# g1mv/density

Hardware: NVIDIA H100
Metric: chameleon_encode_input_GBps (higher is better)
Workload: dtype u32

## Files before the change

### density_b200/csrc/api.cu

```cuda
#include "../../include/density_b200.h"
#include "common.cuh"
#include "encode_internal.cuh"

#include <dlfcn.h>

#include <atomic>
#include <condition_variable>
#include <cstdio>
#include <cstring>
#include <deque>
#include <mutex>
#include <string>
#include <thread>
#include <vector>

namespace dns {

static thread_local std::string g_last_error;
static std::atomic<uint64_t> g_launches{0};

static void set_error(const char* what, cudaError_t e) {
    char buf[512];
    snprintf(buf, sizeof buf, "%s: %s (%s)", what, cudaGetErrorString(e), cudaGetErrorName(e));
    g_last_error = buf;
}
static void set_error(const char* what) { g_last_error = what; }

struct DevBuf {
    uint8_t* p = nullptr; size_t bytes = 0;
    cudaError_t ensure(size_t need, cudaStream_t stream = nullptr) {
        if (need <= bytes) return cudaSuccess;
        if (p) { cudaFree(p); p = nullptr; bytes = 0; }
        size_t want = need + need / 8 + 4096;
        cudaError_t e = cudaMalloc(&p, want);
        if (e != cudaSuccess) { cudaGetLastError(); e = cudaMalloc(&p, need); want = need; }
        if (e == cudaSuccess) { bytes = want; e = cudaMemsetAsync(p, 0, want, stream); }
        return e;
    }
    void release() { if (p) cudaFree(p); p = nullptr; bytes = 0; }
};

class CopyPool {
public:
    static CopyPool& get() { static CopyPool p; return p; }
    void copy(void* dst, const void* src, size_t n) {
        const size_t nparts = (n >= (8u << 20) && !th_.empty()) ? th_.size() : 1;
        if (nparts == 1) { memcpy(dst, src, n); return; }
        Job job; job.left = (int)nparts;
        const size_t per = ((n + nparts - 1) / nparts + 4095) & ~(size_t)4095;
        {
            std::lock_guard<std::mutex> lk(m_);
            for (size_t k = 0; k < nparts; ++k) {
                const size_t off = k * per;
                const size_t len = off >= n ? 0 : (n - off < per ? n - off : per);
                q_.push_back(Task{static_cast<uint8_t*>(dst) + off, static_cast<const uint8_t*>(src) + off, len, &job});
            }
        }
        cv_.notify_all();
        std::unique_lock<std::mutex> lk(m_);
        done_.wait(lk, [&] { return job.left == 0; });
    }
private:
    struct Job { int left; };
    struct Task { uint8_t* d; const uint8_t* s; size_t n; Job* job; };
    CopyPool() {
        unsigned hw = std::thread::hardware_concurrency();
        unsigned nt = hw >= 128 ? 32 : (hw >= 32 ? 16 : (hw >= 8 ? hw / 2 : 0));
        for (unsigned i = 0; i < nt; ++i) th_.emplace_back([this] { run(); });
    }
    ~CopyPool() {
        { std::lock_guard<std::mutex> lk(m_); stop_ = true; }
        cv_.notify_all();
        for (auto& t : th_) t.join();
    }
    void run() {
        for (;;) {
            Task t;
            {
                std::unique_lock<std::mutex> lk(m_);
                cv_.wait(lk, [&] { return stop_ || !q_.empty(); });
                if (stop_ && q_.empty()) return;
                t = q_.front(); q_.pop_front();
            }
            if (t.n) memcpy(t.d, t.s, t.n);
            {
                std::lock_guard<std::mutex> lk(m_);
                if (--t.job->left == 0) done_.notify_all();
            }
        }
    }
    std::vector<std::thread> th_;
    std::mutex m_;
    std::condition_variable cv_, done_;
    std::deque<Task> q_;
    bool stop_ = false;
};

constexpr size_t PIN_SLOT = 64u << 20;
struct PinRing {
    uint8_t* slot[2] = {nullptr, nullptr};
    cudaEvent_t ev[2] = {nullptr, nullptr};
    bool used[2] = {false, false};
    unsigned next = 0;
    cudaError_t ensure() {
        for (int k = 0; k < 2; ++k) {
            if (!slot[k]) { cudaError_t e = cudaHostAlloc(reinterpret_cast<void**>(&slot[k]), PIN_SLOT, cudaHostAllocDefault); if (e != cudaSuccess) return e; }
            if (!ev[k]) { cudaError_t e = cudaEventCreateWithFlags(&ev[k], cudaEventDisableTiming); if (e != cudaSuccess) return e; }
        }
        return cudaSuccess;
    }
    void release() {
        for (int k = 0; k < 2; ++k) { if (slot[k]) cudaFreeHost(slot[k]); if (ev[k]) cudaEventDestroy(ev[k]); slot[k] = nullptr; ev[k] = nullptr; used[k] = false; }
    }
};

static bool is_pageable_host(const void* p) {
    cudaPointerAttributes a;
    cudaError_t e = cudaPointerGetAttributes(&a, p);
    if (e != cudaSuccess) { cudaGetLastError(); return true; }
    return a.type == cudaMemoryTypeUnregistered;
}
static cudaError_t h2d_any(PinRing& ring, uint8_t* dst_dev, const uint8_t* src, size_t n, cudaStream_t s, bool pageable) {
    if (!pageable) return cudaMemcpyAsync(dst_dev, src, n, cudaMemcpyHostToDevice, s);
    cudaError_t e = ring.ensure();
    for (size_t off = 0; off < n && e == cudaSuccess; off += PIN_SLOT) {
        const size_t len = n - off < PIN_SLOT ? n - off : PIN_SLOT;
        const unsigned k = ring.next++ & 1u;
        if (ring.used[k]) e = cudaEventSynchronize(ring.ev[k]);
        if (e != cudaSuccess) break;
        CopyPool::get().copy(ring.slot[k], src + off, len);
        e = cudaMemcpyAsync(dst_dev + off, ring.slot[k], len, cudaMemcpyHostToDevice, s);
        if (e == cudaSuccess) e = cudaEventRecord(ring.ev[k], s);
        ring.used[k] = true;
    }
    return e;
}
static cudaError_t d2h_any(PinRing& ring, uint8_t* dst, const uint8_t* src_dev, size_t n, cudaStream_t s, bool pageable) {
    if (!pageable) return cudaMemcpyAsync(dst, src_dev, n, cudaMemcpyDeviceToHost, s);
    cudaError_t e = ring.ensure();
    size_t pend_off = 0, pend_len = 0; unsigned pend_k = 0; bool pending = false;
    for (size_t off = 0; off < n && e == cudaSuccess; off += PIN_SLOT) {
        const size_t len = n - off < PIN_SLOT ? n - off : PIN_SLOT;
        const unsigned k = ring.next++ & 1u;
        if (ring.used[k] && !(pending && pend_k == k)) e = cudaEventSynchronize(ring.ev[k]);
        if (e != cudaSuccess) break;
        e = cudaMemcpyAsync(ring.slot[k], src_dev + off, len, cudaMemcpyDeviceToHost, s);
        if (e == cudaSuccess) e = cudaEventRecord(ring.ev[k], s);
        ring.used[k] = true;
        if (pending && e == cudaSuccess) {
            e = cudaEventSynchronize(ring.ev[pend_k]);
            if (e == cudaSuccess) CopyPool::get().copy(dst + pend_off, ring.slot[pend_k], pend_len);
        }
        pend_off = off; pend_len = len; pend_k = k; pending = true;
    }
    if (pending && e == cudaSuccess) {
        e = cudaEventSynchronize(ring.ev[pend_k]);
        if (e == cudaSuccess) CopyPool::get().copy(dst + pend_off, ring.slot[pend_k], pend_len);
    }
    return e;
}

struct DeviceCtx {
    int dev = -1;
    int num_sms = 0;
    bool ready = false;
    cudaStream_t stream = nullptr;
    cudaStream_t h2d_stream = nullptr, d2h_stream = nullptr;
    DevBuf ws, stage_in, stage_out, pipe_tables, dec_tables;
    DevBuf chee_tables[2][3];
    uint32_t chee_epoch = 0;
    uint64_t* h_sizes = nullptr;
    cudaEvent_t ev_h2d[2] = {nullptr, nullptr};
    PinRing ring_in, ring_out;
    uint64_t* d_size = nullptr;
    uint64_t* h_size = nullptr;
    ChamLayout layout{};
    int last_was_chameleon_fastpath_capable = 0;
    bool profile = false;
    static constexpr int PROF_RING = 64;
    cudaEvent_t ev[PROF_RING][4] = {};
    uint64_t prof_count = 0;
    const void* last_cl_status = nullptr;
    cudaEvent_t ws_free = nullptr;
    bool ws_free_recorded = false;
    std::mutex mu;
};

constexpr int MAX_DEVICES = 64;
static DeviceCtx g_ctx[MAX_DEVICES];
static std::mutex g_ctx_mu;

static DeviceCtx* current_ctx() {
    int dev = -1;
    cudaError_t e = cudaGetDevice(&dev);
    if (e != cudaSuccess) { set_error("cudaGetDevice", e); return nullptr; }
    if (dev < 0 || dev >= MAX_DEVICES) { set_error("device index out of range"); return nullptr; }
    DeviceCtx* c = &g_ctx[dev];
    std::lock_guard<std::mutex> lk(g_ctx_mu);
    if (!c->ready) {
        cudaDeviceProp prop;
        e = cudaGetDeviceProperties(&prop, dev);
        if (e != cudaSuccess) { set_error("cudaGetDeviceProperties", e); return nullptr; }
        if (prop.major != 9 || prop.minor != 0) { set_error("density_b200 is built for sm_90a and requires a compute capability 9.0 device (H100)"); return nullptr; }
        c->dev = dev;
        c->num_sms = prop.multiProcessorCount;
        e = cudaStreamCreateWithFlags(&c->stream, cudaStreamNonBlocking);
        if (e == cudaSuccess) e = cudaStreamCreateWithFlags(&c->h2d_stream, cudaStreamNonBlocking);
        if (e == cudaSuccess) e = cudaStreamCreateWithFlags(&c->d2h_stream, cudaStreamNonBlocking);
        if (e != cudaSuccess) { set_error("cudaStreamCreate", e); return nullptr; }
        e = cudaMalloc(&c->d_size, 64);
        if (e != cudaSuccess) { set_error("cudaMalloc", e); return nullptr; }
        e = cudaMallocHost(&c->h_size, 64);
        if (e == cudaSuccess) e = cudaMallocHost(&c->h_sizes, sizeof(uint64_t) * 4096);
        if (e != cudaSuccess) { set_error("cudaMallocHost", e); return nullptr; }
        e = cudaEventCreateWithFlags(&c->ws_free, cudaEventDisableTiming);
        if (e != cudaSuccess) { set_error("cudaEventCreate", e); return nullptr; }
        c->ready = true;
    }
    return c;
}

static size_t safe_size(int alg, size_t size) {
    const size_t B = alg_block_bytes(alg), S = alg_sig_bytes(alg);
    return size + (size / B) * S + ((size % B) ? S : 0);
}

static bool is_device_pointer(const void* p) {
    cudaPointerAttributes a;
    cudaError_t e = cudaPointerGetAttributes(&a, p);
    if (e != cudaSuccess) { cudaGetLastError(); return false; }
    return a.type == cudaMemoryTypeDevice || a.type == cudaMemoryTypeManaged;
}

static bool ws_acquire(DeviceCtx* c, cudaStream_t stream) {
    if (!c->ws_free_recorded) return true;
    cudaError_t e = cudaStreamWaitEvent(stream, c->ws_free, 0);
    if (e != cudaSuccess) { set_error("cudaStreamWaitEvent", e); return false; }
    return true;
}
static void ws_release(DeviceCtx* c, cudaStream_t stream) {
    if (cudaEventRecord(c->ws_free, stream) == cudaSuccess) c->ws_free_recorded = true;
}

static int encode_device_locked_impl(DeviceCtx* c, int alg, const uint8_t* d_in, size_t n, uint8_t* d_out, size_t cap,
                                     uint64_t* d_out_size, cudaStream_t stream, int path);
static int encode_device_locked(DeviceCtx* c, int alg, const uint8_t* d_in, size_t n, uint8_t* d_out, size_t cap,
                                uint64_t* d_out_size, cudaStream_t stream, int path) {
    if (!ws_acquire(c, stream)) return DENSITY_B200_ECUDA;
    const int rc = encode_device_locked_impl(c, alg, d_in, n, d_out, cap, d_out_size, stream, path);
    ws_release(c, stream);
    return rc;
}
static int encode_device_locked_impl(DeviceCtx* c, int alg, const uint8_t* d_in, size_t n, uint8_t* d_out, size_t cap,
                                     uint64_t* d_out_size, cudaStream_t stream, int path) {
    uint64_t launches = 0;
    cudaError_t e;
    const bool aligned = !(reinterpret_cast<uintptr_t>(d_in) & 3) && !(reinterpret_cast<uintptr_t>(d_out) & 1);
    if (alg == ALG_CHAMELEON && path != 3 && aligned) {
        ChamLayout L;
        size_t need = cham_workspace_bytes(n, c->num_sms, &L);
        e = c->ws.ensure(need, stream);
        if (e != cudaSuccess) { set_error("workspace cudaMalloc", e); return DENSITY_B200_ECUDA; }
        c->layout = L;
        if (path == 2) {
            e = cham_encode_protected_only(d_in, n, c->ws.p, L, d_out, cap, d_out_size, stream, &launches);
        } else {
            const uint32_t nruns = cham_pick_runs(n, c->num_sms);
            cudaEvent_t* ev = nullptr;
            if (c->profile) {
                ev = c->ev[c->prof_count % DeviceCtx::PROF_RING];
                for (int i = 0; i < 4; ++i) if (!ev[i]) cudaEventCreate(&ev[i]);
            }
            e = cham_encode_phase1(d_in, n, c->ws.p, L, nruns, nullptr, stream, &launches, ev);
            if (e == cudaSuccess && path == 4)
                e = cham_encode_phase2_blocking(d_in, n, c->ws.p, L, nruns, d_out, cap, d_out_size, 12, stream, &launches);
            else if (e == cudaSuccess)
                e = cham_encode_phase2(d_in, n, c->ws.p, L, nruns, nullptr, d_out, cap, d_out_size, path == 0, false, stream, &launches, ev);
            if (ev != nullptr && e == cudaSuccess) c->prof_count++;
        }
        c->last_was_chameleon_fastpath_capable = (path != 2);
    } else if ((alg == ALG_CHEETAH || alg == ALG_LION) && path != 3 && !(reinterpret_cast<uintptr_t>(d_in) & 3) && !(reinterpret_cast<uintptr_t>(d_out) & 1)) {
        const size_t pw = (chee_workspace_bytes(n, c->num_sms) + 255) & ~(size_t)255;
        e = c->ws.ensure(pw + 256 + scalar_workspace_bytes(alg), stream);
        if (e != cudaSuccess) { set_error("workspace cudaMalloc", e); return DENSITY_B200_ECUDA; }
        DevBuf* tb = c->chee_tables[alg == ALG_LION];
        for (int rg = 0; rg < 3 && e == cudaSuccess; ++rg) e = tb[rg].ensure(chee_tables_bytes(alg, rg, n, c->num_sms) + 256, stream);
        if (e != cudaSuccess) { set_error("workspace cudaMalloc", e); return DENSITY_B200_ECUDA; }
        if (c->chee_epoch > 0x0FFFFF00u) {
            for (int a2 = 0; a2 < 2; ++a2) for (int rg = 0; rg < 3; ++rg)
                if (c->chee_tables[a2][rg].p) { e = cudaMemsetAsync(c->chee_tables[a2][rg].p, 0, c->chee_tables[a2][rg].bytes, stream); if (e != cudaSuccess) break; }
            if (e != cudaSuccess) { set_error("cudaMemsetAsync", e); return DENSITY_B200_ECUDA; }
            c->chee_epoch = 0;
        }
        uint32_t* d_conv = reinterpret_cast<uint32_t*>(c->ws.p + pw);
        uint8_t* const tabs[3] = {tb[0].p, tb[1].p, tb[2].p};
        for (int attempt = 0; attempt <= (path == 4 ? 12 : 0); ++attempt) {
            if (attempt > 0) {
                uint32_t conv = 0;
                e = cudaMemcpyAsync(&conv, d_conv, sizeof conv, cudaMemcpyDeviceToHost, stream);
                if (e == cudaSuccess) e = cudaStreamSynchronize(stream);
                if (e != cudaSuccess || conv) break;
            }
            const uint32_t epoch_base = c->chee_epoch + 1;
            c->chee_epoch += 32;
            e = chee_encode_parallel(alg, d_in, n, d_out, cap, c->ws.p, tabs, epoch_base, c->num_sms, d_out_size, d_conv, attempt > 0, stream, &launches);
            if (e != cudaSuccess) break;
        }
        if (e == cudaSuccess && path != 1)
            e = scalar_encode(alg, d_in, n, d_out, cap, c->ws.p + pw + 256, d_out_size, stream, &launches, d_conv);
        c->last_was_chameleon_fastpath_capable = 0;
    } else {
        if (reinterpret_cast<uintptr_t>(d_out) & 1) { set_error("encode_device: d_out must be 2-byte aligned"); return DENSITY_B200_EARG; }
        e = c->ws.ensure(scalar_workspace_bytes(alg), stream);
        if (e != cudaSuccess) { set_error("workspace cudaMalloc", e); return DENSITY_B200_ECUDA; }
        e = scalar_encode(alg, d_in, n, d_out, cap, c->ws.p, d_out_size, stream, &launches);
        c->last_was_chameleon_fastpath_capable = 0;
    }
    g_launches += launches;
    if (e != cudaSuccess) { set_error("encode launch", e); return DENSITY_B200_ECUDA; }
    return DENSITY_B200_OK;
}

static int decode_device_locked_impl(DeviceCtx* c, int alg, const uint8_t* d_in, size_t n, uint8_t* d_out, size_t cap,
                                     uint64_t* d_out_size, cudaStream_t stream, int path);
static int decode_device_locked(DeviceCtx* c, int alg, const uint8_t* d_in, size_t n, uint8_t* d_out, size_t cap,
                                uint64_t* d_out_size, cudaStream_t stream, int path = 0) {
    if (!ws_acquire(c, stream)) return DENSITY_B200_ECUDA;
    const int rc = decode_device_locked_impl(c, alg, d_in, n, d_out, cap, d_out_size, stream, path);
    ws_release(c, stream);
    return rc;
}
static int decode_device_locked_impl(DeviceCtx* c, int alg, const uint8_t* d_in, size_t n, uint8_t* d_out, size_t cap,
                                     uint64_t* d_out_size, cudaStream_t stream, int path) {
    uint64_t launches = 0;
    cudaError_t e;
    const bool parallel_ok = alg == ALG_CHAMELEON && path != 3 && !(reinterpret_cast<uintptr_t>(d_in) & 1) && !(reinterpret_cast<uintptr_t>(d_out) & 3);
    if (parallel_ok) {
        const size_t pw = (cham_decode_workspace_bytes(n, cap, c->num_sms) + 255) & ~(size_t)255;
        e = c->ws.ensure(pw + 256 + scalar_workspace_bytes(alg), stream);
        if (e != cudaSuccess) { set_error("workspace cudaMalloc", e); return DENSITY_B200_ECUDA; }
        uint32_t* d_nonquiet = reinterpret_cast<uint32_t*>(c->ws.p + pw);
        e = cham_decode_parallel(d_in, n, d_out, cap, c->ws.p, c->num_sms, d_out_size, d_nonquiet, stream, &launches);
        if (e == cudaSuccess && path != 1)
            e = scalar_decode(alg, d_in, n, d_out, cap, c->ws.p + pw + 256, d_out_size, stream, &launches, d_nonquiet);
        g_launches += launches;
        if (e != cudaSuccess) { set_error("decode launch", e); return DENSITY_B200_ECUDA; }
        return DENSITY_B200_OK;
    }
    if (alg == ALG_CHEETAH && path != 3 && !(reinterpret_cast<uintptr_t>(d_in) & 1) && !(reinterpret_cast<uintptr_t>(d_out) & 3)) {
        const size_t pw = (chee_decode_workspace_bytes(n, cap, c->num_sms) + 255) & ~(size_t)255;
        e = c->ws.ensure(pw + 256 + 2 * ((scalar_workspace_bytes(alg) + 255) & ~(size_t)255), stream);
        if (e == cudaSuccess) e = c->dec_tables.ensure(chee_decode_tables_bytes(n, c->num_sms) + 256, stream);
        if (e != cudaSuccess) { set_error("workspace cudaMalloc", e); return DENSITY_B200_ECUDA; }
        uint32_t* d_fallback = reinterpret_cast<uint32_t*>(c->ws.p + pw);
        uint8_t* tail_ws = c->ws.p + pw + 256;
        uint8_t* scalar_ws = tail_ws + ((scalar_workspace_bytes(alg) + 255) & ~(size_t)255);
        e = cudaMemsetAsync(tail_ws, 0, 256, stream);
        if (e == cudaSuccess) e = chee_decode_parallel(d_in, n, d_out, cap, c->ws.p, c->dec_tables.p, tail_ws, c->num_sms, d_out_size, d_fallback, stream, &launches);
        if (e == cudaSuccess) {
            const void* cl_st = nullptr;
            const void* b_st = chee_decode_status_ptr(c->ws.p, n, cap, c->num_sms, &cl_st);
            c->last_cl_status = cl_st;
            e = scalar_decode_tail(alg, d_in, n, d_out, cap, tail_ws, b_st, cl_st, d_out_size, stream, &launches, d_fallback);
        }
        if (e == cudaSuccess && path != 1)
            e = scalar_decode(alg, d_in, n, d_out, cap, scalar_ws, d_out_size, stream, &launches, d_fallback);
        g_launches += launches;
        if (e != cudaSuccess) { set_error("decode launch", e); return DENSITY_B200_ECUDA; }
        return DENSITY_B200_OK;
    }
    e = c->ws.ensure(scalar_workspace_bytes(alg), stream);
    if (e != cudaSuccess) { set_error("workspace cudaMalloc", e); return DENSITY_B200_ECUDA; }
    e = scalar_decode(alg, d_in, n, d_out, cap, c->ws.p, d_out_size, stream, &launches);
    g_launches += launches;
    if (e != cudaSuccess) { set_error("decode launch", e); return DENSITY_B200_ECUDA; }
    return DENSITY_B200_OK;
}

constexpr size_t PIPE_CHUNK = 64u << 20;
constexpr size_t PIPE_MIN_BYTES = 96u << 20;

static size_t chameleon_encode_host_pipelined(DeviceCtx* c, const uint8_t* in, size_t n, uint8_t* out, size_t out_cap) {
    const size_t nchunks = (n + PIPE_CHUNK - 1) / PIPE_CHUNK;
    if (nchunks > 4096) return (size_t)-1;
    cudaError_t e = c->stage_in.ensure(n + 16);
    if (e == cudaSuccess) e = c->stage_out.ensure(safe_size(ALG_CHAMELEON, n) + 16);
    if (e == cudaSuccess) e = c->pipe_tables.ensure(2 * 65536 * sizeof(uint32_t) + (nchunks + 1) * sizeof(uint64_t) + 256);
    ChamLayout L;
    if (e == cudaSuccess) e = c->ws.ensure(cham_workspace_bytes(PIPE_CHUNK, c->num_sms, &L));
    if (e != cudaSuccess) { set_error("pipeline cudaMalloc", e); return 0; }
    c->layout = L;
    uint32_t* d_acc = reinterpret_cast<uint32_t*>(c->pipe_tables.p);
    uint32_t* d_tab = d_acc + 65536;
    uint64_t* d_sizes = reinterpret_cast<uint64_t*>(c->pipe_tables.p + 2 * 65536 * sizeof(uint32_t));
    uint32_t* d_flag = reinterpret_cast<uint32_t*>(d_sizes + nchunks);
    for (int k = 0; k < 2; ++k) if (!c->ev_h2d[k]) cudaEventCreateWithFlags(&c->ev_h2d[k], cudaEventDisableTiming);
    uint64_t launches = 0;
    const bool pg_in = is_pageable_host(in), pg_out = is_pageable_host(out);
    std::vector<cudaEvent_t> evs(nchunks, nullptr);
    bool ok = true;
    auto stage_chunk = [&](size_t i) {
        const size_t off = i * PIPE_CHUNK, len = (n - off < PIPE_CHUNK) ? (n - off) : PIPE_CHUNK;
        ok = h2d_any(c->ring_in, c->stage_in.p + off, in + off, len, c->h2d_stream, pg_in) == cudaSuccess;
        if (ok) ok = cudaEventCreateWithFlags(&evs[i], cudaEventDisableTiming) == cudaSuccess;
        if (ok) ok = cudaEventRecord(evs[i], c->h2d_stream) == cudaSuccess;
    };
    size_t staged = 0;
    for (; staged < (pg_in ? (size_t)1 : nchunks) && ok; ++staged) stage_chunk(staged);
    size_t out_off = 0;
    bool nonquiet = false;
    e = cudaMemsetAsync(d_flag, 0, sizeof(uint32_t), c->stream);
    if (ok && e == cudaSuccess) e = cham_table_init(d_acc, c->stream, &launches);
    for (size_t i = 0; i < nchunks && ok && e == cudaSuccess; ++i) {
        const size_t off = i * PIPE_CHUNK, len = (n - off < PIPE_CHUNK) ? (n - off) : PIPE_CHUNK;
        const uint32_t nruns = cham_pick_runs(len, c->num_sms);
        e = cudaStreamWaitEvent(c->stream, evs[i], 0);
        if (e == cudaSuccess) e = cham_encode_phase1(c->stage_in.p + off, len, c->ws.p, L, nruns, d_tab, c->stream, &launches);
        if (e == cudaSuccess) e = cham_encode_phase2(c->stage_in.p + off, len, c->ws.p, L, nruns, i ? d_acc : nullptr, c->stage_out.p + out_off,
                                                     c->stage_out.bytes - out_off, d_sizes + i, false, i != 0, c->stream, &launches);
        if (e == cudaSuccess) e = cham_status_accumulate(c->ws.p, L, d_flag, c->stream, &launches);
        if (e == cudaSuccess) e = cham_table_fold(d_acc, d_tab, c->stream, &launches);
        if (e == cudaSuccess) e = cudaMemcpyAsync(c->h_sizes + i, d_sizes + i, sizeof(uint64_t), cudaMemcpyDeviceToHost, c->stream);
        if (e == cudaSuccess) e = cudaMemcpyAsync(c->h_size, d_flag, sizeof(uint32_t), cudaMemcpyDeviceToHost, c->stream);
        if (e == cudaSuccess && pg_in && staged < nchunks) { stage_chunk(staged); ++staged; }
        if (e == cudaSuccess) e = cudaStreamSynchronize(c->stream);
        if (e != cudaSuccess) break;
        if (*reinterpret_cast<uint32_t*>(c->h_size) != 0) { nonquiet = true; break; }
        const uint64_t sz = c->h_sizes[i];
        if (sz == 0) { ok = false; set_error("pipelined encode: device reported an error"); break; }
        if (out_off + sz > out_cap) { ok = false; set_error("output buffer too small"); break; }
        e = d2h_any(c->ring_out, out + out_off, c->stage_out.p + out_off, sz, c->d2h_stream, pg_out);
        out_off += sz;
    }
    g_launches += launches;
    if (nonquiet) for (; staged < nchunks && ok; ++staged) stage_chunk(staged);
    cudaError_t e2 = cudaStreamSynchronize(c->h2d_stream);
    cudaError_t e3 = cudaStreamSynchronize(c->d2h_stream);
    for (auto ev : evs) if (ev) cudaEventDestroy(ev);
    if (e != cudaSuccess || e2 != cudaSuccess || e3 != cudaSuccess) { set_error("pipelined encode", e != cudaSuccess ? e : (e2 != cudaSuccess ? e2 : e3)); return 0; }
    if (!ok) return 0;
    if (nonquiet) return (size_t)-1;
    c->last_was_chameleon_fastpath_capable = 2;
    return out_off;
}

static size_t run_sync(bool encode, int alg, const uint8_t* in, size_t n, uint8_t* out, size_t out_cap) {
    g_last_error.clear();
    if ((!in && n) || (!out && out_cap)) { set_error("null pointer"); return 0; }
    if (n == 0) return 0;
    DeviceCtx* c = current_ctx();
    if (!c) return 0;
    std::lock_guard<std::mutex> lk(c->mu);
    const bool in_dev = is_device_pointer(in), out_dev = is_device_pointer(out);
    cudaError_t e;
    if (in_dev || out_dev) {
        e = cudaDeviceSynchronize();
        if (e != cudaSuccess) { set_error("cudaDeviceSynchronize", e); return 0; }
    }
    const uint8_t* d_in = in;
    uint8_t* d_out = out;
    size_t d_cap = out_cap;
    bool input_staged = false;
    if (encode && alg == ALG_CHAMELEON && !in_dev && !out_dev && n >= PIPE_MIN_BYTES) {
        const size_t r = chameleon_encode_host_pipelined(c, in, n, out, out_cap);
        if (r != (size_t)-1) return r;
        input_staged = true;
        d_in = c->stage_in.p;
    }
    if (!in_dev && !input_staged) {
        e = c->stage_in.ensure(n + 16);
        if (e != cudaSuccess) { set_error("staging cudaMalloc", e); return 0; }
        e = h2d_any(c->ring_in, c->stage_in.p, in, n, c->stream, is_pageable_host(in));
        if (e != cudaSuccess) { set_error("H2D copy", e); return 0; }
        d_in = c->stage_in.p;
    }
    if (!out_dev) {
        d_cap = encode ? safe_size(alg, n) : out_cap;
        e = c->stage_out.ensure(d_cap + 16);
        if (e != cudaSuccess) { set_error("staging cudaMalloc", e); return 0; }
        d_out = c->stage_out.p;
    }
    int rc = encode ? encode_device_locked(c, alg, d_in, n, d_out, d_cap, c->d_size, c->stream, 4)
                    : decode_device_locked(c, alg, d_in, n, d_out, d_cap, c->d_size, c->stream);
    if (rc != DENSITY_B200_OK) { cudaStreamSynchronize(c->stream); return 0; }
    e = cudaMemcpyAsync(c->h_size, c->d_size, sizeof(uint64_t), cudaMemcpyDeviceToHost, c->stream);
    if (e == cudaSuccess) e = cudaStreamSynchronize(c->stream);
    if (e != cudaSuccess) { set_error("stream sync", e); return 0; }
    const uint64_t produced = *c->h_size;
    if (produced == 0) { set_error(encode ? "encode failed on device (output capacity?)" : "decode failed on device (malformed stream or output capacity)"); return 0; }
    if (produced > out_cap) { set_error("output buffer too small"); return 0; }
    if (!out_dev) {
        e = d2h_any(c->ring_out, out, d_out, produced, c->stream, is_pageable_host(out));
        if (e == cudaSuccess) e = cudaStreamSynchronize(c->stream);
        if (e != cudaSuccess) { set_error("D2H copy", e); return 0; }
    }
    return (size_t)produced;
}

}

using namespace dns;

extern "C" {

int density_b200_decode_status(uint64_t* out10) {
    DeviceCtx* c = current_ctx();
    if (!c || !c->ws.p) return DENSITY_B200_EARG;
    std::lock_guard<std::mutex> lk(c->mu);
    unsigned char raw[64] = {0};
    if (cudaDeviceSynchronize() != cudaSuccess || cudaMemcpy(raw, c->ws.p, sizeof(raw), cudaMemcpyDeviceToHost) != cudaSuccess) return DENSITY_B200_ECUDA;
    const unsigned long long* q = reinterpret_cast<const unsigned long long*>(raw);
    const unsigned int* w = reinterpret_cast<const unsigned int*>(raw + 24);
    out10[0] = q[0]; out10[1] = q[1]; out10[2] = q[2];
    for (int k = 0; k < 7; ++k) out10[3 + k] = w[k];
    return DENSITY_B200_OK;
}

size_t chameleon_encode(const uint8_t* i, size_t n, uint8_t* o, size_t c) { return run_sync(true, ALG_CHAMELEON, i, n, o, c); }
size_t chameleon_decode(const uint8_t* i, size_t n, uint8_t* o, size_t c) { return run_sync(false, ALG_CHAMELEON, i, n, o, c); }
size_t chameleon_safe_encode_buffer_size(size_t s) { return safe_size(ALG_CHAMELEON, s); }
size_t cheetah_encode(const uint8_t* i, size_t n, uint8_t* o, size_t c) { return run_sync(true, ALG_CHEETAH, i, n, o, c); }
size_t cheetah_decode(const uint8_t* i, size_t n, uint8_t* o, size_t c) { return run_sync(false, ALG_CHEETAH, i, n, o, c); }
size_t cheetah_safe_encode_buffer_size(size_t s) { return safe_size(ALG_CHEETAH, s); }
size_t lion_encode(const uint8_t* i, size_t n, uint8_t* o, size_t c) { return run_sync(true, ALG_LION, i, n, o, c); }
size_t lion_decode(const uint8_t* i, size_t n, uint8_t* o, size_t c) { return run_sync(false, ALG_LION, i, n, o, c); }
size_t lion_safe_encode_buffer_size(size_t s) { return safe_size(ALG_LION, s); }

static int device_entry(bool encode, int alg, const uint8_t* d_in, size_t n, uint8_t* d_out, size_t cap, uint64_t* d_out_size,
                        void* stream, int path) {
    g_last_error.clear();
    if (alg < 0 || alg > 2) { set_error("bad algorithm id"); return DENSITY_B200_EARG; }
    if (!d_out_size || (!d_in && n) || (!d_out && cap)) { set_error("null pointer"); return DENSITY_B200_EARG; }
    DeviceCtx* c = current_ctx();
    if (!c) return DENSITY_B200_ECUDA;
    std::lock_guard<std::mutex> lk(c->mu);
    cudaStream_t s = reinterpret_cast<cudaStream_t>(stream);
    if (n == 0) {
        cudaError_t e = cudaMemsetAsync(d_out_size, 0, sizeof(uint64_t), s);
        if (e != cudaSuccess) { set_error("memset", e); return DENSITY_B200_ECUDA; }
        return DENSITY_B200_OK;
    }
    return encode ? encode_device_locked(c, alg, d_in, n, d_out, cap, d_out_size, s, path)
                  : decode_device_locked(c, alg, d_in, n, d_out, cap, d_out_size, s, path);
}

int density_b200_encode_device(int alg, const uint8_t* d_in, size_t n, uint8_t* d_out, size_t cap, uint64_t* d_out_size, void* stream) {
    return device_entry(true, alg, d_in, n, d_out, cap, d_out_size, stream, 0);
}
int density_b200_decode_device(int alg, const uint8_t* d_in, size_t n, uint8_t* d_out, size_t cap, uint64_t* d_out_size, void* stream) {
    return device_entry(false, alg, d_in, n, d_out, cap, d_out_size, stream, 0);
}
int density_b200_encode_device_path(int alg, const uint8_t* d_in, size_t n, uint8_t* d_out, size_t cap, uint64_t* d_out_size,
                                    void* stream, int path) {
    if (path < 0 || path > 4) { set_error("bad path"); return DENSITY_B200_EARG; }
    return device_entry(true, alg, d_in, n, d_out, cap, d_out_size, stream, path);
}
int density_b200_decode_device_path(int alg, const uint8_t* d_in, size_t n, uint8_t* d_out, size_t cap, uint64_t* d_out_size,
                                    void* stream, int path) {
    if (path != 0 && path != 1 && path != 3) { set_error("bad path"); return DENSITY_B200_EARG; }
    return device_entry(false, alg, d_in, n, d_out, cap, d_out_size, stream, path);
}

struct density_b200_shard {
    DevBuf ws;
    ChamLayout L{};
    const uint8_t* d_in = nullptr;
    size_t n = 0;
    uint32_t nruns = 0;
    int is_last = 1;
    int num_sms = 0;
    bool phase1_done = false;
};

density_b200_shard* density_b200_shard_create(void) {
    g_last_error.clear();
    DeviceCtx* c = current_ctx();
    if (!c) return nullptr;
    density_b200_shard* s = new density_b200_shard();
    s->num_sms = c->num_sms;
    return s;
}
void density_b200_shard_destroy(density_b200_shard* s) {
    if (!s) return;
    s->ws.release();
    delete s;
}
int density_b200_shard_phase1(density_b200_shard* s, const uint8_t* d_in, size_t n, int is_last_shard, uint32_t* d_table_out, void* stream) {
    g_last_error.clear();
    if (!s || (!d_in && n) || !d_table_out) { set_error("null pointer"); return DENSITY_B200_EARG; }
    if (!is_last_shard && (n % 256)) { set_error("non-final shards must be a multiple of 256 bytes"); return DENSITY_B200_EARG; }
    if (reinterpret_cast<uintptr_t>(d_in) & 3) { set_error("d_in must be 4-byte aligned"); return DENSITY_B200_EARG; }
    size_t need = cham_workspace_bytes(n, s->num_sms, &s->L);
    cudaError_t e = s->ws.ensure(need);
    if (e != cudaSuccess) { set_error("workspace cudaMalloc", e); return DENSITY_B200_ECUDA; }
    s->d_in = d_in; s->n = n; s->is_last = is_last_shard; s->nruns = cham_pick_runs(n, s->num_sms);
    uint64_t launches = 0;
    cudaStream_t st = reinterpret_cast<cudaStream_t>(stream);
    if (n == 0) {
        e = cudaMemsetAsync(d_table_out, 0, 65536 * sizeof(uint32_t), st);
    } else {
        e = cham_encode_phase1(d_in, n, s->ws.p, s->L, s->nruns, d_table_out, st, &launches);
    }
    g_launches += launches;
    if (e != cudaSuccess) { set_error("shard phase1", e); return DENSITY_B200_ECUDA; }
    s->phase1_done = true;
    return DENSITY_B200_OK;
}
int density_b200_shard_phase2(density_b200_shard* s, const uint32_t* d_carry_in, uint8_t* d_out, size_t cap, uint64_t* d_out_size,
                              uint32_t* d_flags, void* stream) {
    g_last_error.clear();
    if (!s || !s->phase1_done || !d_out_size) { set_error("shard_phase2: phase1 not done / null pointer"); return DENSITY_B200_EARG; }
    if (reinterpret_cast<uintptr_t>(d_out) & 1) { set_error("d_out must be 2-byte aligned"); return DENSITY_B200_EARG; }
    uint64_t launches = 0;
    cudaStream_t st = reinterpret_cast<cudaStream_t>(stream);
    cudaError_t e = cham_encode_phase2(s->d_in, s->n, s->ws.p, s->L, s->nruns, d_carry_in, d_out, cap, d_out_size, false,
                                       d_carry_in != nullptr, st, &launches, nullptr);
    if (e == cudaSuccess && d_flags) {
        if (s->n) e = cudaMemcpyAsync(d_flags, s->ws.p + s->L.status + offsetof(Status, nonquiet), sizeof(uint32_t), cudaMemcpyDeviceToDevice, st);
        else e = cudaMemsetAsync(d_flags, 0, sizeof(uint32_t), st);
    }
    g_launches += launches;
    if (e != cudaSuccess) { set_error("shard phase2", e); return DENSITY_B200_ECUDA; }
    return DENSITY_B200_OK;
}

struct density_b200_decode_shard {
    DevBuf ws;
    const uint8_t* d_in = nullptr;
    size_t n = 0, cap = 0;
    int is_last = 1;
    int num_sms = 0;
    bool phase1_done = false;
};

density_b200_decode_shard* density_b200_decode_shard_create(void) {
    g_last_error.clear();
    DeviceCtx* c = current_ctx();
    if (!c) return nullptr;
    density_b200_decode_shard* s = new density_b200_decode_shard();
    s->num_sms = c->num_sms;
    return s;
}
void density_b200_decode_shard_destroy(density_b200_decode_shard* s) {
    if (!s) return;
    s->ws.release();
    delete s;
}
int density_b200_decode_shard_phase1(density_b200_decode_shard* s, const uint8_t* d_in, size_t n, size_t cap, int is_last_shard,
                                     uint32_t* d_table_out, void* stream) {
    g_last_error.clear();
    if (!s || (!d_in && n) || !d_table_out) { set_error("null pointer"); return DENSITY_B200_EARG; }
    if (reinterpret_cast<uintptr_t>(d_in) & 1) { set_error("d_in must be 2-byte aligned"); return DENSITY_B200_EARG; }
    cudaStream_t st = reinterpret_cast<cudaStream_t>(stream);
    s->phase1_done = false;
    cudaError_t e = s->ws.ensure(cham_decode_workspace_bytes(n, cap, s->num_sms), st);
    if (e != cudaSuccess) { set_error("workspace cudaMalloc", e); return DENSITY_B200_ECUDA; }
    s->d_in = d_in; s->n = n; s->cap = cap; s->is_last = is_last_shard;
    uint64_t launches = 0;
    if (n == 0) e = cudaMemsetAsync(d_table_out, 0, 65536 * sizeof(uint32_t), st);
    else e = cham_decode_phase1(d_in, n, cap, s->ws.p, s->num_sms, d_table_out, st, &launches);
    g_launches += launches;
    if (e != cudaSuccess) { set_error("decode shard phase1", e); return DENSITY_B200_ECUDA; }
    s->phase1_done = true;
    return DENSITY_B200_OK;
}
int density_b200_decode_shard_phase2(density_b200_decode_shard* s, const uint32_t* d_carry_in, uint8_t* d_out, uint64_t* d_out_size,
                                     uint32_t* d_seam8, void* stream) {
    g_last_error.clear();
    if (!s || !s->phase1_done) { set_error("decode_shard_phase2: phase1 not done"); return DENSITY_B200_EARG; }
    if ((!d_out && s->cap) || !d_out_size || !d_seam8) { set_error("null pointer"); return DENSITY_B200_EARG; }
    if (reinterpret_cast<uintptr_t>(d_out) & 3) { set_error("d_out must be 4-byte aligned"); return DENSITY_B200_EARG; }
    cudaStream_t st = reinterpret_cast<cudaStream_t>(stream);
    uint64_t launches = 0;
    cudaError_t e;
    if (s->n == 0) {
        e = cudaMemsetAsync(d_out_size, 0, sizeof(uint64_t), st);
        if (e == cudaSuccess) e = cudaMemsetAsync(d_seam8, 0, 8 * sizeof(uint32_t), st);
    } else {
        e = cham_decode_phase2(s->d_in, s->n, d_out, s->cap, s->ws.p, s->num_sms, d_carry_in, d_out_size, st, &launches);
        if (e == cudaSuccess) e = cham_decode_seam_words(s->d_in, s->n, s->cap, s->ws.p, s->num_sms, s->is_last, d_out_size, d_seam8, st, &launches);
    }
    g_launches += launches;
    s->phase1_done = false;
    if (e != cudaSuccess) { set_error("decode shard phase2", e); return DENSITY_B200_ECUDA; }
    return DENSITY_B200_OK;
}

namespace {
typedef struct ncclComm* nccl_comm_t;
struct nccl_unique_id { char internal[128]; };
enum { NCCL_UINT8 = 1, NCCL_UINT32 = 3 };
struct NcclApi {
    int (*GetUniqueId)(nccl_unique_id*) = nullptr;
    int (*CommInitRank)(nccl_comm_t*, int, nccl_unique_id, int) = nullptr;
    int (*CommDestroy)(nccl_comm_t) = nullptr;
    int (*AllGather)(const void*, void*, size_t, int, nccl_comm_t, cudaStream_t) = nullptr;
    int (*Send)(const void*, size_t, int, int, nccl_comm_t, cudaStream_t) = nullptr;
    int (*Recv)(void*, size_t, int, int, nccl_comm_t, cudaStream_t) = nullptr;
    int (*GroupStart)() = nullptr;
    int (*GroupEnd)() = nullptr;
    const char* (*GetErrorString)(int) = nullptr;
    bool ok = false;
};
NcclApi* nccl_api() {
    static NcclApi api;
    static std::once_flag once;
    std::call_once(once, [] {
        void* h = dlopen("libnccl.so.2", RTLD_NOW | RTLD_NOLOAD);
        if (!h) h = dlopen("libnccl.so.2", RTLD_NOW | RTLD_GLOBAL);
        if (!h) return;
        auto sym = [&](const char* n) { return dlsym(h, n); };
        api.GetUniqueId = reinterpret_cast<decltype(api.GetUniqueId)>(sym("ncclGetUniqueId"));
        api.CommInitRank = reinterpret_cast<decltype(api.CommInitRank)>(sym("ncclCommInitRank"));
        api.CommDestroy = reinterpret_cast<decltype(api.CommDestroy)>(sym("ncclCommDestroy"));
        api.AllGather = reinterpret_cast<decltype(api.AllGather)>(sym("ncclAllGather"));
        api.Send = reinterpret_cast<decltype(api.Send)>(sym("ncclSend"));
        api.Recv = reinterpret_cast<decltype(api.Recv)>(sym("ncclRecv"));
        api.GroupStart = reinterpret_cast<decltype(api.GroupStart)>(sym("ncclGroupStart"));
        api.GroupEnd = reinterpret_cast<decltype(api.GroupEnd)>(sym("ncclGroupEnd"));
        api.GetErrorString = reinterpret_cast<decltype(api.GetErrorString)>(sym("ncclGetErrorString"));
        api.ok = api.GetUniqueId && api.CommInitRank && api.CommDestroy && api.AllGather && api.Send && api.Recv && api.GroupStart && api.GroupEnd;
    });
    return api.ok ? &api : nullptr;
}
bool nccl_check(int rc, const char* what) {
    if (rc == 0) return true;
    NcclApi* a = nccl_api();
    std::string m = std::string(what) + ": " + ((a && a->GetErrorString) ? a->GetErrorString(rc) : "NCCL error");
    dns::set_error(m.c_str());
    return false;
}
}

struct density_b200_sharded {
    int rank = 0, world = 1, num_sms = 0;
    nccl_comm_t comm = nullptr;
    DevBuf ws, aux;
    DevBuf dws;
    ChamLayout L{};
    uint64_t* h_offsets = nullptr;
    uint64_t* h_maps = nullptr;
    cudaEvent_t ev[6] = {};
    bool timed = false;
};

int density_b200_sharded_unique_id(uint8_t* out128) {
    g_last_error.clear();
    NcclApi* a = nccl_api();
    if (!a || !out128) { set_error("NCCL is not available in this process"); return DENSITY_B200_ECUDA; }
    nccl_unique_id id;
    if (!nccl_check(a->GetUniqueId(&id), "ncclGetUniqueId")) return DENSITY_B200_ECUDA;
    memcpy(out128, id.internal, 128);
    return DENSITY_B200_OK;
}

density_b200_sharded* density_b200_sharded_create(const uint8_t* nccl_unique_id_128, int rank, int world) {
    g_last_error.clear();
    if (world < 1 || rank < 0 || rank >= world) { set_error("bad rank / world"); return nullptr; }
    DeviceCtx* c = current_ctx();
    if (!c) return nullptr;
    density_b200_sharded* h = new density_b200_sharded();
    h->rank = rank; h->world = world; h->num_sms = c->num_sms;
    if (world > 1) {
        NcclApi* a = nccl_api();
        if (!a || !nccl_unique_id_128) { set_error("NCCL is not available / no unique id"); delete h; return nullptr; }
        nccl_unique_id id; memcpy(id.internal, nccl_unique_id_128, 128);
        if (!nccl_check(a->CommInitRank(&h->comm, world, id, rank), "ncclCommInitRank")) { delete h; return nullptr; }
    }
    if (cudaMallocHost(&h->h_offsets, sizeof(uint64_t) * (world + 2)) != cudaSuccess ||
        cudaMallocHost(&h->h_maps, sizeof(uint64_t) * DENSITY_B200_LOCATE_MAP_WORDS * world) != cudaSuccess) {
        set_error("cudaMallocHost");
        if (h->h_offsets) cudaFreeHost(h->h_offsets);
        if (h->comm) { NcclApi* a = nccl_api(); if (a) a->CommDestroy(h->comm); }
        delete h;
        return nullptr;
    }
    for (auto& e : h->ev) cudaEventCreate(&e);
    return h;
}

void density_b200_sharded_destroy(density_b200_sharded* h) {
    if (!h) return;
    if (h->comm) { NcclApi* a = nccl_api(); if (a) a->CommDestroy(h->comm); }
    h->ws.release(); h->aux.release(); h->dws.release();
    if (h->h_offsets) cudaFreeHost(h->h_offsets);
    if (h->h_maps) cudaFreeHost(h->h_maps);
    for (auto& e : h->ev) if (e) cudaEventDestroy(e);
    delete h;
}

struct ShardedAux { uint32_t *tables, *carry, *words; uint64_t *offsets, *maps; };
static cudaError_t sharded_aux(density_b200_sharded* h, cudaStream_t st, ShardedAux* x) {
    const size_t W = (size_t)h->world;
    const size_t aux_tables = W * 65536 * sizeof(uint32_t), aux_carry = 65536 * sizeof(uint32_t), aux_words = W * 8 * sizeof(uint32_t);
    const size_t aux_offsets = (W + 2) * sizeof(uint64_t), aux_maps = W * DENSITY_B200_LOCATE_MAP_WORDS * sizeof(uint64_t);
    const cudaError_t e = h->aux.ensure(aux_tables + aux_carry + aux_words + aux_offsets + aux_maps + 256, st);
    x->tables = reinterpret_cast<uint32_t*>(h->aux.p);
    x->carry = reinterpret_cast<uint32_t*>(h->aux.p + aux_tables);
    x->words = reinterpret_cast<uint32_t*>(h->aux.p + aux_tables + aux_carry);
    x->offsets = reinterpret_cast<uint64_t*>(h->aux.p + aux_tables + aux_carry + aux_words);
    x->maps = reinterpret_cast<uint64_t*>(h->aux.p + aux_tables + aux_carry + aux_words + aux_offsets);
    return e;
}

int density_b200_encode_sharded(density_b200_sharded* h, const uint8_t* d_in, size_t n, uint8_t* d_out, size_t cap, uint64_t* d_out_size,
                                uint32_t* d_flags, uint64_t* d_total_size, int gather_root, uint8_t* d_gather, size_t gather_cap, void* stream_v) {
    g_last_error.clear();
    if (!h || (!d_in && n) || !d_out || !d_out_size) { set_error("null pointer"); return DENSITY_B200_EARG; }
    const bool last = h->rank == h->world - 1;
    if (!last && (n % 256)) { set_error("non-final shards must be a multiple of 256 bytes"); return DENSITY_B200_EARG; }
    if ((reinterpret_cast<uintptr_t>(d_in) & 3) || (reinterpret_cast<uintptr_t>(d_out) & 1)) { set_error("d_in must be 4-byte, d_out 2-byte aligned"); return DENSITY_B200_EARG; }
    if (gather_root >= h->world) { set_error("bad gather root"); return DENSITY_B200_EARG; }
    cudaStream_t st = reinterpret_cast<cudaStream_t>(stream_v);
    NcclApi* a = h->world > 1 ? nccl_api() : nullptr;
    const size_t W = (size_t)h->world;
    cudaError_t e = h->ws.ensure(cham_workspace_bytes(n, h->num_sms, &h->L), st);
    ShardedAux x;
    if (e == cudaSuccess) e = sharded_aux(h, st, &x);
    if (e != cudaSuccess) { set_error("workspace cudaMalloc", e); return DENSITY_B200_ECUDA; }
    uint32_t* d_tables = x.tables;
    uint32_t* d_carry = x.carry;
    uint32_t* d_words = x.words;
    uint64_t* d_offsets = x.offsets;
    const uint32_t nruns = cham_pick_runs(n, h->num_sms);
    uint64_t launches = 0;
    cudaEventRecord(h->ev[0], st);
    cudaEvent_t pev[4] = {nullptr, nullptr, nullptr, nullptr};
    if (n) e = cham_encode_phase1(d_in, n, h->ws.p, h->L, nruns, d_tables + (size_t)h->rank * 65536, st, &launches);
    else e = cudaMemsetAsync(d_tables + (size_t)h->rank * 65536, 0, 65536 * sizeof(uint32_t), st);
    if (e != cudaSuccess) { set_error("sharded phase 1", e); return DENSITY_B200_ECUDA; }
    cudaEventRecord(h->ev[1], st);
    if (h->world > 1) {
        if (!a) { set_error("NCCL is not available"); return DENSITY_B200_ECUDA; }
        if (!nccl_check(a->AllGather(d_tables + (size_t)h->rank * 65536, d_tables, 65536, NCCL_UINT32, h->comm, st), "ncclAllGather(tables)")) return DENSITY_B200_ECUDA;
    }
    e = cham_rank_fold(d_tables, (uint32_t)h->rank, d_carry, st, &launches);
    cudaEventRecord(h->ev[2], st);
    pev[2] = h->ev[3]; pev[3] = h->ev[4];
    if (e == cudaSuccess) e = cham_encode_phase2(d_in, n, h->ws.p, h->L, nruns, d_carry, d_out, cap, d_out_size, false, false, st, &launches, n ? pev : nullptr);
    if (!n) { cudaEventRecord(h->ev[3], st); cudaEventRecord(h->ev[4], st); }
    if (e == cudaSuccess && n) e = cham_seam_words(h->ws.p, h->L, n, d_out_size, d_words + 8 * h->rank, st, &launches);
    else if (e == cudaSuccess) e = cudaMemsetAsync(d_words + 8 * h->rank, 0, 8 * sizeof(uint32_t), st);
    if (e != cudaSuccess) { set_error("sharded phase 2", e); return DENSITY_B200_ECUDA; }
    if (h->world > 1 && !nccl_check(a->AllGather(d_words + 8 * h->rank, d_words, 8, NCCL_UINT32, h->comm, st), "ncclAllGather(seams)")) return DENSITY_B200_ECUDA;
    e = cham_seam_verdict(d_words, (uint32_t)h->world, (uint32_t)h->rank, d_flags, d_total_size, d_offsets, st, &launches);
    if (e != cudaSuccess) { set_error("seam verdict", e); return DENSITY_B200_ECUDA; }
    if (gather_root >= 0) {
        e = cudaMemcpyAsync(h->h_offsets, d_offsets, (W + 1) * sizeof(uint64_t), cudaMemcpyDeviceToHost, st);
        if (e == cudaSuccess) e = cudaStreamSynchronize(st);
        if (e != cudaSuccess) { set_error("gather: sizes to host", e); return DENSITY_B200_ECUDA; }
        const uint64_t total = h->h_offsets[W];
        const uint64_t my_off = h->h_offsets[h->rank], my_size = h->h_offsets[h->rank + 1] - my_off;
        if (h->rank == gather_root) {
            if (!d_gather || gather_cap < total) { set_error("gather buffer too small"); return DENSITY_B200_ECAPACITY; }
            if (my_size) e = cudaMemcpyAsync(d_gather + my_off, d_out, my_size, cudaMemcpyDeviceToDevice, st);
            if (e != cudaSuccess) { set_error("gather: local piece", e); return DENSITY_B200_ECUDA; }
        }
        if (h->world > 1) {
            if (!nccl_check(a->GroupStart(), "ncclGroupStart")) return DENSITY_B200_ECUDA;
            bool ok = true;
            if (h->rank == gather_root) {
                for (int r = 0; r < h->world && ok; ++r) {
                    const uint64_t sz = h->h_offsets[r + 1] - h->h_offsets[r];
                    if (r != h->rank && sz) ok = nccl_check(a->Recv(d_gather + h->h_offsets[r], sz, NCCL_UINT8, r, h->comm, st), "ncclRecv");
                }
            } else if (my_size) ok = nccl_check(a->Send(d_out, my_size, NCCL_UINT8, gather_root, h->comm, st), "ncclSend");
            if (!nccl_check(a->GroupEnd(), "ncclGroupEnd") || !ok) return DENSITY_B200_ECUDA;
        }
    }
    cudaEventRecord(h->ev[5], st);
    h->timed = true;
    g_launches += launches;
    return DENSITY_B200_OK;
}

static int decode_sharded_piece(density_b200_sharded* h, const uint8_t* d_in, size_t n, int is_last, uint8_t* d_out, size_t cap,
                                uint64_t* d_out_size, uint32_t* d_flags, uint64_t* d_total_size, uint64_t* d_out_offset, cudaStream_t st) {
    NcclApi* a = h->world > 1 ? nccl_api() : nullptr;
    if (h->world > 1 && !a) { set_error("NCCL is not available"); return DENSITY_B200_ECUDA; }
    ShardedAux x;
    cudaError_t e = h->dws.ensure(cham_decode_workspace_bytes(n, cap, h->num_sms), st);
    if (e == cudaSuccess) e = sharded_aux(h, st, &x);
    if (e != cudaSuccess) { set_error("workspace cudaMalloc", e); return DENSITY_B200_ECUDA; }
    uint32_t* my_table = x.tables + (size_t)h->rank * 65536;
    uint32_t* my_words = x.words + 8 * h->rank;
    uint64_t launches = 0;
    if (n) e = cham_decode_phase1(d_in, n, cap, h->dws.p, h->num_sms, my_table, st, &launches);
    else e = cudaMemsetAsync(my_table, 0, 65536 * sizeof(uint32_t), st);
    if (e != cudaSuccess) { set_error("sharded decode phase 1", e); return DENSITY_B200_ECUDA; }
    if (h->world > 1 && !nccl_check(a->AllGather(my_table, x.tables, 65536, NCCL_UINT32, h->comm, st), "ncclAllGather(tables)")) return DENSITY_B200_ECUDA;
    e = cham_rank_fold(x.tables, (uint32_t)h->rank, x.carry, st, &launches);
    if (e == cudaSuccess && n) e = cham_decode_phase2(d_in, n, d_out, cap, h->dws.p, h->num_sms, x.carry, d_out_size, st, &launches);
    if (e == cudaSuccess && n) e = cham_decode_seam_words(d_in, n, cap, h->dws.p, h->num_sms, is_last, d_out_size, my_words, st, &launches);
    if (e == cudaSuccess && !n) e = cudaMemsetAsync(d_out_size, 0, sizeof(uint64_t), st);
    if (e == cudaSuccess && !n) e = cudaMemsetAsync(my_words, 0, 8 * sizeof(uint32_t), st);
    if (e != cudaSuccess) { set_error("sharded decode phase 2", e); return DENSITY_B200_ECUDA; }
    if (h->world > 1 && !nccl_check(a->AllGather(my_words, x.words, 8, NCCL_UINT32, h->comm, st), "ncclAllGather(seams)")) return DENSITY_B200_ECUDA;
    e = cham_seam_verdict(x.words, (uint32_t)h->world, (uint32_t)h->rank, d_flags, d_total_size, x.offsets, st, &launches);
    g_launches += launches;
    if (e == cudaSuccess && d_out_offset) e = cudaMemcpyAsync(d_out_offset, x.offsets + h->rank, sizeof(uint64_t), cudaMemcpyDeviceToDevice, st);
    if (e != cudaSuccess) { set_error("seam verdict", e); return DENSITY_B200_ECUDA; }
    return DENSITY_B200_OK;
}

int density_b200_decode_sharded(density_b200_sharded* h, const uint8_t* d_in, size_t n, uint8_t* d_out, size_t cap, uint64_t* d_out_size,
                                uint32_t* d_flags, uint64_t* d_total_size, void* stream_v) {
    g_last_error.clear();
    if (!h || (!d_in && n) || (!d_out && cap) || !d_out_size || !d_flags) { set_error("null pointer"); return DENSITY_B200_EARG; }
    if ((reinterpret_cast<uintptr_t>(d_in) & 1) || (reinterpret_cast<uintptr_t>(d_out) & 3)) { set_error("d_in must be 2-byte, d_out 4-byte aligned"); return DENSITY_B200_EARG; }
    return decode_sharded_piece(h, d_in, n, h->rank == h->world - 1, d_out, cap, d_out_size, d_flags, d_total_size, nullptr,
                                reinterpret_cast<cudaStream_t>(stream_v));
}

int density_b200_decode_locate(density_b200_decode_shard* s, const uint8_t* d_in, size_t n_range, size_t n_halo, uint64_t* d_map, void* stream) {
    g_last_error.clear();
    if (!s || (!d_in && n_range + n_halo) || !d_map) { set_error("null pointer"); return DENSITY_B200_EARG; }
    if ((reinterpret_cast<uintptr_t>(d_in) & 1) || (reinterpret_cast<uintptr_t>(d_map) & 7)) { set_error("d_in must be 2-byte, d_map 8-byte aligned"); return DENSITY_B200_EARG; }
    cudaStream_t st = reinterpret_cast<cudaStream_t>(stream);
    s->phase1_done = false;
    cudaError_t e = s->ws.ensure(cham_locate_workspace_bytes(n_range + n_halo), st);
    if (e != cudaSuccess) { set_error("workspace cudaMalloc", e); return DENSITY_B200_ECUDA; }
    uint64_t launches = 0;
    e = cham_decode_locate(d_in, n_range, n_halo, s->ws.p, d_map, st, &launches);
    g_launches += launches;
    if (e != cudaSuccess) { set_error("decode locate", e); return DENSITY_B200_ECUDA; }
    return DENSITY_B200_OK;
}

int density_b200_locate_piece(const uint64_t* h_maps, int world, int rank, uint64_t out4[4]) {
    g_last_error.clear();
    constexpr uint64_t W = DENSITY_B200_LOCATE_MAP_WORDS, TERM = ~0ull, CH = 16384, HALO = 264, NCAND = 132;
    if (!h_maps || !out4 || world < 1 || rank < 0 || rank >= world) { set_error("locate_piece: null pointer / bad rank or world"); return DENSITY_B200_EARG; }
    uint64_t later = 0;
    for (int r = world - 1; r >= 0; --r) {
        const uint64_t* m = h_maps + (size_t)r * W;
        if (r < world - 1 && m[0] % CH) { set_error("locate_piece: a non-last range is not a multiple of 16384 bytes"); return DENSITY_B200_EARG; }
        if (m[1] != (later < HALO ? later : HALO)) { set_error("locate_piece: a halo is not min(264, the bytes of the later ranges)"); return DENSITY_B200_EARG; }
        for (uint64_t c = 0; c < NCAND; ++c)
            if (m[2 + 2 * c] != TERM && m[2 + 2 * c] >= NCAND) { set_error("locate_piece: bad exit index in a range map"); return DENSITY_B200_EARG; }
        if (m[0] > ~later) { set_error("locate_piece: ranges overflow"); return DENSITY_B200_EARG; }
        later += m[0];
    }
    uint64_t idx = 0, blocks = 0;
    for (int r = 0; r < rank; ++r) {
        const uint64_t* m = h_maps + (size_t)r * W;
        if (m[0] == 0) continue;
        blocks += m[3 + 2 * idx];
        idx = m[2 + 2 * idx];
        if (idx == TERM) { out4[0] = 0; out4[1] = 0; out4[2] = blocks; out4[3] = 1; return DENSITY_B200_OK; }
    }
    const uint64_t* m = h_maps + (size_t)rank * W;
    const uint64_t n_range = m[0], n_halo = m[1];
    if (n_range == 0) { out4[0] = 0; out4[1] = 0; out4[2] = blocks; out4[3] = n_halo == 0; return DENSITY_B200_OK; }
    const uint64_t ex = m[2 + 2 * idx];
    const uint64_t start = 2 * idx, end = ex == TERM ? n_range + n_halo : n_range + 2 * ex;
    if (start > end || end > n_range + n_halo) { set_error("locate_piece: inconsistent range maps"); return DENSITY_B200_EARG; }
    out4[0] = start; out4[1] = end; out4[2] = blocks; out4[3] = end == n_range + n_halo;
    return DENSITY_B200_OK;
}

int density_b200_decode_sharded_stream(density_b200_sharded* h, const uint8_t* d_in, size_t n_range, size_t n_halo, uint8_t* d_out, size_t cap,
                                       uint64_t* d_out_size, uint64_t* d_out_offset, uint32_t* d_flags, uint64_t* d_total_size, void* stream_v) {
    g_last_error.clear();
    if (!h || (!d_in && n_range + n_halo) || (!d_out && cap) || !d_out_size || !d_flags) { set_error("null pointer"); return DENSITY_B200_EARG; }
    if ((reinterpret_cast<uintptr_t>(d_in) & 1) || (reinterpret_cast<uintptr_t>(d_out) & 3)) { set_error("d_in must be 2-byte, d_out 4-byte aligned"); return DENSITY_B200_EARG; }
    cudaStream_t st = reinterpret_cast<cudaStream_t>(stream_v);
    NcclApi* a = h->world > 1 ? nccl_api() : nullptr;
    if (h->world > 1 && !a) { set_error("NCCL is not available"); return DENSITY_B200_ECUDA; }
    const size_t W = (size_t)h->world;
    ShardedAux x;
    cudaError_t e = h->dws.ensure(cham_decode_workspace_bytes(n_range + n_halo, cap, h->num_sms), st);
    if (e == cudaSuccess) e = sharded_aux(h, st, &x);
    if (e != cudaSuccess) { set_error("workspace cudaMalloc", e); return DENSITY_B200_ECUDA; }
    uint64_t* my_map = x.maps + (size_t)h->rank * DENSITY_B200_LOCATE_MAP_WORDS;
    uint64_t launches = 0;
    e = cham_decode_locate(d_in, n_range, n_halo, h->dws.p, my_map, st, &launches);
    g_launches += launches;
    if (e != cudaSuccess) { set_error("decode locate", e); return DENSITY_B200_ECUDA; }
    if (h->world > 1 && !nccl_check(a->AllGather(my_map, x.maps, DENSITY_B200_LOCATE_MAP_WORDS * 8, NCCL_UINT8, h->comm, st), "ncclAllGather(maps)"))
        return DENSITY_B200_ECUDA;
    e = cudaMemcpyAsync(h->h_maps, x.maps, W * DENSITY_B200_LOCATE_MAP_WORDS * sizeof(uint64_t), cudaMemcpyDeviceToHost, st);
    if (e == cudaSuccess) e = cudaStreamSynchronize(st);
    if (e != cudaSuccess) { set_error("range maps to host", e); return DENSITY_B200_ECUDA; }
    uint64_t piece[4];
    const int rc = density_b200_locate_piece(h->h_maps, h->world, h->rank, piece);
    if (rc != DENSITY_B200_OK) return rc;
    return decode_sharded_piece(h, d_in + piece[0], (size_t)(piece[1] - piece[0]), (int)piece[3], d_out, cap, d_out_size, d_flags,
                                d_total_size, d_out_offset, st);
}

int density_b200_sharded_profile(density_b200_sharded* h, float* out_ms) {
    if (!h || !out_ms || !h->timed) return DENSITY_B200_EARG;
    cudaError_t e = cudaEventSynchronize(h->ev[5]);
    for (int k = 0; k < 5 && e == cudaSuccess; ++k) e = cudaEventElapsedTime(&out_ms[k], h->ev[k], h->ev[k + 1]);
    if (e != cudaSuccess) { set_error("sharded_profile", e); return DENSITY_B200_ECUDA; }
    return DENSITY_B200_OK;
}


struct density_b200_codec {
    int alg = 0;
    DevBuf state;
    DevBuf tables;
};

density_b200_codec* density_b200_codec_create(int alg) {
    g_last_error.clear();
    if (alg < 0 || alg > 2) { set_error("bad algorithm id"); return nullptr; }
    DeviceCtx* c = current_ctx();
    if (!c) return nullptr;
    density_b200_codec* h = new density_b200_codec();
    h->alg = alg;
    cudaError_t e = h->state.ensure(scalar_workspace_bytes(alg) + 256, c->stream);
    if (e == cudaSuccess && alg == ALG_CHAMELEON) e = h->tables.ensure(2 * 65536 * sizeof(uint32_t), c->stream);
    if (e == cudaSuccess) e = cudaStreamSynchronize(c->stream);
    if (e != cudaSuccess) { set_error("codec_create", e); h->state.release(); h->tables.release(); delete h; return nullptr; }
    return h;
}
void density_b200_codec_destroy(density_b200_codec* h) {
    if (!h) return;
    h->state.release(); h->tables.release();
    delete h;
}
int density_b200_codec_clear_state(density_b200_codec* h) {
    g_last_error.clear();
    DeviceCtx* c = current_ctx();
    if (!h || !c) return DENSITY_B200_EARG;
    std::lock_guard<std::mutex> lk(c->mu);
    cudaError_t e = cudaMemsetAsync(h->state.p, 0, scalar_workspace_bytes(h->alg) + 256, c->stream);
    if (e == cudaSuccess) e = cudaStreamSynchronize(c->stream);
    if (e != cudaSuccess) { set_error("clear_state", e); return DENSITY_B200_ECUDA; }
    return DENSITY_B200_OK;
}

static size_t codec_run(density_b200_codec* h, bool encode, const uint8_t* in, size_t n, uint8_t* out, size_t out_cap) {
    g_last_error.clear();
    if (!h || (!in && n) || (!out && out_cap)) { set_error("null pointer"); return 0; }
    if (n == 0) return 0;
    DeviceCtx* c = current_ctx();
    if (!c) return 0;
    std::lock_guard<std::mutex> lk(c->mu);
    const int alg = h->alg;
    const bool in_dev = is_device_pointer(in), out_dev = is_device_pointer(out);
    cudaError_t e = cudaSuccess;
    if (in_dev || out_dev) { e = cudaDeviceSynchronize(); if (e != cudaSuccess) { set_error("cudaDeviceSynchronize", e); return 0; } }
    cudaStream_t st = c->stream;
    if (!ws_acquire(c, st)) return 0;
    const uint8_t* d_in = in; uint8_t* d_out = out; size_t d_cap = out_cap;
    if (!in_dev) {
        e = c->stage_in.ensure(n + 16, st);
        if (e == cudaSuccess) e = cudaMemcpyAsync(c->stage_in.p, in, n, cudaMemcpyHostToDevice, st);
        if (e != cudaSuccess) { set_error("H2D copy", e); return 0; }
        d_in = c->stage_in.p;
    }
    if (!out_dev) {
        d_cap = encode ? safe_size(alg, n) : out_cap;
        e = c->stage_out.ensure(d_cap + 16, st);
        if (e != cudaSuccess) { set_error("staging cudaMalloc", e); return 0; }
        d_out = c->stage_out.p;
    }
    uint64_t launches = 0;
    uint32_t* quads = reinterpret_cast<uint32_t*>(h->state.p + 256);
    bool done = false;
    if (encode && alg == ALG_CHAMELEON && !(reinterpret_cast<uintptr_t>(d_in) & 3) && !(reinterpret_cast<uintptr_t>(d_out) & 1)) {
        uint32_t* d_carry = reinterpret_cast<uint32_t*>(h->tables.p);
        uint32_t* d_tab = d_carry + 65536;
        ChamLayout L;
        e = c->ws.ensure(cham_workspace_bytes(n, c->num_sms, &L), st);
        c->layout = L;
        const uint32_t nruns = cham_pick_runs(n, c->num_sms);
        bool ok = false;
        if (e == cudaSuccess) e = cham_quads_to_table(quads, d_carry, st, &launches);
        if (e == cudaSuccess) e = cham_encode_phase1(d_in, n, c->ws.p, L, nruns, nullptr, st, &launches);
        if (e == cudaSuccess) e = cham_encode_phase2_stream(d_in, n, c->ws.p, L, nruns, d_carry, d_out, d_cap, c->d_size, d_tab, 12, st, &launches, &ok);
        if (e == cudaSuccess && ok) { e = cham_table_into_quads(d_tab, quads, st, &launches); done = true; }
        c->last_was_chameleon_fastpath_capable = 0;
    }
    if (e == cudaSuccess && !done) {
        e = encode ? scalar_encode(alg, d_in, n, d_out, d_cap, h->state.p, c->d_size, st, &launches, nullptr, true)
                   : scalar_decode(alg, d_in, n, d_out, d_cap, h->state.p, c->d_size, st, &launches, nullptr, true);
    }
    g_launches += launches;
    if (e == cudaSuccess) e = cudaMemcpyAsync(c->h_size, c->d_size, sizeof(uint64_t), cudaMemcpyDeviceToHost, st);
    if (e == cudaSuccess) e = cudaStreamSynchronize(st);
    ws_release(c, st);
    if (e != cudaSuccess) { set_error("codec call", e); return 0; }
    const uint64_t produced = *c->h_size;
    if (produced == 0) { set_error(encode ? "encode failed on device (output capacity?)" : "decode failed on device (malformed stream or output capacity)"); return 0; }
    if (produced > out_cap) { set_error("output buffer too small"); return 0; }
    if (!out_dev) {
        e = cudaMemcpyAsync(out, d_out, produced, cudaMemcpyDeviceToHost, st);
        if (e == cudaSuccess) e = cudaStreamSynchronize(st);
        if (e != cudaSuccess) { set_error("D2H copy", e); return 0; }
    }
    return (size_t)produced;
}
size_t density_b200_codec_encode(density_b200_codec* h, const uint8_t* in, size_t n, uint8_t* out, size_t cap) { return codec_run(h, true, in, n, out, cap); }
size_t density_b200_codec_decode(density_b200_codec* h, const uint8_t* in, size_t n, uint8_t* out, size_t cap) { return codec_run(h, false, in, n, out, cap); }

int density_b200_table_init(uint32_t* d_table, void* stream) {
    uint64_t l = 0;
    cudaError_t e = cham_table_init(d_table, reinterpret_cast<cudaStream_t>(stream), &l);
    g_launches += l;
    if (e != cudaSuccess) { set_error("table_init", e); return DENSITY_B200_ECUDA; }
    return DENSITY_B200_OK;
}
int density_b200_table_fold(uint32_t* d_acc, const uint32_t* d_next, void* stream) {
    uint64_t l = 0;
    cudaError_t e = cham_table_fold(d_acc, d_next, reinterpret_cast<cudaStream_t>(stream), &l);
    g_launches += l;
    if (e != cudaSuccess) { set_error("table_fold", e); return DENSITY_B200_ECUDA; }
    return DENSITY_B200_OK;
}

void density_b200_profile_enable(int enable) {
    DeviceCtx* c = current_ctx();
    if (!c) return;
    std::lock_guard<std::mutex> lk(c->mu);
    c->profile = enable != 0;
    c->prof_count = 0;
}
int density_b200_profile_get(float* out_ms) {
    DeviceCtx* c = current_ctx();
    if (!c || !out_ms) return DENSITY_B200_EARG;
    std::lock_guard<std::mutex> lk(c->mu);
    if (c->prof_count == 0) return DENSITY_B200_EARG;
    const int nset = (int)(c->prof_count < (uint64_t)DeviceCtx::PROF_RING ? c->prof_count : DeviceCtx::PROF_RING);
    double acc[3] = {0, 0, 0};
    cudaError_t e = cudaSuccess;
    for (int s = 0; s < nset && e == cudaSuccess; ++s) {
        cudaEvent_t* ev = c->ev[s];
        float ms[3];
        e = cudaEventSynchronize(ev[3]);
        if (e == cudaSuccess) e = cudaEventElapsedTime(&ms[0], ev[0], ev[1]);
        if (e == cudaSuccess) e = cudaEventElapsedTime(&ms[1], ev[1], ev[2]);
        if (e == cudaSuccess) e = cudaEventElapsedTime(&ms[2], ev[2], ev[3]);
        for (int k = 0; k < 3; ++k) acc[k] += ms[k];
    }
    if (e != cudaSuccess) { set_error("profile_get", e); return DENSITY_B200_ECUDA; }
    for (int k = 0; k < 3; ++k) out_ms[k] = (float)(acc[k] / nset);
    return DENSITY_B200_OK;
}

const char* density_b200_last_error(void) { return g_last_error.c_str(); }
uint64_t density_b200_kernel_launches(void) { return g_launches.load(); }

int density_b200_last_encode_was_fast(void) {
    DeviceCtx* c = current_ctx();
    if (!c) return 0;
    std::lock_guard<std::mutex> lk(c->mu);
    if (c->last_was_chameleon_fastpath_capable == 2) return 1;
    if (!c->last_was_chameleon_fastpath_capable || !c->ws.p) return 0;
    Status st;
    if (cudaDeviceSynchronize() != cudaSuccess) return 0;
    if (cudaMemcpy(&st, c->ws.p + c->layout.status, sizeof st, cudaMemcpyDeviceToHost) != cudaSuccess) return 0;
    return st.nonquiet ? 0 : 1;
}

int density_b200_encode_status(uint64_t* out6) {
    DeviceCtx* c = current_ctx();
    if (!c || !c->ws.p) return DENSITY_B200_EARG;
    std::lock_guard<std::mutex> lk(c->mu);
    Status st;
    if (cudaDeviceSynchronize() != cudaSuccess || cudaMemcpy(&st, c->ws.p + c->layout.status, sizeof st, cudaMemcpyDeviceToHost) != cudaSuccess) return DENSITY_B200_ECUDA;
    out6[0] = st.out_bytes; out6[1] = st.nonquiet; out6[2] = st.error; out6[3] = st.first_nonquiet_block; out6[4] = st.converged; out6[5] = st.iter_changed;
    return DENSITY_B200_OK;
}

void density_b200_shutdown(void) {
    std::lock_guard<std::mutex> lk(g_ctx_mu);
    int cur = -1;
    cudaGetDevice(&cur);
    for (int d = 0; d < MAX_DEVICES; ++d) {
        DeviceCtx& c = g_ctx[d];
        if (!c.ready) continue;
        cudaSetDevice(d);
        c.ws.release(); c.stage_in.release(); c.stage_out.release(); c.dec_tables.release(); for (int a2 = 0; a2 < 2; ++a2) for (int rg = 0; rg < 3; ++rg) c.chee_tables[a2][rg].release();
        c.chee_epoch = 0;
        if (c.d_size) cudaFree(c.d_size);
        if (c.h_size) cudaFreeHost(c.h_size);
        if (c.stream) cudaStreamDestroy(c.stream);
        if (c.ws_free) { cudaEventDestroy(c.ws_free); c.ws_free = nullptr; c.ws_free_recorded = false; }
        if (c.h2d_stream) cudaStreamDestroy(c.h2d_stream);
        if (c.d2h_stream) cudaStreamDestroy(c.d2h_stream);
        if (c.h_sizes) cudaFreeHost(c.h_sizes);
        c.h2d_stream = c.d2h_stream = nullptr; c.h_sizes = nullptr; c.pipe_tables.release();
        c.ring_in.release(); c.ring_out.release();
        for (auto& set : c.ev) for (auto& e : set) if (e) { cudaEventDestroy(e); e = nullptr; }
        c.d_size = nullptr; c.h_size = nullptr; c.stream = nullptr; c.ready = false;
    }
    if (cur >= 0) cudaSetDevice(cur);
}

int density_b200_cheetah_decode_rounds(uint32_t* out4) {
    DeviceCtx* c = current_ctx();
    if (!c || !c->last_cl_status || !out4) return DENSITY_B200_EARG;
    std::lock_guard<std::mutex> lk(c->mu);
    unsigned int raw[8] = {0};
    if (cudaDeviceSynchronize() != cudaSuccess || cudaMemcpy(raw, c->last_cl_status, sizeof raw, cudaMemcpyDeviceToHost) != cudaSuccess) return DENSITY_B200_ECUDA;
    out4[0] = raw[3]; out4[1] = raw[2] && !raw[5]; out4[2] = raw[6]; out4[3] = 40;
    return DENSITY_B200_OK;
}

void density_b200_test_set_stage_rounds(int k) { g_chee_stage_rounds = (k >= 1 && k <= 7) ? k : 7; }

void density_b200_test_set_flag_impl(int k) { g_cham_flag_impl = (k == 1) ? 1 : 6; }
void density_b200_test_set_decode_impl(int k) { g_cham_decode_impl = (k == 1) ? 1 : 7; }

int density_b200_prot_debug(uint64_t* out32) {
    if (!out32) return DENSITY_B200_EARG;
    if (cudaDeviceSynchronize() != cudaSuccess) return DENSITY_B200_ECUDA;
    return prot_debug_read(reinterpret_cast<unsigned long long*>(out32)) == cudaSuccess ? DENSITY_B200_OK : DENSITY_B200_ECUDA;
}

const char* density_b200_version(void) { return "density_b200 0.1.0 (sm_90a)"; }

}
```

### density_b200/csrc/chameleon_encode.cu

```cuda
#include <cstdio>
#include "common.cuh"
#include "encode_internal.cuh"

namespace dns {
namespace cham {

constexpr int FP_THREADS = 1024;
constexpr int FP_QPT = 4;
constexpr int TILE_Q = FP_THREADS * FP_QPT;
constexpr int SIDE_N = 8192;
constexpr uint32_t SIDE_EMPTY = 0xFFFFFFFFu;

constexpr int CLS_N = 32;
constexpr int CLS_CAP = 128;

constexpr uint32_t R_TOUCHED = 1u << 12, R_SLOW = 1u << 13, R_FIRST = 1u << 14;

struct FlagSmem {
    uint16_t tab[65536];
    uint32_t vbit[2048];
    uint32_t conf[2048];
    uint32_t side[SIDE_N];
    uint2 rec[TILE_Q];
    uint16_t cls_list[CLS_N][CLS_CAP];
    uint32_t cls_count[CLS_N];
    uint32_t sigw[TILE_Q / 32];
    uint32_t nrec;
    uint32_t unres_count;
    uint32_t cls_overflow;
};
static_assert(sizeof(FlagSmem) <= 227 * 1024, "flag pass shared memory");

__device__ __forceinline__ bool bit_test(const uint32_t* bm, uint32_t i) { return (bm[i >> 5] >> (i & 31)) & 1u; }

__device__ __forceinline__ void append_unres(bool pred, uint32_t qidx_in_run, uint32_t h, uint32_t f,
                                             uint32_t* s_count, uint2* __restrict__ unres_run) {
    uint32_t m = __ballot_sync(0xFFFFFFFFu, pred);
    if (m == 0) return;
    uint32_t base = 0;
    const uint32_t lane = threadIdx.x & 31;
    if (lane == 0) base = atomicAdd(s_count, (uint32_t)__popc(m));
    base = __shfl_sync(0xFFFFFFFFu, base, 0);
    if (pred) {
        uint32_t idx = base + __popc(m & lanemask_lt());
        if (idx < 65536u) unres_run[idx] = make_uint2(qidx_in_run, h | (f << 16));
    }
}

__device__ __noinline__ void tile_in_order(FlagSmem& S, const uint32_t* qs, uint32_t rem, uint32_t run_q0,
                                           uint2* __restrict__ unres_run, const uint8_t* __restrict__ cm_tile) {
    const uint32_t lane = threadIdx.x & 31;
    for (uint32_t c = 0; c < TILE_Q / 32; ++c) {
        const uint32_t pos = c * 32 + lane;
        const bool valid = pos < rem && !(cm_tile && cm_tile[pos >> 6]);
        const uint32_t q = qs[pos];
        const uint32_t p = hash_prod(q);
        const uint32_t hh = valid ? prod_hash(p) : 0x10000u + lane;
        const uint32_t ff = prod_fp(p, q);
        uint32_t cur = 0; bool touched = false;
        if (valid) { cur = S.tab[hh]; touched = cur != 0 || bit_test(S.vbit, hh); }
        const uint32_t grp = __match_any_sync(0xFFFFFFFFu, hh);
        const uint32_t lower = grp & lanemask_lt();
        const int pl = lower ? 31 - __clz(lower) : 0;
        const uint32_t fprev = __shfl_sync(0xFFFFFFFFu, ff, pl);
        const bool hit = valid && (lower ? (fprev == ff) : (touched && cur == ff));
        const bool is_last = (grp & lanemask_gt()) == 0;
        if (valid && is_last && (lower || !hit)) {
            S.tab[hh] = (uint16_t)ff;
            if (ff == 0) atomicOr(&S.vbit[hh >> 5], 1u << (hh & 31));
        }
        const uint32_t fb = __ballot_sync(0xFFFFFFFFu, hit);
        if (lane == 0) S.sigw[c] = fb;
        append_unres(valid && !lower && !touched, run_q0 + pos, hh, ff, &S.unres_count, unres_run);
        __syncwarp();
    }
}

__global__ void __launch_bounds__(FP_THREADS, 1)
cham_flag_pass(const uint32_t* __restrict__ in, uint64_t nquads, uint32_t tiles_total, uint32_t nruns,
               uint32_t* __restrict__ sigw_g,
               uint2* __restrict__ unres,
               uint32_t* __restrict__ unres_count,
               uint32_t* __restrict__ final_tab,
               const uint8_t* __restrict__ copymap,
               const Status* __restrict__ gate)
{
    if (gate && !(gate->nonquiet && !gate->converged)) return;
    extern __shared__ __align__(16) unsigned char smem_raw[];
    FlagSmem& S = *reinterpret_cast<FlagSmem*>(smem_raw);
    const uint32_t tid = threadIdx.x, lane = tid & 31, warp = tid >> 5;
    const uint32_t run = blockIdx.x;
    const uint64_t t_begin = (uint64_t)run * tiles_total / nruns;
    const uint64_t t_end = (uint64_t)(run + 1) * tiles_total / nruns;
    uint2* __restrict__ unres_run = unres + (size_t)run * 65536;
    const uint32_t pos0 = warp * 128 + lane;
    const uint32_t ntile_run = (uint32_t)(t_end - t_begin);
    const uint64_t q_begin = t_begin * TILE_Q;
    const uint64_t q_end64 = (t_end * TILE_Q < nquads) ? t_end * TILE_Q : nquads;
    const uint32_t run_quads = q_begin < q_end64 ? (uint32_t)(q_end64 - q_begin) : 0u;
    const uint32_t* __restrict__ rin = in + q_begin;
    uint32_t* __restrict__ rsig = sigw_g + t_begin * (TILE_Q / 32);
    const uint8_t* __restrict__ rcm = copymap ? copymap + t_begin * 64 : nullptr;

    {
        uint4 z = make_uint4(0, 0, 0, 0);
        uint4* t4 = reinterpret_cast<uint4*>(S.tab);
        #pragma unroll 1
        for (uint32_t i = tid; i < 65536 * 2 / 16; i += FP_THREADS) t4[i] = z;
        #pragma unroll 1
        for (uint32_t i = tid; i < 2048; i += FP_THREADS) { S.vbit[i] = 0; S.conf[i] = 0; }
        #pragma unroll 1
        for (uint32_t i = tid; i < SIDE_N; i += FP_THREADS) S.side[i] = SIDE_EMPTY;
        if (tid < CLS_N) S.cls_count[tid] = 0;
        if (tid == 0) { S.unres_count = 0; S.cls_overflow = 0; S.nrec = 0; }
    }
    __syncthreads();

    uint32_t nxt[FP_QPT];
#pragma unroll
    for (int j = 0; j < FP_QPT; ++j) nxt[j] = (pos0 + 32 * j < run_quads) ? ld_stream_u32(rin + pos0 + 32 * j) : 0u;

#ifdef DNS_PHASE_TIMING
    long long ph[8] = {0, 0, 0, 0, 0, 0, 0, 0}, tprev = clock64();
#define DNS_PH(k) { long long tn = clock64(); ph[k] += tn - tprev; tprev = tn; }
#else
#define DNS_PH(k)
#endif
    #pragma unroll 1
    for (uint32_t lt = 0; lt < ntile_run; ++lt) {
        uint32_t q[FP_QPT], h[FP_QPT], f[FP_QPT];
        const uint32_t run_q0 = lt * TILE_Q;
        const uint32_t left = run_q0 < run_quads ? run_quads - run_q0 : 0u;
        const uint32_t rem = left < (uint32_t)TILE_Q ? left : (uint32_t)TILE_Q;
#pragma unroll
        for (int j = 0; j < FP_QPT; ++j) q[j] = nxt[j];
        {
            const uint32_t nleft = left > (uint32_t)TILE_Q ? left - TILE_Q : 0u;
            const uint32_t* __restrict__ np = rin + run_q0 + TILE_Q + pos0;
#pragma unroll
            for (int j = 0; j < FP_QPT; ++j) nxt[j] = (pos0 + 32 * j < nleft) ? ld_stream_u32(np + 32 * j) : 0u;
        }

        uint32_t actmask = 0;
        {
            uint32_t cp = 0;
            if (rcm) cp = (rcm[lt * 64 + warp * 2] ? 1u : 0u) | (rcm[lt * 64 + warp * 2 + 1] ? 2u : 0u);
#pragma unroll
            for (int j = 0; j < FP_QPT; ++j)
                if (pos0 + 32 * j < rem && !((cp >> (j >> 1)) & 1u)) actmask |= 1u << j;
        }
        uint32_t missmask = 0;
        {
            uint32_t old[FP_QPT], tch = 0;
#pragma unroll
            for (int j = 0; j < FP_QPT; ++j) {
                const uint32_t p = hash_prod(q[j]);
                h[j] = prod_hash(p);
                f[j] = prod_fp(p, q[j]);
                old[j] = S.tab[h[j]];
            }
            uint32_t mb[FP_QPT], tot = 0;
#pragma unroll
            for (int j = 0; j < FP_QPT; ++j) {
                bool touched = old[j] != 0;
                if (!touched) touched = bit_test(S.vbit, h[j]);
                if (touched) tch |= 1u << j;
                const bool miss = ((actmask >> j) & 1u) && !(touched && old[j] == f[j]);
                if (miss) missmask |= 1u << j;
                mb[j] = __ballot_sync(0xFFFFFFFFu, miss);
                tot += __popc(mb[j]);
            }
            if (tot) {
                uint32_t base = 0;
                if (lane == 0) base = atomicAdd(&S.nrec, tot);
                base = __shfl_sync(0xFFFFFFFFu, base, 0);
#pragma unroll
                for (int j = 0; j < FP_QPT; ++j) {
                    if (missmask & (1u << j))
                        S.rec[base + __popc(mb[j] & lanemask_lt())] =
                            make_uint2(h[j] | (f[j] << 16), (pos0 + 32 * j) | ((tch >> j) & 1u ? R_TOUCHED : 0u) | (old[j] << 16));
                    base += __popc(mb[j]);
                }
            }
        }
        __syncthreads();
        DNS_PH(0)
        const uint32_t nmiss = S.nrec;

        #pragma unroll 1
        for (uint32_t i = tid; i < nmiss; i += FP_THREADS) {
            const uint2 r = S.rec[i];
            const uint32_t hh = r.x & 0xFFFFu;
            S.tab[hh] = (uint16_t)(r.x >> 16);
            atomicMin(&S.side[hh & (SIDE_N - 1)], ((r.y & 0xFFFu) << 16) | hh);
        }
        __syncthreads();
        DNS_PH(1)

#pragma unroll
        for (int j = 0; j < FP_QPT; ++j) {
            const uint32_t pos = pos0 + 32 * j;
            bool ok = false;
            if (((actmask >> j) & 1u) && !(missmask & (1u << j))) {
                ok = S.tab[h[j]] == f[j];
                if (!ok) {
                    const uint32_t slot = S.side[h[j] & (SIDE_N - 1)];
                    if ((slot & 0xFFFFu) == h[j] && pos < (slot >> 16)) {
                        ok = true;
                    } else {
                        const uint32_t idx = atomicAdd(&S.nrec, 1u);
                        S.rec[idx] = make_uint2(h[j] | (f[j] << 16), pos | R_TOUCHED | (f[j] << 16));
                        const uint32_t c = h[j] >> 11;
                        const uint32_t k = atomicAdd(&S.cls_count[c], 1u);
                        if (k < CLS_CAP) S.cls_list[c][k] = (uint16_t)idx; else S.cls_overflow = 1;
                        atomicOr(&S.conf[h[j] >> 5], 1u << (h[j] & 31));
                    }
                }
            }
            const uint32_t fb = __ballot_sync(0xFFFFFFFFu, ok);
            if (lane == 0) S.sigw[warp * 4 + j] = fb;
        }
        #pragma unroll 1
        for (uint32_t i = tid; i < nmiss; i += FP_THREADS) {
            const uint2 r = S.rec[i];
            const uint32_t hh = r.x & 0xFFFFu;
            const uint32_t slot = S.side[hh & (SIDE_N - 1)];
            const uint32_t w = S.tab[hh];
            uint32_t y = r.y;
            if ((slot & 0xFFFFu) != hh || w != (r.x >> 16)) {
                y |= R_SLOW;
                atomicOr(&S.conf[hh >> 5], 1u << (hh & 31));
            } else if (slot == (((r.y & 0xFFFu) << 16) | hh)) {
                y |= R_FIRST;
            }
            if (y != r.y) S.rec[i].y = y;
        }
        __syncthreads();
        DNS_PH(2)

        #pragma unroll 1
        for (uint32_t i = tid; i < nmiss; i += FP_THREADS) {
            const uint2 r = S.rec[i];
            const uint32_t hh = r.x & 0xFFFFu;
            uint32_t y = r.y;
            if (!(y & R_SLOW) && bit_test(S.conf, hh)) { y |= R_SLOW; S.rec[i].y = y; }
            if (y & R_SLOW) {
                const uint32_t c = hh >> 11;
                const uint32_t k = atomicAdd(&S.cls_count[c], 1u);
                if (k < CLS_CAP) S.cls_list[c][k] = (uint16_t)i; else S.cls_overflow = 1;
            } else if (!(y & R_FIRST)) {
                const uint32_t pos = y & 0xFFFu;
                atomicOr(&S.sigw[pos >> 5], 1u << (pos & 31));
            }
            S.side[hh & (SIDE_N - 1)] = SIDE_EMPTY;
        }
        __syncthreads();
        DNS_PH(3)

        S.conf[tid] = 0; S.conf[tid + FP_THREADS] = 0;
        if (S.cls_overflow) {
            #pragma unroll 1
            for (uint32_t i = tid; i < nmiss; i += FP_THREADS) {
                const uint2 r = S.rec[i];
                S.tab[r.x & 0xFFFFu] = (uint16_t)(r.y >> 16);
            }
            if (tid < CLS_N) S.cls_count[tid] = 0;
            __syncthreads();
            uint32_t* qs = reinterpret_cast<uint32_t*>(S.rec);
#pragma unroll
            for (int j = 0; j < FP_QPT; ++j) qs[pos0 + 32 * j] = q[j];
            if (tid == 0) { S.nrec = 0; S.cls_overflow = 0; }
            __syncthreads();
            if (warp == 0) tile_in_order(S, qs, rem, run_q0, unres_run, rcm ? rcm + lt * 64 : nullptr);
        } else {
            #pragma unroll 1
            for (uint32_t base = warp * 32; base < nmiss; base += FP_THREADS) {
                const uint32_t i = base + lane;
                uint2 r = make_uint2(0, 0);
                if (i < nmiss) r = S.rec[i];
                const uint32_t hh = r.x & 0xFFFFu;
                const bool first = (i < nmiss) && (r.y & (R_FIRST | R_SLOW)) == R_FIRST;
                if (first && (r.x >> 16) == 0) atomicOr(&S.vbit[hh >> 5], 1u << (hh & 31));
                append_unres(first && !(r.y & R_TOUCHED), run_q0 + (r.y & 0xFFFu), hh, r.x >> 16, &S.unres_count, unres_run);
            }
            const uint32_t n = S.cls_count[warp];
            const uint16_t* __restrict__ lst = S.cls_list[warp];
            #pragma unroll 1
            for (uint32_t base = 0; base < n; base += 32) {
                const uint32_t i = base + lane;
                const bool valid = i < n;
                uint32_t pos = 0, hh = 0xFFFFFFFFu, ff = 0, oldv = 0; bool touched = false;
                if (valid) {
                    const uint2 d = S.rec[lst[i]];
                    hh = d.x & 0xFFFFu; ff = d.x >> 16; pos = d.y & 0xFFFu; touched = (d.y & R_TOUCHED) != 0; oldv = d.y >> 16;
                }
                int best = -1; uint32_t bestf = 0; bool later = false;
                #pragma unroll 1
                for (uint32_t k = 0; k < n; ++k) {
                    const uint2 dk = S.rec[lst[k]];
                    const uint32_t pk = dk.y & 0xFFFu;
                    if ((dk.x & 0xFFFFu) == hh) {
                        if (pk < pos && (int)pk > best) { best = (int)pk; bestf = dk.x >> 16; }
                        later |= pk > pos;
                    }
                }
                const bool hit = valid && (best >= 0 ? (bestf == ff) : (touched && oldv == ff));
                if (hit) atomicOr(&S.sigw[pos >> 5], 1u << (pos & 31));
                if (valid && !later) {
                    S.tab[hh] = (uint16_t)ff;
                    if (ff == 0) atomicOr(&S.vbit[hh >> 5], 1u << (hh & 31));
                }
                append_unres(valid && best < 0 && !touched, run_q0 + pos, hh, ff, &S.unres_count, unres_run);
            }
            __syncwarp();
            if (lane == 0) S.cls_count[warp] = 0;
            if (tid == 0) S.nrec = 0;
        }
        __syncthreads();
        DNS_PH(4)

        if (tid < TILE_Q / 32) rsig[lt * (TILE_Q / 32) + tid] = S.sigw[tid];
    }

#ifdef DNS_PHASE_TIMING
    if (tid == 0 && run == 77) { const long long nt = (long long)ntile_run;
        printf("run %u tiles %lld cycles/tile: A %lld B %lld C %lld D %lld F %lld  total %lld\n", run, nt,
               ph[0] / nt, ph[1] / nt, ph[2] / nt, ph[3] / nt, ph[4] / nt, (ph[0] + ph[1] + ph[2] + ph[3] + ph[4]) / nt); }
#endif
    #pragma unroll 1
    for (uint32_t i = tid; i < 65536; i += FP_THREADS) {
        uint32_t v = S.tab[i];
        uint32_t tch = (v != 0 || bit_test(S.vbit, i)) ? 0x10000u : 0u;
        final_tab[(size_t)run * 65536 + i] = v | tch;
    }
    if (tid == 0) unres_count[run] = S.unres_count < 65536u ? S.unres_count : 65536u;
}

constexpr int F6_THREADS = 512, F6_QPT = 8;
constexpr int F6_NW = F6_THREADS / 32, F6_WQ = 32 * F6_QPT;
static_assert(F6_THREADS * F6_QPT == TILE_Q, "tile geometry");
constexpr int F6_MB_SLOTS = 4096, F6_MB_CAP = 4;
constexpr int F6_SEC_SLOTS = 64, F6_SEC_CAP = 16;
#ifdef DNS_PHASE_TIMING
__device__ long long g_f6_ph[8];
#define F6_PH(k) { if (threadIdx.x == 0 && blockIdx.x == 77) { long long tn = clock64(); g_f6_ph[k] += tn - f6_tprev; f6_tprev = tn; } }
#define F6_PH_DECL long long f6_tprev = clock64();
#else
#define F6_PH(k)
#define F6_PH_DECL
#endif
constexpr uint32_t F6_TOUCHED = 1u << 12, F6_DROPPED = 1u << 13;
struct Flag6Smem {
    uint16_t tab[65536];
    uint32_t vbit[2048];
    uint2 rec[TILE_Q];
    union {
        uint16_t mb[F6_MB_SLOTS][F6_MB_CAP];
        uint2 stage[F6_NW][64];
    };
    uint32_t mbcnt[2][F6_MB_SLOTS / 4];
    __align__(16) uint32_t sec[F6_SEC_SLOTS][F6_SEC_CAP];
    uint32_t seccnt[2][F6_SEC_SLOTS];
    uint32_t sigw[2][TILE_Q / 32];
    uint32_t cnt[32];
    uint32_t unres_count;
    uint32_t overflow;
};
static_assert(sizeof(Flag6Smem) <= 227 * 1024, "flag pass shared memory");

__device__ __forceinline__ void f6_append_unres(bool pred, uint32_t qidx_in_run, uint32_t hf, uint32_t* s_count, uint2* __restrict__ unres_run) {
    const uint32_t m = __ballot_sync(0xFFFFFFFFu, pred);
    if (m == 0) return;
    uint32_t base = 0;
    if ((threadIdx.x & 31) == 0) base = atomicAdd(s_count, (uint32_t)__popc(m));
    base = __shfl_sync(0xFFFFFFFFu, base, 0);
    if (pred) {
        const uint32_t idx = base + __popc(m & lanemask_lt());
        if (idx < 65536u) unres_run[idx] = make_uint2(qidx_in_run, hf);
    }
}

static_assert(F6_NW == 16, "one warp per bucket class hash >> 12");
__device__ __forceinline__ void f6_replay_step(Flag6Smem& S, const uint2* stage, uint32_t n, uint32_t buf, uint32_t run_q0,
                                               uint2* __restrict__ unres_run) {
    const uint32_t lane = threadIdx.x & 31;
    const bool valid = lane < n;
    uint2 r = make_uint2(0, 0);
    if (valid) r = stage[lane];
    const uint32_t hh = r.x & 0xFFFFu, ff = r.x >> 16, pos = r.y & 0xFFFu;
    uint32_t cur = 0;
    if (valid) cur = S.tab[hh];
    const uint32_t grp = __match_any_sync(0xFFFFFFFFu, valid ? hh : 0x10000u + lane);
    const uint32_t lower = grp & lanemask_lt();
    const uint32_t fprev = __shfl_sync(0xFFFFFFFFu, ff, lower ? 31 - __clz(lower) : 0);
    bool touched = true, hit;
    if (lower) hit = fprev == ff;
    else {
        if (cur == 0) touched = bit_test(S.vbit, hh);
        hit = touched && cur == ff;
    }
    if (valid && (grp & lanemask_gt()) == 0) {
        S.tab[hh] = (uint16_t)ff;
        if (ff == 0) atomicOr(&S.vbit[hh >> 5], 1u << (hh & 31));
    }
    if (valid && hit) atomicOr(&S.sigw[buf][pos >> 5], 1u << (pos & 31));
    f6_append_unres(valid && !touched, run_q0 + pos, r.x, &S.unres_count, unres_run);
    __syncwarp();
}

__device__ __noinline__ void f6_replay(Flag6Smem& S, uint32_t buf, uint32_t run_q0, uint2* __restrict__ unres_run) {
    const uint32_t lane = threadIdx.x & 31, warp = threadIdx.x >> 5;
    {
        const uint32_t n = S.cnt[warp];
        const uint2* __restrict__ myrec = S.rec + warp * F6_WQ;
        #pragma unroll 1
        for (uint32_t i = lane; i < n; i += 32) {
            const uint2 r = myrec[i];
            S.tab[r.x & 0xFFFFu] = (uint16_t)(r.y >> 16);
        }
    }
    __syncthreads();
    uint2* __restrict__ stage = S.stage[warp];
    uint32_t ns = 0;
    #pragma unroll 1
    for (uint32_t w = 0; w < (uint32_t)F6_NW; ++w) {
        const uint32_t n = S.cnt[w];
        const uint2* __restrict__ rg = S.rec + w * F6_WQ;
        #pragma unroll 1
        for (uint32_t i0 = 0; i0 < n; i0 += 32) {
            const uint32_t i = i0 + lane;
            uint2 r = make_uint2(0, 0);
            if (i < n) r = rg[i];
            const bool mine = i < n && ((r.x & 0xFFFFu) >> 12) == warp;
            const uint32_t m = __ballot_sync(0xFFFFFFFFu, mine);
            if (mine) stage[ns + __popc(m & lanemask_lt())] = r;
            ns += __popc(m);
            if (ns >= 32) {
                __syncwarp();
                f6_replay_step(S, stage, 32, buf, run_q0, unres_run);
                const uint2 rest = stage[32 + lane];
                __syncwarp();
                if (lane < ns - 32) stage[lane] = rest;
                ns -= 32;
                __syncwarp();
            }
        }
    }
    __syncwarp();
    if (ns) f6_replay_step(S, stage, ns, buf, run_q0, unres_run);
}

template <bool GENERIC>
__device__ __forceinline__ void f6_tile(Flag6Smem& S, const uint32_t (&q)[F6_QPT], uint32_t validmask, uint32_t buf, uint32_t run_q0,
                                        uint2* __restrict__ unres_run) {
    const uint32_t tid = threadIdx.x, lane = tid & 31, warp = tid >> 5;
    const uint32_t pos0 = warp * F6_WQ + lane;
    uint32_t h[F6_QPT], f[F6_QPT], old[F6_QPT];
    uint32_t missmask = 0;
    F6_PH_DECL
#pragma unroll
    for (int k = 0; k < F6_MB_SLOTS / 4 / F6_THREADS; ++k) S.mbcnt[buf ^ 1u][tid + k * F6_THREADS] = 0;
    if (tid < F6_SEC_SLOTS) S.seccnt[buf ^ 1u][tid] = 0;
#pragma unroll
    for (int j = 0; j < F6_QPT; ++j) {
        const uint32_t p = hash_prod(q[j]);
        h[j] = prod_hash(p);
        f[j] = prod_fp(p, q[j]);
        old[j] = S.tab[h[j]];
    }
    uint32_t fmin = f[0];
#pragma unroll
    for (int j = 0; j < F6_QPT; ++j) {
        bool miss = old[j] != f[j];
        if (GENERIC) miss = miss && ((validmask >> j) & 1u);
        if (miss) missmask |= 1u << j;
        fmin = min(fmin, f[j]);
    }
    if (fmin == 0) {
#pragma unroll
        for (int j = 0; j < F6_QPT; ++j)
            if (f[j] == 0 && old[j] == 0 && (!GENERIC || ((validmask >> j) & 1u)) && !bit_test(S.vbit, h[j])) missmask |= 1u << j;
    }
    __syncthreads();
    F6_PH(0)
#pragma unroll
    for (int j = 0; j < F6_QPT; ++j)
        if (missmask & (1u << j)) S.tab[h[j]] = (uint16_t)f[j];
    __syncthreads();
    F6_PH(1)
    uint32_t clean[F6_QPT], base = 0;
    uint2* __restrict__ myrec = S.rec + warp * F6_WQ;
#pragma unroll
    for (int j = 0; j < F6_QPT; ++j) {
        bool dirty = (missmask >> j) & 1u;
        if (!dirty) dirty = S.tab[h[j]] != f[j];
        if (GENERIC) dirty = dirty && ((validmask >> j) & 1u);
        const uint32_t db = __ballot_sync(0xFFFFFFFFu, dirty);
        clean[j] = GENERIC ? __ballot_sync(0xFFFFFFFFu, !dirty && ((validmask >> j) & 1u)) : ~db;
        if (dirty) myrec[base + __popc(db & lanemask_lt())] = make_uint2(h[j] | (f[j] << 16), (pos0 + 32 * j) | (old[j] << 16));
        base += __popc(db);
    }
    if (lane == 0) {
#pragma unroll
        for (int j = 0; j < F6_QPT; j += 4)
            *reinterpret_cast<uint4*>(&S.sigw[buf][warp * F6_QPT + j]) = make_uint4(clean[j], clean[j + 1], clean[j + 2], clean[j + 3]);
        S.cnt[warp] = base;
    }
    __syncwarp();
    uint2 r0 = make_uint2(0, 0);
    bool drop0 = false;
    {
        uint32_t carry_x = 0, carry_pos = 0;
        #pragma unroll 1
        for (uint32_t i0 = 0; i0 < base; i0 += 32) {
            const uint32_t i = i0 + lane;
            const bool valid = i < base;
            uint2 r = make_uint2(0xFFFFFFFFu, 0);
            if (valid) {
                r = myrec[i];
                if ((r.y >> 16) != 0 || bit_test(S.vbit, r.x & 0xFFFFu)) r.y |= F6_TOUCHED;
            }
            uint32_t px = __shfl_up_sync(0xFFFFFFFFu, r.x, 1), ppos = __shfl_up_sync(0xFFFFFFFFu, r.y & 0xFFFu, 1);
            if (lane == 0) { px = carry_x; ppos = carry_pos; }
            const bool drop = valid && i != 0 && px == r.x && ppos + 1 == (r.y & 0xFFFu);
            carry_x = __shfl_sync(0xFFFFFFFFu, r.x, 31); carry_pos = __shfl_sync(0xFFFFFFFFu, r.y & 0xFFFu, 31);
            if (i0 == 0) { r0 = r; drop0 = drop; }
            if (drop) {
                const uint32_t pos = r.y & 0xFFFu;
                atomicOr(&S.sigw[buf][pos >> 5], 1u << (pos & 31));
                if (i0) myrec[i].y = r.y | F6_DROPPED;
            } else if (valid) {
                if (i0 && (r.y & F6_TOUCHED)) myrec[i].y = r.y;
                const uint32_t hh = r.x & 0xFFFFu, slot = hh & (F6_MB_SLOTS - 1), sh = (slot & 3u) * 8u;
                const uint32_t k = (atomicAdd(&S.mbcnt[buf][slot >> 2], 1u << sh) >> sh) & 0xFFu;
                if (k < (uint32_t)F6_MB_CAP) S.mb[slot][k] = (uint16_t)(((hh >> 12) << 12) | (warp * F6_WQ + i));
                else {
                    const uint32_t s2 = slot & (F6_SEC_SLOTS - 1);
                    const uint32_t k2 = atomicAdd(&S.seccnt[buf][s2], 1u);
                    if (k2 < (uint32_t)F6_SEC_CAP) S.sec[s2][k2] = (hh << 12) | (warp * F6_WQ + i);
                    else S.overflow = 1;
                }
            }
        }
    }
    __syncthreads();
    F6_PH(2)
#ifdef DNS_PHASE_TIMING
    if (threadIdx.x == 0 && blockIdx.x == 77) { g_f6_ph[6] += S.overflow; uint32_t tot = 0; for (int w = 0; w < F6_NW; ++w) tot += S.cnt[w]; g_f6_ph[7] += tot; }
#endif
    if (S.overflow) {
        f6_replay(S, buf, run_q0, unres_run);
    } else {
        #pragma unroll 1
        for (uint32_t i0 = 0; i0 < base; i0 += 32) {
            const uint32_t i = i0 + lane;
            bool valid = i < base;
            uint2 r = r0;
            if (i0) r = valid ? myrec[i] : make_uint2(0, 0);
            if (i0 ? (r.y & F6_DROPPED) != 0 : drop0) valid = false;
            const uint32_t hh = r.x & 0xFFFFu, ff = r.x >> 16, pos = r.y & 0xFFFu, slot = hh & (F6_MB_SLOTS - 1);
            const uint32_t myidx = warp * F6_WQ + i;
            bool later = false, hit = false, unres = false;
            if (valid) {
                const uint32_t n = (S.mbcnt[buf][slot >> 2] >> ((slot & 3u) * 8u)) & 0xFFu;
                const uint2 e2 = *reinterpret_cast<const uint2*>(&S.mb[slot][0]);
                const uint32_t me = ((hh >> 12) << 12) | myidx;
                int best = -1;
#pragma unroll
                for (int t = 0; t < F6_MB_CAP; ++t) {
                    const uint32_t e = ((t & 2) ? e2.y : e2.x) >> ((t & 1) * 16) & 0xFFFFu;
                    if ((uint32_t)t < n && ((e ^ me) >> 12) == 0) {
                        if (e < me) best = max(best, (int)(e & 0xFFFu));
                        later |= e > me;
                    }
                }
                if (n > (uint32_t)F6_MB_CAP) {
                    const uint32_t s2 = slot & (F6_SEC_SLOTS - 1);
                    const uint32_t n2 = S.seccnt[buf][s2];
                    const uint32_t mine = (hh << 12) | myidx;
                    #pragma unroll 1
                    for (uint32_t t4 = 0; t4 < n2; t4 += 4) {
                        const uint4 e4 = *reinterpret_cast<const uint4*>(&S.sec[s2][t4]);
                        const uint32_t ev[4] = {e4.x, e4.y, e4.z, e4.w};
#pragma unroll
                        for (int t = 0; t < 4; ++t) {
                            const uint32_t e = ev[t];
                            if (t4 + t < n2 && ((e ^ mine) & 0xFFFFF000u) == 0) {
                                if (e < mine) best = max(best, (int)(e & 0xFFFu));
                                later |= e > mine;
                            }
                        }
                    }
                }
                if (best >= 0) hit = (S.rec[best].x >> 16) == ff;
                else if (r.y & F6_TOUCHED) hit = (r.y >> 16) == ff;
                else unres = true;
                if (!later) {
                    S.tab[hh] = (uint16_t)ff;
                    if (ff == 0) atomicOr(&S.vbit[hh >> 5], 1u << (hh & 31));
                }
                if (hit) atomicOr(&S.sigw[buf][pos >> 5], 1u << (pos & 31));
            }
            f6_append_unres(unres, run_q0 + pos, r.x, &S.unres_count, unres_run);
        }
    }
    __syncthreads();
    F6_PH(3)
}

__global__ void __launch_bounds__(F6_THREADS, 1)
cham_flag_pass6(const uint32_t* __restrict__ in, uint64_t nquads, uint32_t tiles_total, uint32_t nruns,
                uint32_t* __restrict__ sigw_g, uint2* __restrict__ unres, uint32_t* __restrict__ unres_count,
                uint32_t* __restrict__ final_tab, const uint8_t* __restrict__ copymap, const Status* __restrict__ gate)
{
    if (gate && !(gate->nonquiet && !gate->converged)) return;
    extern __shared__ __align__(16) unsigned char smem_raw[];
    Flag6Smem& S = *reinterpret_cast<Flag6Smem*>(smem_raw);
    const uint32_t tid = threadIdx.x, lane = tid & 31, warp = tid >> 5;
    const uint32_t run = blockIdx.x;
    const uint64_t t_begin = (uint64_t)run * tiles_total / nruns;
    const uint64_t t_end = (uint64_t)(run + 1) * tiles_total / nruns;
    uint2* __restrict__ unres_run = unres + (size_t)run * 65536;
    const uint32_t pos0 = warp * F6_WQ + lane;
    const uint32_t ntile_run = (uint32_t)(t_end - t_begin);
    const uint64_t q_begin = t_begin * TILE_Q;
    const uint64_t q_end64 = (t_end * TILE_Q < nquads) ? t_end * TILE_Q : nquads;
    const uint32_t run_quads = q_begin < q_end64 ? (uint32_t)(q_end64 - q_begin) : 0u;
    const uint32_t* __restrict__ rin = in + q_begin;
    uint32_t* __restrict__ rsig = sigw_g + t_begin * (TILE_Q / 32);
    const uint8_t* __restrict__ rcm = copymap ? copymap + t_begin * 64 : nullptr;
    {
        const uint4 z = make_uint4(0, 0, 0, 0);
        uint4* t4 = reinterpret_cast<uint4*>(S.tab);
        #pragma unroll 1
        for (uint32_t i = tid; i < 65536 * 2 / 16; i += F6_THREADS) t4[i] = z;
        #pragma unroll 1
        for (uint32_t i = tid; i < 2048; i += F6_THREADS) S.vbit[i] = 0;
        #pragma unroll 1
        for (uint32_t i = tid; i < F6_MB_SLOTS / 4; i += F6_THREADS) { S.mbcnt[0][i] = 0; S.mbcnt[1][i] = 0; }
        if (tid < F6_SEC_SLOTS) { S.seccnt[0][tid] = 0; S.seccnt[1][tid] = 0; }
        if (tid == 0) { S.unres_count = 0; S.overflow = 0; }
    }
    __syncthreads();
    uint32_t nxt[F6_QPT], nxt2[F6_QPT];
#pragma unroll
    for (int j = 0; j < F6_QPT; ++j) {
        nxt[j] = (pos0 + 32 * j < run_quads) ? ld_stream_u32(rin + pos0 + 32 * j) : 0u;
        nxt2[j] = (TILE_Q + pos0 + 32 * j < run_quads) ? ld_stream_u32(rin + TILE_Q + pos0 + 32 * j) : 0u;
    }
    #pragma unroll 1
    for (uint32_t lt = 0; lt < ntile_run; ++lt) {
        uint32_t q[F6_QPT];
        const uint32_t run_q0 = lt * TILE_Q;
        const uint32_t left = run_q0 < run_quads ? run_quads - run_q0 : 0u;
        const uint32_t buf = lt & 1u;
#pragma unroll
        for (int j = 0; j < F6_QPT; ++j) { q[j] = nxt[j]; nxt[j] = nxt2[j]; }
        {
            const uint32_t nleft = left > 2u * TILE_Q ? left - 2u * TILE_Q : 0u;
            const uint32_t* __restrict__ np = rin + run_q0 + 2 * TILE_Q + pos0;
            if (nleft >= (uint32_t)TILE_Q) {
#pragma unroll
                for (int j = 0; j < F6_QPT; ++j) nxt2[j] = ld_stream_u32(np + 32 * j);
            } else {
#pragma unroll
                for (int j = 0; j < F6_QPT; ++j) nxt2[j] = (pos0 + 32 * j < nleft) ? ld_stream_u32(np + 32 * j) : 0u;
            }
        }
        if (left >= (uint32_t)TILE_Q && !rcm) {
            f6_tile<false>(S, q, (1u << F6_QPT) - 1u, buf, run_q0, unres_run);
        } else {
            uint32_t validmask = 0, cp = 0;
            if (rcm) {
#pragma unroll
                for (int b = 0; b < F6_WQ / 64; ++b) cp |= (rcm[lt * 64 + warp * (F6_WQ / 64) + b] ? 1u : 0u) << b;
            }
#pragma unroll
            for (int j = 0; j < F6_QPT; ++j)
                if (pos0 + 32 * j < left && !((cp >> (j >> 1)) & 1u)) validmask |= 1u << j;
            f6_tile<true>(S, q, validmask, buf, run_q0, unres_run);
        }
        if (tid < TILE_Q / 32) rsig[lt * (TILE_Q / 32) + tid] = S.sigw[buf][tid];
        if (tid == 0) S.overflow = 0;
    }
    #pragma unroll 1
    for (uint32_t i = tid; i < 65536; i += F6_THREADS) {
        const uint32_t v = S.tab[i];
        const uint32_t tch = (v != 0 || bit_test(S.vbit, i)) ? 0x10000u : 0u;
        final_tab[(size_t)run * 65536 + i] = v | tch;
    }
    if (tid == 0) unres_count[run] = S.unres_count < 65536u ? S.unres_count : 65536u;
#ifdef DNS_PHASE_TIMING
    if (tid == 0 && run == 77 && ntile_run) { const long long nt = ntile_run;
        printf("f6 run %u tiles %lld cycles/tile: A %lld B %lld C+deposit %lld D+S4 %lld  overflow tiles %lld dirty/tile %lld\n", run, nt, g_f6_ph[0] / nt, g_f6_ph[1] / nt,
               g_f6_ph[2] / nt, g_f6_ph[3] / nt, g_f6_ph[6], g_f6_ph[7] / nt);
        for (int k = 0; k < 8; ++k) g_f6_ph[k] = 0; }
#endif
}

__device__ __forceinline__ bool gate_open(const Status* g) { return !g || (g->nonquiet && !g->converged); }

__global__ void cham_carry_scan(const uint32_t* __restrict__ final_tab, const uint32_t* __restrict__ init, int init_untouched,
                                uint32_t nruns, uint32_t* __restrict__ carry, uint32_t* __restrict__ table_out,
                                const Status* __restrict__ gate = nullptr) {
    if (!gate_open(gate)) return;
    uint32_t hb = blockIdx.x * blockDim.x + threadIdx.x;
    if (hb >= 65536) return;
    uint32_t c = init ? init[hb] : ((hb == 0 && !init_untouched) ? 0x10000u : 0u);
    for (uint32_t r = 0; r < nruns; ++r) {
        if (carry) carry[(size_t)r * 65536 + hb] = c;
        uint32_t v = final_tab[(size_t)r * 65536 + hb];
        if (v & 0x10000u) c = v;
    }
    if (table_out) table_out[hb] = c;
}

__global__ void cham_resolve(const uint2* __restrict__ unres, const uint32_t* __restrict__ unres_count,
                             const uint32_t* __restrict__ carry, uint32_t tiles_total, uint32_t nruns,
                             uint32_t* __restrict__ sigw_g, const Status* __restrict__ gate = nullptr) {
    if (!gate_open(gate)) return;
    const uint32_t run = blockIdx.y;
    const uint32_t n = unres_count[run];
    const uint64_t run_q0 = ((uint64_t)run * tiles_total / nruns) * TILE_Q;
    for (uint32_t i = blockIdx.x * blockDim.x + threadIdx.x; i < n; i += gridDim.x * blockDim.x) {
        uint2 e = unres[(size_t)run * 65536 + i];
        uint32_t c = carry[(size_t)run * 65536 + (e.y & 0xFFFFu)];
        if ((c & 0x10000u) && (c & 0xFFFFu) == (e.y >> 16)) {
            uint64_t gq = run_q0 + e.x;
            atomicOr(&sigw_g[gq >> 5], 1u << (gq & 31));
        }
    }
}

struct ProtSmem {
    uint16_t tab[65536];
    uint32_t vbit[2048];
};

__global__ void __launch_bounds__(1024, 1)
cham_protected_pass(const uint32_t* __restrict__ in, uint64_t nbytes, const Status* __restrict__ status, int only_if_nonquiet,
                    uint32_t* __restrict__ sigw_g, uint8_t* __restrict__ copymap) {
    if (only_if_nonquiet && !(status->nonquiet && !status->converged)) return;
    extern __shared__ __align__(16) unsigned char smem_raw[];
    ProtSmem& S = *reinterpret_cast<ProtSmem*>(smem_raw);
    const uint32_t tid = threadIdx.x, lane = tid & 31;
    {
        uint4 z = make_uint4(0, 0, 0, 0);
        uint4* t4 = reinterpret_cast<uint4*>(S.tab);
        for (uint32_t i = tid; i < 65536 * 2 / 16; i += blockDim.x) t4[i] = z;
        for (uint32_t i = tid; i < 2048; i += blockDim.x) S.vbit[i] = (i == 0) ? 1u : 0u;
    }
    __syncthreads();
    if (tid >= 32) return;

    const uint64_t nquads = nbytes / 4;
    const uint64_t nblocks = (nbytes + 255) / 256;
    Protection ps; ps.init();
    uint32_t n0 = 0, n1 = 0;
    if (nblocks) {
        if (lane < nquads) n0 = in[lane];
        if (32 + lane < nquads) n1 = in[32 + lane];
    }
    for (uint64_t b = 0; b < nblocks; ++b) {
        const uint32_t q0 = n0, q1 = n1;
        {
            uint64_t g = (b + 1) * 64 + lane;
            n0 = (b + 1 < nblocks && g < nquads) ? in[g] : 0u;
            n1 = (b + 1 < nblocks && g + 32 < nquads) ? in[g + 32] : 0u;
        }
        const uint64_t bq0 = b * 64;
        const uint32_t nq = (uint32_t)((nquads - bq0 < 64) ? (nquads - bq0) : 64);
        if (ps.revert_to_copy()) {
            if (lane == 0) { copymap[b] = 1; sigw_g[2 * b] = 0; sigw_g[2 * b + 1] = 0; }
            ps.decay();
            continue;
        }
        uint32_t sig[2];
#pragma unroll
        for (int half = 0; half < 2; ++half) {
            const uint32_t q = half ? q1 : q0;
            const bool valid = half * 32 + lane < nq;
            const uint32_t p = hash_prod(q);
            uint32_t hh = valid ? prod_hash(p) : 0x10000u + lane;
            const uint32_t ff = prod_fp(p, q);
            uint32_t cur = 0; bool touched = false;
            if (valid) { cur = S.tab[hh]; touched = cur != 0 || bit_test(S.vbit, hh); }
            const uint32_t grp = __match_any_sync(0xFFFFFFFFu, hh);
            const uint32_t lower = grp & lanemask_lt();
            const int pl = lower ? 31 - __clz(lower) : 0;
            const uint32_t fprev = __shfl_sync(0xFFFFFFFFu, ff, pl);
            const bool hit = valid && (lower ? (fprev == ff) : (touched && cur == ff));
            const bool is_last = (grp & lanemask_gt()) == 0;
            if (valid && is_last && (lower || !hit)) {
                S.tab[hh] = (uint16_t)ff;
                if (ff == 0) atomicOr(&S.vbit[hh >> 5], 1u << (hh & 31));
            }
            sig[half] = __ballot_sync(0xFFFFFFFFu, hit);
            __syncwarp();
        }
        if (lane == 0) { copymap[b] = 0; sigw_g[2 * b] = sig[0]; sigw_g[2 * b + 1] = sig[1]; }
        const uint32_t hits = __popc(sig[0]) + __popc(sig[1]);
        const uint32_t tailb = (b == nblocks - 1) ? (uint32_t)(nbytes & 3) : 0u;
        const uint32_t out_sz = 8 + 4 * nq - 2 * hits + tailb;
        ps.update(out_sz >= 256);
    }
}

constexpr int PSEG = 256;

__device__ __forceinline__ uint32_t prot_pack(const Protection& ps) { return ps.copy_penalty | (ps.copy_penalty_start << 8) | (ps.previous_incompressible << 16); }
__device__ __forceinline__ void prot_walk(Protection& ps, const uint8_t* __restrict__ inc, uint64_t b0, uint64_t b1, uint8_t* __restrict__ cm) {
    for (uint64_t b = b0; b < b1; ++b) {
        if (ps.revert_to_copy()) { cm[b] = 1; ps.decay(); }
        else { cm[b] = 0; ps.update(__ldcg(&inc[b]) != 0); }
    }
}
constexpr int PROT_ROUNDS = 48, PROT_FAST_ROUNDS = 4;
constexpr int PI_THREADS = 1024;

constexpr uint32_t PC_NS = 10, PC_NP = 10, PC_NC = 2 * PC_NS * PC_NP, PC_ESC = 0xFFFFu, PC_GROUP = 128;
__host__ __device__ __forceinline__ size_t prot_table_elems(uint64_t nseg) {
    const uint64_t ngrp = (nseg + PC_GROUP - 1) / PC_GROUP;
    return (size_t)(2 * (ngrp + 2) + nseg * PC_NC + ngrp * PC_NC + 64);
}
__device__ __forceinline__ void pc_decode(uint32_t c, Protection& ps) {
    ps.copy_penalty = c % PC_NP; ps.copy_penalty_start = (c / PC_NP) % PC_NS + 1u; ps.previous_incompressible = c / (PC_NP * PC_NS);
}
__device__ __forceinline__ uint32_t pc_encode(const Protection& ps) {
    if (ps.copy_penalty >= PC_NP || ps.copy_penalty_start < 1u || ps.copy_penalty_start > PC_NS) return PC_ESC;
    return (ps.previous_incompressible * PC_NS + (ps.copy_penalty_start - 1u)) * PC_NP + ps.copy_penalty;
}

__device__ __forceinline__ void grid_barrier(unsigned int* counter, unsigned int nctas, unsigned int& epoch) {
    __syncthreads();
    if (threadIdx.x == 0) {
        __threadfence();
        atomicAdd(counter, 1u);
        const unsigned int target = (epoch + 1) * nctas;
        while (atomicAdd(counter, 0u) < target) { __nanosleep(64); }
        __threadfence();
    }
    ++epoch;
    __syncthreads();
}

__device__ unsigned long long g_prot_dbg[16][2];

__global__ void __launch_bounds__(PI_THREADS)
prot_iterate(const uint32_t* __restrict__ sigw_g, uint64_t nbytes, uint64_t nblocks, uint32_t nseg, Status* __restrict__ st, int it,
             uint8_t* __restrict__ inc, uint8_t* __restrict__ cm_old, uint8_t* __restrict__ cm_new,
             uint32_t* __restrict__ in_state, uint32_t* __restrict__ out_state, uint16_t* __restrict__ ptab) {
    if (!gate_open(st)) return;
    __shared__ uint32_t s_state[1024], s_in[1024];
    __shared__ uint8_t s_inc[PSEG], s_cm[PSEG];
    __shared__ uint32_t s_cur, s_redo;
    const uint32_t tid = threadIdx.x;
    const uint64_t gtid = (uint64_t)blockIdx.x * PI_THREADS + tid, gsz = (uint64_t)gridDim.x * PI_THREADS;
    unsigned int epoch = 0;
    unsigned int* bar = &st->barrier[it & 7];

    if (sigw_g)
        for (uint64_t b = gtid; b < nblocks; b += gsz)
            if (!(it && cm_old[b])) inc[b] = (nbytes - b * 256 >= 256) && (__popc(sigw_g[2 * b]) + __popc(sigw_g[2 * b + 1]) <= 4);
    if (gtid == 0) { st->relax_changed[0] = 0; st->relax_changed[1] = 0; st->iter_changed = 0; st->pad2[0] = 0; }
    if (gtid < 16 && it == 0) { g_prot_dbg[gtid][0] = ~0ull; g_prot_dbg[gtid][1] = 0; }
    grid_barrier(bar, gridDim.x, epoch);

    bool settled = false;
    int round = 0;
    for (int phase = 0; phase < 2 && !settled; ++phase) {
    const int limit = (phase == 0 && ptab) ? PROT_FAST_ROUNDS : PROT_ROUNDS;
    for (; round < limit; ++round) {
        for (uint64_t s = gtid; s < nseg; s += gsz) {
            const uint32_t new_in = (s && round) ? __ldcg(&out_state[s - 1]) : (1u << 8);
            if (round > 0 && new_in == in_state[s]) continue;
            Protection ps;
            ps.copy_penalty = new_in & 0xFFu; ps.copy_penalty_start = (new_in >> 8) & 0xFFu; ps.previous_incompressible = (new_in >> 16) & 1u;
            ps.counter = s * PSEG;
            const uint64_t b1 = ((s + 1) * PSEG < nblocks) ? (s + 1) * PSEG : nblocks;
            prot_walk(ps, inc, s * PSEG, b1, cm_new);
            in_state[s] = new_in;
            out_state[s] = prot_pack(ps);
            if (round > 0) st->relax_changed[round & 1] = 1;
            else if (prot_pack(ps) != (1u << 8)) atomicAdd(&st->pad2[0], 1u);
        }
        grid_barrier(bar, gridDim.x, epoch);
        if (round == 0 && phase == 0 && ptab) {
            const unsigned int bad = *((volatile unsigned int*)&st->pad2[0]);
            if (bad == 0) { settled = true; break; }
            if (bad > 8u) { round = 1; break; }
        }
        if (round > 0) {
            const bool changed = *((volatile unsigned int*)&st->relax_changed[round & 1]) != 0;
            if (!changed) { settled = true; break; }
        }
        if (gtid == 0) st->relax_changed[(round + 1) & 1] = 0;
        grid_barrier(bar, gridDim.x, epoch);
    }
    if (phase == 0 && !settled && ptab) {
        const uint32_t ngrp = (nseg + PC_GROUP - 1) / PC_GROUP;
        uint32_t* gin = reinterpret_cast<uint32_t*>(ptab);
        uint16_t* T = ptab + 2 * (ngrp + 2);
        uint16_t* GT = T + (size_t)nseg * PC_NC;
        for (uint64_t idx = gtid; idx < (uint64_t)nseg * PC_NC; idx += gsz) {
            const uint64_t s = idx / PC_NC;
            Protection ps; pc_decode((uint32_t)(idx % PC_NC), ps);
            ps.counter = s * PSEG;
            const uint64_t b1 = ((s + 1) * PSEG < nblocks) ? (s + 1) * PSEG : nblocks;
            uint64_t b = s * PSEG;
            for (; b + 16 <= b1; b += 16) {
                const uint4 v = __ldcg(reinterpret_cast<const uint4*>(inc + b));
                const uint32_t w[4] = {v.x, v.y, v.z, v.w};
#pragma unroll
                for (int k = 0; k < 16; ++k) {
                    if (ps.revert_to_copy()) ps.decay();
                    else ps.update(((w[k >> 2] >> ((k & 3) * 8)) & 0xFFu) != 0);
                }
            }
            for (; b < b1; ++b) {
                if (ps.revert_to_copy()) ps.decay();
                else ps.update(__ldcg(&inc[b]) != 0);
            }
            T[idx] = (uint16_t)pc_encode(ps);
        }
        grid_barrier(bar, gridDim.x, epoch);
        for (uint64_t idx = gtid; idx < (uint64_t)ngrp * PC_NC; idx += gsz) {
            const uint32_t g = (uint32_t)(idx / PC_NC);
            uint32_t x = (uint32_t)(idx % PC_NC);
            const uint32_t s1 = ((g + 1) * PC_GROUP < nseg) ? (g + 1) * PC_GROUP : nseg;
            for (uint32_t s = g * PC_GROUP; s < s1 && x != PC_ESC; ++s) x = __ldcg(&T[(size_t)s * PC_NC + x]);
            GT[idx] = (uint16_t)x;
        }
        grid_barrier(bar, gridDim.x, epoch);
        if (gtid == 0) {
            uint32_t x = 0;
            for (uint32_t g = 0; g < ngrp; ++g) { gin[g] = x; if (x != PC_ESC) x = __ldcg(&GT[(size_t)g * PC_NC + x]); }
            gin[ngrp] = x;
        }
        grid_barrier(bar, gridDim.x, epoch);
        if (__ldcg(&gin[ngrp]) != PC_ESC) {
            for (uint64_t g = gtid; g < ngrp; g += gsz) {
                uint32_t x = __ldcg(&gin[g]);
                const uint32_t s1 = ((g + 1) * PC_GROUP < nseg) ? (uint32_t)((g + 1) * PC_GROUP) : nseg;
                for (uint32_t s = (uint32_t)g * PC_GROUP; s < s1; ++s) { in_state[s] = x; x = __ldcg(&T[(size_t)s * PC_NC + x]); }
            }
            grid_barrier(bar, gridDim.x, epoch);
            for (uint64_t s = gtid; s < nseg; s += gsz) {
                Protection ps; pc_decode(__ldcg(&in_state[s]), ps);
                ps.counter = s * PSEG;
                const uint64_t b1 = ((s + 1) * PSEG < nblocks) ? (s + 1) * PSEG : nblocks;
                prot_walk(ps, inc, s * PSEG, b1, cm_new);
            }
            grid_barrier(bar, gridDim.x, epoch);
            settled = true;
        }
    }

    }

    if (!settled) {
        if (blockIdx.x == 0) {
            if (tid == 0) s_cur = 1u << 8;
            for (uint32_t s0 = 0; s0 < nseg; s0 += 1024) {
                __syncthreads();
                for (uint32_t i = tid; i < 1024 && s0 + i < nseg; i += PI_THREADS) { s_state[i] = __ldcg(&out_state[s0 + i]); s_in[i] = __ldcg(&in_state[s0 + i]); }
                __syncthreads();
                const uint32_t cnt = (nseg - s0 < 1024u) ? (nseg - s0) : 1024u;
                uint32_t i = 0;
                while (i < cnt) {
                    if (tid == 0) {
                        uint32_t cur = s_cur;
                        while (i < cnt && cur == s_in[i]) { cur = s_state[i]; ++i; }
                        s_cur = cur;
                        s_redo = (i < cnt) ? i : 0xFFFFFFFFu;
                    }
                    __syncthreads();
                    const uint32_t r = s_redo;
                    if (r == 0xFFFFFFFFu) break;
                    const uint64_t b0 = (uint64_t)(s0 + r) * PSEG;
                    const uint32_t nb = (uint32_t)((nblocks - b0 < (uint64_t)PSEG) ? (nblocks - b0) : PSEG);
                    if (tid < nb) s_inc[tid] = __ldcg(&inc[b0 + tid]);
                    __syncthreads();
                    if (tid == 0) {
                        Protection ps; const uint32_t c = s_cur;
                        ps.copy_penalty = c & 0xFFu; ps.copy_penalty_start = (c >> 8) & 0xFFu; ps.previous_incompressible = (c >> 16) & 1u; ps.counter = b0;
                        for (uint32_t k = 0; k < nb; ++k) {
                            if (ps.revert_to_copy()) { s_cm[k] = 1; ps.decay(); }
                            else { s_cm[k] = 0; ps.update(s_inc[k] != 0); }
                        }
                        s_cur = prot_pack(ps);
                    }
                    __syncthreads();
                    if (tid < nb) cm_new[b0 + tid] = s_cm[tid];
                    i = r + 1;
                    __syncthreads();
                }
            }
        }
        grid_barrier(bar, gridDim.x, epoch);
    }

    {
        bool diff = false;
        unsigned long long first = ~0ull; unsigned int nd = 0;
        for (uint64_t b = gtid; b < nblocks; b += gsz)
            if (__ldcg(&cm_new[b]) != (it ? cm_old[b] : 0)) { diff = true; ++nd; if (b < first) first = b; }
        if (diff) {
            atomicOr(&st->iter_changed, 1u);
            if (it >= 0 && it < 16) { atomicAdd(&g_prot_dbg[it][1], (unsigned long long)nd); atomicMin(&g_prot_dbg[it][0], first); }
        }
    }
    grid_barrier(bar, gridDim.x, epoch);
    const bool converged = *((volatile unsigned int*)&st->iter_changed) == 0;
    if (!converged || it == 0)
        for (uint64_t b = gtid; b < nblocks; b += gsz) cm_old[b] = __ldcg(&cm_new[b]);
    grid_barrier(bar, gridDim.x, epoch);
    if (gtid == 0 && converged) st->converged = 1;
}

__device__ __forceinline__ uint32_t block_out_bytes(uint64_t b, uint64_t nbytes, uint32_t hits, bool copied) {
    const uint64_t boff = b * 256;
    const uint32_t blen = (uint32_t)((nbytes - boff < 256) ? (nbytes - boff) : 256);
    return copied ? blen : 8 + blen - 2 * hits;
}

__global__ void cham_tile_sizes(const uint32_t* __restrict__ sigw_g, const uint8_t* __restrict__ copymap, uint64_t nbytes,
                                uint64_t nblocks, uint32_t ntiles, int use_copymap_if_nonquiet, int check_quiet, int assume_prev_inc,
                                Status* __restrict__ status, uint32_t* __restrict__ tile_bytes) {
    const uint32_t lane = threadIdx.x & 31;
    const uint32_t tile = blockIdx.x * (blockDim.x >> 5) + (threadIdx.x >> 5);
    if (tile >= ntiles) return;
    if (use_copymap_if_nonquiet && !check_quiet && !status->nonquiet) return;
    const bool use_cm = copymap && (!use_copymap_if_nonquiet || status->nonquiet);
    uint32_t sum = 0, incm[2];
#pragma unroll
    for (int k = 0; k < 2; ++k) {
        const uint64_t b = (uint64_t)tile * 64 + k * 32 + lane;
        uint32_t sz = 0; bool inc = false;
        if (b < nblocks) {
            const bool copied = use_cm && copymap[b];
            const uint32_t hits = __popc(sigw_g[2 * b]) + __popc(sigw_g[2 * b + 1]);
            sz = block_out_bytes(b, nbytes, hits, copied);
            inc = !copied && sz >= 256 && (nbytes - b * 256 >= 256);
        }
        sum += sz;
        incm[k] = __ballot_sync(0xFFFFFFFFu, inc);
    }
#pragma unroll
    for (int d = 16; d; d >>= 1) sum += __shfl_xor_sync(0xFFFFFFFFu, sum, d);
    if (lane == 0) tile_bytes[tile] = sum;
    if (check_quiet && lane == 0) {
        bool prev = assume_prev_inc != 0;
        if (tile > 0) {
            const uint64_t b = (uint64_t)tile * 64 - 1;
            const uint32_t hits = __popc(sigw_g[2 * b]) + __popc(sigw_g[2 * b + 1]);
            prev = (8 + 256 - 2 * hits) >= 256;
        }
        const uint64_t m = ((uint64_t)incm[1] << 32) | incm[0];
        const uint64_t pairs = m & ((m << 1) | (prev ? 1ull : 0ull));
        if (pairs) {
            atomicOr(&status->nonquiet, 1u);
            atomicMin(&status->first_nonquiet_block, (unsigned long long)tile * 64 + (__ffsll((long long)pairs) - 1));
        }
    }
}

constexpr int SCAN_T = 1024;
constexpr int SCAN_PER = 4;
constexpr int SCAN_G = SCAN_T * SCAN_PER;

__device__ __forceinline__ uint64_t block_exclusive_scan_u64(uint64_t v, uint64_t* s_warp, uint64_t* total) {
    const uint32_t lane = threadIdx.x & 31, warp = threadIdx.x >> 5;
    uint64_t incl = v;
#pragma unroll
    for (int d = 1; d < 32; d <<= 1) { uint64_t u = __shfl_up_sync(0xFFFFFFFFu, incl, d); if (lane >= (uint32_t)d) incl += u; }
    if (lane == 31) s_warp[warp] = incl;
    __syncthreads();
    if (warp == 0) {
        uint64_t w = (lane < (blockDim.x >> 5)) ? s_warp[lane] : 0;
        uint64_t wi = w;
#pragma unroll
        for (int d = 1; d < 32; d <<= 1) { uint64_t u = __shfl_up_sync(0xFFFFFFFFu, wi, d); if (lane >= (uint32_t)d) wi += u; }
        s_warp[lane] = wi - w;
        if (lane == 31) s_warp[32] = wi;
    }
    __syncthreads();
    if (total) *total = s_warp[32];
    return incl - v + s_warp[warp];
}

__global__ void __launch_bounds__(SCAN_T) scan_groups_local(const uint32_t* __restrict__ tile_bytes, uint32_t ntiles,
                                                           uint32_t* __restrict__ tile_local, uint64_t* __restrict__ group_total) {
    __shared__ uint64_t s_warp[33];
    const uint32_t base = blockIdx.x * SCAN_G + threadIdx.x * SCAN_PER;
    uint32_t v[SCAN_PER]; uint64_t sum = 0;
#pragma unroll
    for (int k = 0; k < SCAN_PER; ++k) { v[k] = (base + k < ntiles) ? tile_bytes[base + k] : 0u; sum += v[k]; }
    uint64_t tot;
    uint64_t ex = block_exclusive_scan_u64(sum, s_warp, &tot);
#pragma unroll
    for (int k = 0; k < SCAN_PER; ++k) { if (base + k < ntiles) tile_local[base + k] = (uint32_t)ex; ex += v[k]; }
    if (threadIdx.x == 0) group_total[blockIdx.x] = tot;
}

__global__ void __launch_bounds__(SCAN_T) scan_group_totals(const uint64_t* __restrict__ group_total, uint32_t ngroups,
                                                           uint64_t* __restrict__ group_off, Status* __restrict__ status,
                                                           uint64_t cap, uint64_t* __restrict__ d_out_size) {
    __shared__ uint64_t s_warp[33];
    __shared__ uint64_t s_carry;
    if (threadIdx.x == 0) s_carry = 0;
    __syncthreads();
    for (uint32_t base = 0; base < ngroups; base += SCAN_T) {
        uint32_t i = base + threadIdx.x;
        uint64_t v = (i < ngroups) ? group_total[i] : 0;
        uint64_t tot;
        uint64_t ex = block_exclusive_scan_u64(v, s_warp, &tot);
        if (i < ngroups) group_off[i] = s_carry + ex;
        __syncthreads();
        if (threadIdx.x == 0) s_carry += tot;
        __syncthreads();
    }
    if (threadIdx.x == 0) {
        uint64_t total = s_carry;
        if (total > cap) { status->error = 2; total = 0; }
        status->out_bytes = total;
        if (d_out_size) *d_out_size = total;
    }
}

constexpr int EM_THREADS = 256;
constexpr int EM_STAGE = 64 * 264 + 32;

__device__ __forceinline__ uint4 ld_stream_u128(const uint32_t* p) {
    uint4 v;
    asm volatile("ld.global.nc.L1::no_allocate.v4.u32 {%0, %1, %2, %3}, [%4];" : "=r"(v.x), "=r"(v.y), "=r"(v.z), "=r"(v.w) : "l"(p));
    return v;
}
__device__ __forceinline__ void bulk_store_smem_to_global(void* gdst, const void* ssrc, uint32_t bytes) {
    const uint32_t s = (uint32_t)__cvta_generic_to_shared(ssrc);
    asm volatile("fence.proxy.async.shared::cta;" ::: "memory");
    asm volatile("cp.async.bulk.global.shared::cta.bulk_group [%0], [%1], %2;" :: "l"(gdst), "r"(s), "r"(bytes) : "memory");
    asm volatile("cp.async.bulk.commit_group;" ::: "memory");
    asm volatile("cp.async.bulk.wait_group.read 0;" ::: "memory");
}

template <bool FULL>
__device__ __forceinline__ void emit_quads(uint8_t* __restrict__ st, const uint32_t* s_off, const uint32_t* s_sig, const uint8_t* s_copied,
                                           const uint4 v, uint32_t u, uint32_t nvalid_tile ) {
    const uint32_t bl = u >> 4, k = (u & 15u) * 4;
    const uint32_t qs[4] = {v.x, v.y, v.z, v.w};
    uint32_t nv = 4;
    if (!FULL) { const uint32_t first = u * 4; nv = nvalid_tile > first ? (nvalid_tile - first < 4 ? nvalid_tile - first : 4u) : 0u; }
    uint8_t* p = st + s_off[bl];
    if (s_copied[bl]) {
        p += 4 * k;
#pragma unroll
        for (int j = 0; j < 4; ++j)
            if (FULL || (uint32_t)j < nv) { st_u16(p + 4 * j, qs[j] & 0xFFFFu); st_u16(p + 4 * j + 2, qs[j] >> 16); }
        return;
    }
    const uint32_t lo = s_sig[2 * bl], hi = s_sig[2 * bl + 1];
    if (k == 0 && (FULL || nv > 0 || true)) {
        st_u16(p, lo & 0xFFFFu); st_u16(p + 2, lo >> 16); st_u16(p + 4, hi & 0xFFFFu); st_u16(p + 6, hi >> 16);
    }
    const uint32_t word = k < 32 ? lo : hi, kk = k & 31u;
    const uint32_t before = (k < 32 ? 0u : (uint32_t)__popc(lo)) + __popc(word & ((1u << kk) - 1u));
    const uint32_t fl = word >> kk;
    p += 8 + 4 * k - 2 * before;
#pragma unroll
    for (int j = 0; j < 4; ++j) {
        if (FULL || (uint32_t)j < nv) {
            const bool hit = (fl >> j) & 1u;
            const uint32_t hsh = prod_hash(hash_prod(qs[j]));
            st_u16(p, hit ? hsh : (qs[j] & 0xFFFFu));
            if (!hit) st_u16(p + 2, qs[j] >> 16);
            p += hit ? 2 : 4;
        }
    }
}

template <bool AL16>
__global__ void __launch_bounds__(EM_THREADS)
cham_emit(const uint32_t* __restrict__ in, uint64_t nbytes, uint64_t nblocks, const uint32_t* __restrict__ sigw_g,
          const uint8_t* __restrict__ copymap, int use_copymap_if_nonquiet, const Status* __restrict__ status,
          const uint32_t* __restrict__ tile_local, const uint64_t* __restrict__ group_off, uint8_t* __restrict__ out) {
    if (status->error) return;
    __shared__ __align__(16) uint8_t s_stage[EM_STAGE];
    __shared__ uint32_t s_off[65];
    __shared__ uint32_t s_sig[128];
    __shared__ uint8_t s_copied[64];
    __shared__ uint32_t s_wsum[2];
    const uint32_t tid = threadIdx.x, lane = tid & 31, warp = tid >> 5;
    const uint32_t tile = blockIdx.x;
    const bool use_cm = copymap && (!use_copymap_if_nonquiet || status->nonquiet);
    const uint64_t tile_off = group_off[tile / SCAN_G] + tile_local[tile];
    const uint64_t nquads = nbytes / 4;
    const uint64_t tq0 = (uint64_t)tile * 4096;
    const bool full = tq0 + 4096 <= nquads;
    const uint32_t nvalid_tile = full ? 4096u : (uint32_t)(nquads > tq0 ? nquads - tq0 : 0);
    uint4 qv[4];
    if (AL16 && full) {
#pragma unroll
        for (int i = 0; i < 4; ++i) qv[i] = ld_stream_u128(in + tq0 + 4u * (i * EM_THREADS + tid));
    } else {
#pragma unroll
        for (int i = 0; i < 4; ++i) {
            const uint32_t r = 4u * (i * EM_THREADS + tid);
            const uint32_t* g = in + tq0 + r;
            qv[i].x = (r + 0 < nvalid_tile) ? ld_stream_u32(g + 0) : 0u;
            qv[i].y = (r + 1 < nvalid_tile) ? ld_stream_u32(g + 1) : 0u;
            qv[i].z = (r + 2 < nvalid_tile) ? ld_stream_u32(g + 2) : 0u;
            qv[i].w = (r + 3 < nvalid_tile) ? ld_stream_u32(g + 3) : 0u;
        }
    }

    const uint64_t b_first = (uint64_t)tile * 64;
    const uint32_t nb_tile = (uint32_t)((nblocks - b_first < 64) ? (nblocks - b_first) : 64);
    if (tid < 64) {
        const uint64_t b = b_first + tid;
        uint32_t sz = 0, lo = 0, hi = 0; bool copied = false;
        if (tid < nb_tile) {
            copied = use_cm && copymap[b];
            lo = sigw_g[2 * b]; hi = sigw_g[2 * b + 1];
            sz = block_out_bytes(b, nbytes, __popc(lo) + __popc(hi), copied);
        }
        s_sig[2 * tid] = lo; s_sig[2 * tid + 1] = hi; s_copied[tid] = copied;
        uint32_t incl = sz;
#pragma unroll
        for (int d = 1; d < 32; d <<= 1) { uint32_t u = __shfl_up_sync(0xFFFFFFFFu, incl, d); if (lane >= (uint32_t)d) incl += u; }
        if (lane == 31) s_wsum[warp] = incl;
        s_off[tid + 1] = incl;
    }
    __syncthreads();
    if (tid >= 32 && tid < 64) s_off[tid + 1] += s_wsum[0];
    if (tid == 0) s_off[0] = 0;
    __syncthreads();

    uint8_t* const gdst = out + tile_off;
    const uint32_t a = (uint32_t)(reinterpret_cast<uintptr_t>(gdst) & 15u);
    uint8_t* const st = s_stage + a;
    if (full) {
#pragma unroll
        for (int i = 0; i < 4; ++i) emit_quads<true>(st, s_off, s_sig, s_copied, qv[i], i * EM_THREADS + tid, 4096u);
    } else {
#pragma unroll
        for (int i = 0; i < 4; ++i) {
            const uint32_t u = i * EM_THREADS + tid;
            if ((u >> 4) < nb_tile) emit_quads<false>(st, s_off, s_sig, s_copied, qv[i], u, nvalid_tile);
        }
        if ((nbytes & 3u) && b_first + nb_tile == nblocks && tid < (uint32_t)(nbytes & 3u)) {
            const uint64_t b = nblocks - 1;
            const uint32_t bl = nb_tile - 1;
            const uint32_t blen = (uint32_t)(nbytes - b * 256);
            const uint32_t nq = blen >> 2;
            const uint32_t at = s_copied[bl] ? (blen & ~3u) : 8 + 4 * nq - 2 * (__popc(s_sig[2 * bl]) + __popc(s_sig[2 * bl + 1]));
            st[s_off[bl] + at + tid] = reinterpret_cast<const uint8_t*>(in)[b * 256 + (blen & ~3u) + tid];
        }
    }
    __syncthreads();

    const uint32_t total = s_off[nb_tile];
    const uint32_t end = a + total;
    const uint32_t mid_lo = a ? 16u : 0u;
    const uint32_t mid_hi = end & ~15u;
    const bool have_mid = mid_hi > mid_lo;
    uint8_t* const gbase = gdst - a;
    if (have_mid && tid == 0) bulk_store_smem_to_global(gbase + mid_lo, s_stage + mid_lo, mid_hi - mid_lo);
    const uint32_t head_hi = have_mid ? mid_lo : end;
    if (tid >= 32 && tid < 64) {
        for (uint32_t o = a + 2 * (tid - 32); o < head_hi; o += 64) {
            if (o + 2 <= head_hi) st_u16(gbase + o, *reinterpret_cast<const uint16_t*>(s_stage + o));
            else gbase[o] = s_stage[o];
        }
    }
    if (have_mid && tid >= 64 && tid < 96) {
        for (uint32_t o = mid_hi + 2 * (tid - 64); o < end; o += 64) {
            if (o + 2 <= end) st_u16(gbase + o, *reinterpret_cast<const uint16_t*>(s_stage + o));
            else gbase[o] = s_stage[o];
        }
    }
}

__global__ void cham_status_accumulate_k(const Status* __restrict__ st, uint32_t* __restrict__ flag) {
    if (st->nonquiet || st->error) *flag = 1;
}
__global__ void cham_table_init_k(uint32_t* __restrict__ t) {
    uint32_t i = blockIdx.x * blockDim.x + threadIdx.x;
    if (i < 65536) t[i] = (i == 0) ? 0x10000u : 0u;
}
__global__ void cham_table_fold_k(uint32_t* __restrict__ acc, const uint32_t* __restrict__ next) {
    uint32_t i = blockIdx.x * blockDim.x + threadIdx.x;
    if (i < 65536) { uint32_t v = next[i]; if (v & 0x10000u) acc[i] = v; }
}

__global__ void cham_quads_to_table_k(const uint32_t* __restrict__ quads, uint32_t* __restrict__ t) {
    const uint32_t h = blockIdx.x * blockDim.x + threadIdx.x;
    if (h >= 65536) return;
    const uint32_t v = quads[h];
    const uint32_t p = hash_prod(v);
    t[h] = (prod_hash(p) == h) ? (0x10000u | prod_fp(p, v)) : 0u;
}
__global__ void cham_table_into_quads_k(const uint32_t* __restrict__ t, uint32_t* __restrict__ quads) {
    const uint32_t h = blockIdx.x * blockDim.x + threadIdx.x;
    if (h >= 65536) return;
    const uint32_t v = t[h];
    if (v & 0x10000u) quads[h] = quad_from_hf(h, v & 0xFFFFu);
}

__global__ void cham_rank_fold_k(const uint32_t* __restrict__ tables, uint32_t rank, uint32_t* __restrict__ carry) {
    const uint32_t i = blockIdx.x * blockDim.x + threadIdx.x;
    if (i >= 65536) return;
    uint32_t c = (i == 0) ? 0x10000u : 0u;
    for (uint32_t r = 0; r < rank; ++r) { const uint32_t v = tables[(size_t)r * 65536 + i]; if (v & 0x10000u) c = v; }
    carry[i] = c;
}
__global__ void cham_seam_words_k(const uint32_t* __restrict__ sigw_g, uint64_t nbytes, uint64_t nblocks, const Status* __restrict__ st,
                                  const uint64_t* __restrict__ d_out_size, uint32_t* __restrict__ words ) {
    if (threadIdx.x || blockIdx.x) return;
    auto inc = [&](uint64_t b) { return (nbytes - b * 256 >= 256) && (__popc(sigw_g[2 * b]) + __popc(sigw_g[2 * b + 1]) <= 4); };
    words[0] = nblocks ? (inc(0) ? 1u : 0u) : 0u;
    words[1] = nblocks ? (inc(nblocks - 1) ? 1u : 0u) : 0u;
    words[2] = (nblocks && (st->nonquiet || st->error)) ? 1u : 0u;
    words[3] = nblocks ? 1u : 0u;
    const uint64_t sz = *d_out_size;
    words[4] = (uint32_t)sz; words[5] = (uint32_t)(sz >> 32); words[6] = 0; words[7] = 0;
}
__global__ void cham_seam_verdict_k(const uint32_t* __restrict__ all_words, uint32_t world, uint32_t rank, uint32_t* __restrict__ d_flags,
                                    uint64_t* __restrict__ d_total, uint64_t* __restrict__ d_sizes ) {
    if (threadIdx.x || blockIdx.x) return;
    uint32_t bad = 0, prev_inc = 0; uint64_t off = 0;
    for (uint32_t r = 0; r < world; ++r) {
        const uint32_t* w = all_words + 8 * r;
        if (w[2]) bad = 1;
        if (w[3]) { if (prev_inc && w[0]) bad = 1; prev_inc = w[1]; }
        if (d_sizes) d_sizes[r] = off;
        off += (uint64_t)w[4] | ((uint64_t)w[5] << 32);
    }
    if (d_sizes) d_sizes[world] = off;
    if (d_flags) *d_flags = bad;
    if (d_total) *d_total = off;
    (void)rank;
}

}

using namespace cham;

size_t cham_workspace_bytes(size_t nbytes, int nruns_max, ChamLayout* L) {
    const uint64_t nblocks = (nbytes + 255) / 256;
    const uint64_t ntiles = (nblocks + 63) / 64;
    const uint64_t ngroups = (ntiles + SCAN_G - 1) / SCAN_G;
    size_t off = 0;
    auto take = [&](size_t bytes) { size_t o = off; off += (bytes + 255) & ~(size_t)255; return o; };
    L->status = take(sizeof(Status));
    L->sigw = take((ntiles * 64 * 2 + 64 + 256) * sizeof(uint32_t));
    L->copymap = take(ntiles * 64 + 64 + 128);
    L->copymap2 = take(ntiles * 64 + 64 + 128);
    L->seg_state = take(prot_state_bytes(ntiles * 64 / PSEG + 2));
    L->incb = take(ntiles * 64 + 64);
    L->tile_bytes = take((ntiles + 1) * sizeof(uint32_t));
    L->tile_local = take((ntiles + 1) * sizeof(uint32_t));
    L->group_total = take((ngroups + 1) * sizeof(uint64_t));
    L->group_off = take((ngroups + 1) * sizeof(uint64_t));
    L->unres = take((size_t)nruns_max * 65536 * sizeof(uint2));
    L->unres_count = take((size_t)nruns_max * sizeof(uint32_t));
    L->final_tab = take((size_t)nruns_max * 65536 * sizeof(uint32_t));
    L->carry = take((size_t)nruns_max * 65536 * sizeof(uint32_t));
    L->total = off;
    return off;
}

static cudaError_t set_smem_attrs_once() {
    static bool done = false;
    static cudaError_t err = cudaSuccess;
    if (!done) {
        err = cudaFuncSetAttribute(cham_flag_pass, cudaFuncAttributeMaxDynamicSharedMemorySize, (int)sizeof(FlagSmem));
        if (err == cudaSuccess)
            err = cudaFuncSetAttribute(cham_flag_pass6, cudaFuncAttributeMaxDynamicSharedMemorySize, (int)sizeof(Flag6Smem));
        if (err == cudaSuccess)
            err = cudaFuncSetAttribute(cham_protected_pass, cudaFuncAttributeMaxDynamicSharedMemorySize, (int)sizeof(ProtSmem));
        done = true;
    }
    return err;
}

int g_cham_flag_impl = 6;
static void launch_flag_pass(uint32_t nruns, cudaStream_t stream, const uint32_t* in, uint64_t nquads, uint32_t ntiles, uint32_t* sigw,
                             uint2* unres, uint32_t* unres_count, uint32_t* final_tab, const uint8_t* copymap, const Status* gate) {
    if (g_cham_flag_impl == 1)
        cham_flag_pass<<<nruns, FP_THREADS, sizeof(FlagSmem), stream>>>(in, nquads, ntiles, nruns, sigw, unres, unres_count, final_tab, copymap, gate);
    else
        cham_flag_pass6<<<nruns, F6_THREADS, sizeof(Flag6Smem), stream>>>(in, nquads, ntiles, nruns, sigw, unres, unres_count, final_tab, copymap, gate);
}

static cudaError_t prot_iterate_coop(int ctas, cudaStream_t stream, const uint32_t* sigw, uint64_t nbytes, uint64_t nblocks, uint32_t nseg, Status* st, int it,
                                     uint8_t* inc, uint8_t* cm_old, uint8_t* cm_new, uint32_t* in_state, uint32_t* out_state, uint16_t* ptab) {
    void* args[] = {&sigw, &nbytes, &nblocks, &nseg, &st, &it, &inc, &cm_old, &cm_new, &in_state, &out_state, &ptab};
    return cudaLaunchCooperativeKernel(reinterpret_cast<const void*>(prot_iterate), dim3((unsigned)ctas), dim3(PI_THREADS), args, 0, stream);
}

cudaError_t prot_debug_read(unsigned long long* out32) { return cudaMemcpyFromSymbol(out32, g_prot_dbg, sizeof(unsigned long long) * 32); }

size_t prot_state_bytes(uint64_t nseg_max) { return (2 * (nseg_max + 2) + 64) * sizeof(uint32_t) + prot_table_elems(nseg_max) * sizeof(uint16_t); }

uint32_t cham_pick_runs(size_t nbytes, int num_sms) {
    const uint64_t nblocks = (nbytes + 255) / 256;
    const uint64_t ntiles = (nblocks + 63) / 64;
    uint64_t r = ntiles / 16;
    if (r < 1) r = 1;
    if (r > (uint64_t)num_sms) r = num_sms;
    return (uint32_t)r;
}

cudaError_t cham_encode_phase1(const uint8_t* d_in, size_t nbytes, uint8_t* ws, const ChamLayout& L, uint32_t nruns,
                               uint32_t* d_table_out, cudaStream_t stream, uint64_t* launches, cudaEvent_t* ev) {
    cudaError_t e = set_smem_attrs_once();
    if (e != cudaSuccess) return e;
    const uint64_t nquads = nbytes / 4;
    const uint64_t nblocks = (nbytes + 255) / 256;
    const uint32_t ntiles = (uint32_t)((nblocks + 63) / 64);
    Status* st = reinterpret_cast<Status*>(ws + L.status);
    e = cudaMemsetAsync(st, 0, sizeof(Status), stream);
    if (e != cudaSuccess) return e;
    {
        e = cudaMemsetAsync(&st->first_nonquiet_block, 0xFF, sizeof(unsigned long long), stream);
        if (e != cudaSuccess) return e;
    }
    if (nblocks == 0) return cudaSuccess;
    if (ev) cudaEventRecord(ev[0], stream);
    launch_flag_pass(nruns, stream, reinterpret_cast<const uint32_t*>(d_in), nquads, ntiles, reinterpret_cast<uint32_t*>(ws + L.sigw),
        reinterpret_cast<uint2*>(ws + L.unres), reinterpret_cast<uint32_t*>(ws + L.unres_count),
        reinterpret_cast<uint32_t*>(ws + L.final_tab), nullptr, nullptr);
    ++*launches;
    if (ev) cudaEventRecord(ev[1], stream);
    if (d_table_out) {
        cham_carry_scan<<<65536 / 256, 256, 0, stream>>>(reinterpret_cast<uint32_t*>(ws + L.final_tab), nullptr, 1, nruns,
                                                        nullptr, d_table_out);
        ++*launches;
    }
    return cudaGetLastError();
}

cudaError_t cham_phase2_begin(const uint8_t* d_in, size_t nbytes, uint8_t* ws, const ChamLayout& L, uint32_t nruns, const uint32_t* d_carry_in,
                              bool assume_prev_inc, cudaStream_t stream, uint64_t* launches) {
    (void)d_in;
    const uint64_t nblocks = (nbytes + 255) / 256;
    const uint32_t ntiles = (uint32_t)((nblocks + 63) / 64);
    Status* st = reinterpret_cast<Status*>(ws + L.status);
    uint32_t* sigw = reinterpret_cast<uint32_t*>(ws + L.sigw);
    cham_carry_scan<<<65536 / 256, 256, 0, stream>>>(reinterpret_cast<uint32_t*>(ws + L.final_tab), d_carry_in, 0, nruns,
                                                    reinterpret_cast<uint32_t*>(ws + L.carry), nullptr);
    cham_resolve<<<dim3(32, nruns), 256, 0, stream>>>(reinterpret_cast<uint2*>(ws + L.unres), reinterpret_cast<uint32_t*>(ws + L.unres_count),
                                                     reinterpret_cast<uint32_t*>(ws + L.carry), ntiles, nruns, sigw);
    cham_tile_sizes<<<(ntiles + 7) / 8, 256, 0, stream>>>(sigw, nullptr, nbytes, nblocks, ntiles, 0, 1, assume_prev_inc ? 1 : 0, st,
                                                          reinterpret_cast<uint32_t*>(ws + L.tile_bytes));
    *launches += 3;
    return cudaGetLastError();
}

cudaError_t cham_phase2_rounds(const uint8_t* d_in, size_t nbytes, uint8_t* ws, const ChamLayout& L, uint32_t nruns, const uint32_t* d_carry_in,
                               int it_first, int it_last, bool reset_barriers, cudaStream_t stream, uint64_t* launches) {
    const uint64_t nblocks = (nbytes + 255) / 256;
    const uint32_t ntiles = (uint32_t)((nblocks + 63) / 64);
    Status* st = reinterpret_cast<Status*>(ws + L.status);
    uint32_t* sigw = reinterpret_cast<uint32_t*>(ws + L.sigw);
    uint8_t* copymap = ws + L.copymap;
    uint8_t* copymap2 = ws + L.copymap2;
    uint32_t* seg_state = reinterpret_cast<uint32_t*>(ws + L.seg_state);
    uint8_t* incb = ws + L.incb;
    int num_ctas = 0;
    { int dev = 0; cudaGetDevice(&dev); cudaDeviceGetAttribute(&num_ctas, cudaDevAttrMultiProcessorCount, dev); if (num_ctas < 1) num_ctas = 1; }
    const uint32_t nseg = (uint32_t)((nblocks + PSEG - 1) / PSEG);
    const uint32_t* in32 = reinterpret_cast<const uint32_t*>(d_in);
    const uint64_t nquads = nbytes / 4;
    if (it_last - it_first >= 8) return cudaErrorInvalidValue;
    if (reset_barriers) {
        cudaError_t e = cudaMemsetAsync(st->barrier, 0, sizeof(st->barrier), stream);
        if (e != cudaSuccess) return e;
    }
    for (int it = it_first; it <= it_last; ++it) {
        if (it > 0) {
            launch_flag_pass(nruns, stream, in32, nquads, ntiles, sigw,
                reinterpret_cast<uint2*>(ws + L.unres), reinterpret_cast<uint32_t*>(ws + L.unres_count),
                reinterpret_cast<uint32_t*>(ws + L.final_tab), copymap, st);
            cham_carry_scan<<<65536 / 256, 256, 0, stream>>>(reinterpret_cast<uint32_t*>(ws + L.final_tab), d_carry_in, 0, nruns,
                                                            reinterpret_cast<uint32_t*>(ws + L.carry), nullptr, st);
            cham_resolve<<<dim3(32, nruns), 256, 0, stream>>>(reinterpret_cast<uint2*>(ws + L.unres), reinterpret_cast<uint32_t*>(ws + L.unres_count),
                                                             reinterpret_cast<uint32_t*>(ws + L.carry), ntiles, nruns, sigw, st);
            *launches += 3;
        }
        {
            cudaError_t le = prot_iterate_coop(num_ctas, stream, sigw, nbytes, nblocks, nseg, st, it, incb, copymap, copymap2, seg_state, seg_state + (nseg + 1),
                                               reinterpret_cast<uint16_t*>(seg_state + 2 * (nseg + 1)));
            if (le != cudaSuccess) return le;
        }
        ++*launches;
    }
    return cudaGetLastError();
}

cudaError_t cham_phase2_finish(const uint8_t* d_in, size_t nbytes, uint8_t* ws, const ChamLayout& L, uint8_t* d_out, size_t cap,
                               uint64_t* d_out_size, bool with_copy_map, cudaStream_t stream, uint64_t* launches, cudaEvent_t* ev,
                               bool inorder_fallback = true) {
    const uint64_t nblocks = (nbytes + 255) / 256;
    const uint32_t ntiles = (uint32_t)((nblocks + 63) / 64);
    const uint32_t ngroups = (ntiles + SCAN_G - 1) / SCAN_G;
    Status* st = reinterpret_cast<Status*>(ws + L.status);
    uint32_t* sigw = reinterpret_cast<uint32_t*>(ws + L.sigw);
    uint8_t* copymap = ws + L.copymap;
    if (with_copy_map) {
        if (inorder_fallback) { cham_protected_pass<<<1, 1024, sizeof(ProtSmem), stream>>>(reinterpret_cast<const uint32_t*>(d_in), nbytes, st, 1, sigw, copymap); ++*launches; }
        cham_tile_sizes<<<(ntiles + 7) / 8, 256, 0, stream>>>(sigw, copymap, nbytes, nblocks, ntiles, 1, 0, 0, st,
                                                              reinterpret_cast<uint32_t*>(ws + L.tile_bytes));
        ++*launches;
    }
    scan_groups_local<<<ngroups, SCAN_T, 0, stream>>>(reinterpret_cast<uint32_t*>(ws + L.tile_bytes), ntiles,
                                                      reinterpret_cast<uint32_t*>(ws + L.tile_local),
                                                      reinterpret_cast<uint64_t*>(ws + L.group_total));
    scan_group_totals<<<1, SCAN_T, 0, stream>>>(reinterpret_cast<uint64_t*>(ws + L.group_total), ngroups,
                                                reinterpret_cast<uint64_t*>(ws + L.group_off), st, (uint64_t)cap, d_out_size);
    *launches += 2;
    if (ev) cudaEventRecord(ev[2], stream);
    if ((reinterpret_cast<uintptr_t>(d_in) & 15u) == 0)
        cham_emit<true><<<ntiles, EM_THREADS, 0, stream>>>(reinterpret_cast<const uint32_t*>(d_in), nbytes, nblocks, sigw,
                                                           with_copy_map ? copymap : nullptr, 1, st,
                                                           reinterpret_cast<uint32_t*>(ws + L.tile_local),
                                                           reinterpret_cast<uint64_t*>(ws + L.group_off), d_out);
    else
        cham_emit<false><<<ntiles, EM_THREADS, 0, stream>>>(reinterpret_cast<const uint32_t*>(d_in), nbytes, nblocks, sigw,
                                                            with_copy_map ? copymap : nullptr, 1, st,
                                                            reinterpret_cast<uint32_t*>(ws + L.tile_local),
                                                            reinterpret_cast<uint64_t*>(ws + L.group_off), d_out);
    ++*launches;
    if (ev) cudaEventRecord(ev[3], stream);
    return cudaGetLastError();
}

cudaError_t cham_phase2_needs_more(uint8_t* ws, const ChamLayout& L, cudaStream_t stream, bool* more) {
    Status h;
    cudaError_t e = cudaMemcpyAsync(&h, ws + L.status, sizeof h, cudaMemcpyDeviceToHost, stream);
    if (e == cudaSuccess) e = cudaStreamSynchronize(stream);
    if (e != cudaSuccess) return e;
    *more = h.nonquiet && !h.converged && !h.error;
    return cudaSuccess;
}

constexpr int PROT_ITERS = 4;

cudaError_t cham_encode_phase2(const uint8_t* d_in, size_t nbytes, uint8_t* ws, const ChamLayout& L, uint32_t nruns,
                               const uint32_t* d_carry_in, uint8_t* d_out, size_t cap, uint64_t* d_out_size,
                               bool allow_protected_fallback, bool assume_prev_inc, cudaStream_t stream, uint64_t* launches,
                               cudaEvent_t* ev) {
    if (nbytes == 0) return cudaMemsetAsync(d_out_size, 0, sizeof(uint64_t), stream);
    cudaError_t e = cham_phase2_begin(d_in, nbytes, ws, L, nruns, d_carry_in, assume_prev_inc, stream, launches);
    if (e == cudaSuccess && allow_protected_fallback)
        e = cham_phase2_rounds(d_in, nbytes, ws, L, nruns, d_carry_in, 0, PROT_ITERS, false, stream, launches);
    if (e == cudaSuccess) e = cham_phase2_finish(d_in, nbytes, ws, L, d_out, cap, d_out_size, allow_protected_fallback, stream, launches, ev);
    return e;
}

cudaError_t cham_encode_phase2_blocking(const uint8_t* d_in, size_t nbytes, uint8_t* ws, const ChamLayout& L, uint32_t nruns, uint8_t* d_out,
                                        size_t cap, uint64_t* d_out_size, int max_batches, cudaStream_t stream, uint64_t* launches) {
    if (nbytes == 0) return cudaMemsetAsync(d_out_size, 0, sizeof(uint64_t), stream);
    cudaError_t e = cham_phase2_begin(d_in, nbytes, ws, L, nruns, nullptr, false, stream, launches);
    if (e == cudaSuccess) e = cham_phase2_rounds(d_in, nbytes, ws, L, nruns, nullptr, 0, PROT_ITERS, false, stream, launches);
    for (int batch = 0; e == cudaSuccess && batch < max_batches; ++batch) {
        bool more = false;
        e = cham_phase2_needs_more(ws, L, stream, &more);
        if (e != cudaSuccess || !more) break;
        e = cham_phase2_rounds(d_in, nbytes, ws, L, nruns, nullptr, 8, 15, true, stream, launches);
    }
    if (e == cudaSuccess) e = cham_phase2_finish(d_in, nbytes, ws, L, d_out, cap, d_out_size, true, stream, launches, nullptr);
    return e;
}

cudaError_t cham_encode_phase2_stream(const uint8_t* d_in, size_t nbytes, uint8_t* ws, const ChamLayout& L, uint32_t nruns, const uint32_t* d_carry_in,
                                      uint8_t* d_out, size_t cap, uint64_t* d_out_size, uint32_t* d_table_out, int max_batches, cudaStream_t stream,
                                      uint64_t* launches, bool* ok) {
    *ok = true;
    if (nbytes == 0) return cudaMemsetAsync(d_out_size, 0, sizeof(uint64_t), stream);
    cudaError_t e = cham_phase2_begin(d_in, nbytes, ws, L, nruns, d_carry_in, false, stream, launches);
    if (e == cudaSuccess) e = cham_phase2_rounds(d_in, nbytes, ws, L, nruns, d_carry_in, 0, PROT_ITERS, false, stream, launches);
    bool more = false;
    for (int batch = 0; e == cudaSuccess; ++batch) {
        e = cham_phase2_needs_more(ws, L, stream, &more);
        if (e != cudaSuccess || !more || batch >= max_batches) break;
        e = cham_phase2_rounds(d_in, nbytes, ws, L, nruns, d_carry_in, 8, 15, true, stream, launches);
    }
    if (e != cudaSuccess) return e;
    if (more) { *ok = false; return cudaSuccess; }
    e = cham_phase2_finish(d_in, nbytes, ws, L, d_out, cap, d_out_size, true, stream, launches, nullptr, false);
    if (e == cudaSuccess) {
        cham_carry_scan<<<65536 / 256, 256, 0, stream>>>(reinterpret_cast<uint32_t*>(ws + L.final_tab), nullptr, 1, nruns, nullptr, d_table_out);
        ++*launches;
        e = cudaGetLastError();
    }
    return e;
}
cudaError_t cham_quads_to_table(const uint32_t* d_quads, uint32_t* d_table, cudaStream_t stream, uint64_t* launches) {
    cham_quads_to_table_k<<<65536 / 256, 256, 0, stream>>>(d_quads, d_table);
    ++*launches;
    return cudaGetLastError();
}
cudaError_t cham_table_into_quads(const uint32_t* d_table, uint32_t* d_quads, cudaStream_t stream, uint64_t* launches) {
    cham_table_into_quads_k<<<65536 / 256, 256, 0, stream>>>(d_table, d_quads);
    ++*launches;
    return cudaGetLastError();
}

cudaError_t cham_status_accumulate(const uint8_t* ws, const ChamLayout& L, uint32_t* d_flag, cudaStream_t stream, uint64_t* launches) {
    cham_status_accumulate_k<<<1, 1, 0, stream>>>(reinterpret_cast<const Status*>(ws + L.status), d_flag);
    ++*launches;
    return cudaGetLastError();
}
cudaError_t prot_iterate_launch(const uint32_t* sigw_or_null, uint64_t nbytes, uint64_t nblocks, uint32_t nseg, Status* st, int it, uint8_t* inc,
                                uint8_t* cm_old, uint8_t* cm_new, uint32_t* in_state, uint32_t* out_state, int , int num_sms,
                                cudaStream_t stream) {
    int ctas = num_sms > 0 ? num_sms : 1;
    if ((uint32_t)ctas > nseg) ctas = nseg ? (int)nseg : 1;
    return prot_iterate_coop(ctas, stream, sigw_or_null, nbytes, nblocks, nseg, st, it, inc, cm_old, cm_new, in_state, out_state,
                             reinterpret_cast<uint16_t*>(out_state + (nseg + 1)));

}
cudaError_t scan_tiles_launch(const uint32_t* tile_bytes, uint32_t ntiles, uint32_t* tile_local, uint64_t* group_total, uint64_t* group_off,
                              uint32_t ngroups, Status* st, uint64_t cap, uint64_t* d_out_size, cudaStream_t stream) {
    scan_groups_local<<<ngroups, SCAN_T, 0, stream>>>(tile_bytes, ntiles, tile_local, group_total);
    scan_group_totals<<<1, SCAN_T, 0, stream>>>(group_total, ngroups, group_off, st, cap, d_out_size);
    return cudaGetLastError();
}
cudaError_t cham_rank_fold(const uint32_t* d_tables, uint32_t rank, uint32_t* d_carry, cudaStream_t stream, uint64_t* launches) {
    cham_rank_fold_k<<<65536 / 256, 256, 0, stream>>>(d_tables, rank, d_carry);
    ++*launches;
    return cudaGetLastError();
}
cudaError_t cham_seam_words(const uint8_t* ws, const ChamLayout& L, size_t nbytes, const uint64_t* d_out_size, uint32_t* d_words, cudaStream_t stream, uint64_t* launches) {
    cham_seam_words_k<<<1, 1, 0, stream>>>(reinterpret_cast<const uint32_t*>(ws + L.sigw), nbytes, (nbytes + 255) / 256,
                                           reinterpret_cast<const Status*>(ws + L.status), d_out_size, d_words);
    ++*launches;
    return cudaGetLastError();
}
cudaError_t cham_seam_verdict(const uint32_t* d_all_words, uint32_t world, uint32_t rank, uint32_t* d_flags, uint64_t* d_total, uint64_t* d_offsets,
                              cudaStream_t stream, uint64_t* launches) {
    cham_seam_verdict_k<<<1, 1, 0, stream>>>(d_all_words, world, rank, d_flags, d_total, d_offsets);
    ++*launches;
    return cudaGetLastError();
}
cudaError_t cham_table_init(uint32_t* d_table, cudaStream_t stream, uint64_t* launches) {
    cham_table_init_k<<<65536 / 256, 256, 0, stream>>>(d_table);
    ++*launches;
    return cudaGetLastError();
}
cudaError_t cham_table_fold(uint32_t* d_acc, const uint32_t* d_next, cudaStream_t stream, uint64_t* launches) {
    cham_table_fold_k<<<65536 / 256, 256, 0, stream>>>(d_acc, d_next);
    ++*launches;
    return cudaGetLastError();
}

cudaError_t cham_encode_protected_only(const uint8_t* d_in, size_t nbytes, uint8_t* ws, const ChamLayout& L, uint8_t* d_out,
                                       size_t cap, uint64_t* d_out_size, cudaStream_t stream, uint64_t* launches) {
    cudaError_t e = set_smem_attrs_once();
    if (e != cudaSuccess) return e;
    const uint64_t nblocks = (nbytes + 255) / 256;
    const uint32_t ntiles = (uint32_t)((nblocks + 63) / 64);
    const uint32_t ngroups = (ntiles + SCAN_G - 1) / SCAN_G;
    Status* st = reinterpret_cast<Status*>(ws + L.status);
    uint32_t* sigw = reinterpret_cast<uint32_t*>(ws + L.sigw);
    uint8_t* copymap = ws + L.copymap;
    e = cudaMemsetAsync(st, 0, sizeof(Status), stream);
    if (e != cudaSuccess) return e;
    if (nblocks == 0) return cudaMemsetAsync(d_out_size, 0, sizeof(uint64_t), stream);
    cham_protected_pass<<<1, 1024, sizeof(ProtSmem), stream>>>(reinterpret_cast<const uint32_t*>(d_in), nbytes, st, 0, sigw, copymap);
    ++*launches;
    cham_tile_sizes<<<(ntiles + 7) / 8, 256, 0, stream>>>(sigw, copymap, nbytes, nblocks, ntiles, 0, 0, 0, st,
                                                          reinterpret_cast<uint32_t*>(ws + L.tile_bytes));
    ++*launches;
    scan_groups_local<<<ngroups, SCAN_T, 0, stream>>>(reinterpret_cast<uint32_t*>(ws + L.tile_bytes), ntiles,
                                                      reinterpret_cast<uint32_t*>(ws + L.tile_local),
                                                      reinterpret_cast<uint64_t*>(ws + L.group_total));
    ++*launches;
    scan_group_totals<<<1, SCAN_T, 0, stream>>>(reinterpret_cast<uint64_t*>(ws + L.group_total), ngroups,
                                                reinterpret_cast<uint64_t*>(ws + L.group_off), st, (uint64_t)cap, d_out_size);
    ++*launches;
    cham_emit<false><<<ntiles, EM_THREADS, 0, stream>>>(reinterpret_cast<const uint32_t*>(d_in), nbytes, nblocks, sigw, copymap, 0, st,
                                                        reinterpret_cast<uint32_t*>(ws + L.tile_local),
                                                        reinterpret_cast<uint64_t*>(ws + L.group_off), d_out);
    ++*launches;
    return cudaGetLastError();
}

}
```

### density_b200/csrc/encode_internal.cuh

```cuda
#pragma once
#include <cuda_runtime.h>
#include <stdint.h>
#include <stddef.h>

namespace dns {

struct ChamLayout {
    size_t status, sigw, copymap, copymap2, seg_state, incb, tile_bytes, tile_local, group_total, group_off, unres, unres_count, final_tab, carry, total;
};

size_t cham_workspace_bytes(size_t nbytes, int nruns_max, ChamLayout* L);
uint32_t cham_pick_runs(size_t nbytes, int num_sms);
extern int g_cham_decode_impl;
extern int g_cham_flag_impl;
cudaError_t cham_encode_phase1(const uint8_t* d_in, size_t nbytes, uint8_t* ws, const ChamLayout& L, uint32_t nruns,
                               uint32_t* d_table_out, cudaStream_t stream, uint64_t* launches, cudaEvent_t* ev = nullptr);
cudaError_t cham_encode_phase2(const uint8_t* d_in, size_t nbytes, uint8_t* ws, const ChamLayout& L, uint32_t nruns,
                               const uint32_t* d_carry_in, uint8_t* d_out, size_t cap, uint64_t* d_out_size,
                               bool allow_protected_fallback, bool assume_prev_inc, cudaStream_t stream, uint64_t* launches,
                               cudaEvent_t* ev = nullptr);
cudaError_t cham_encode_phase2_blocking(const uint8_t* d_in, size_t nbytes, uint8_t* ws, const ChamLayout& L, uint32_t nruns, uint8_t* d_out,
                                        size_t cap, uint64_t* d_out_size, int max_batches, cudaStream_t stream, uint64_t* launches);
cudaError_t cham_encode_protected_only(const uint8_t* d_in, size_t nbytes, uint8_t* ws, const ChamLayout& L, uint8_t* d_out,
                                       size_t cap, uint64_t* d_out_size, cudaStream_t stream, uint64_t* launches);

cudaError_t cham_quads_to_table(const uint32_t* d_quads, uint32_t* d_table, cudaStream_t stream, uint64_t* launches);
cudaError_t cham_table_into_quads(const uint32_t* d_table, uint32_t* d_quads, cudaStream_t stream, uint64_t* launches);
cudaError_t cham_encode_phase2_stream(const uint8_t* d_in, size_t nbytes, uint8_t* ws, const ChamLayout& L, uint32_t nruns, const uint32_t* d_carry_in,
                                      uint8_t* d_out, size_t cap, uint64_t* d_out_size, uint32_t* d_table_out, int max_batches, cudaStream_t stream,
                                      uint64_t* launches, bool* ok);

struct Status;
size_t prot_state_bytes(uint64_t nseg_max);
cudaError_t prot_debug_read(unsigned long long* out32);
cudaError_t prot_iterate_launch(const uint32_t* sigw_or_null, uint64_t nbytes, uint64_t nblocks, uint32_t nseg, Status* st, int it, uint8_t* inc,
                                uint8_t* cm_old, uint8_t* cm_new, uint32_t* in_state, uint32_t* out_state, int block_bytes, int num_sms,
                                cudaStream_t stream);
cudaError_t scan_tiles_launch(const uint32_t* tile_bytes, uint32_t ntiles, uint32_t* tile_local, uint64_t* group_total, uint64_t* group_off,
                              uint32_t ngroups, Status* st, uint64_t cap, uint64_t* d_out_size, cudaStream_t stream);

extern int g_chee_stage_rounds;
size_t chee_workspace_bytes(size_t nbytes, int num_sms);
size_t chee_tables_bytes(int alg, int region, size_t nbytes, int num_sms);
cudaError_t chee_encode_parallel(int alg, const uint8_t* d_in, size_t nbytes, uint8_t* d_out, size_t cap, uint8_t* ws, uint8_t* const tables[3],
                                 uint32_t epoch_base, int num_sms, uint64_t* d_out_size, uint32_t* d_converged, bool resume,
                                 cudaStream_t stream, uint64_t* launches);

size_t cham_decode_workspace_bytes(size_t nbytes, size_t cap, int nruns_max);
cudaError_t cham_decode_parallel(const uint8_t* d_in, size_t nbytes, uint8_t* d_out, size_t cap, uint8_t* ws, int num_sms,
                                 uint64_t* d_out_size, uint32_t* d_nonquiet, cudaStream_t stream, uint64_t* launches);
cudaError_t cham_decode_phase1(const uint8_t* d_in, size_t nbytes, size_t cap, uint8_t* ws, int num_sms, uint32_t* d_table_out,
                               cudaStream_t stream, uint64_t* launches);
cudaError_t cham_decode_phase2(const uint8_t* d_in, size_t nbytes, uint8_t* d_out, size_t cap, uint8_t* ws, int num_sms, const uint32_t* d_carry_in,
                               uint64_t* d_out_size, cudaStream_t stream, uint64_t* launches);
cudaError_t cham_decode_seam_words(const uint8_t* d_in, size_t nbytes, size_t cap, uint8_t* ws, int num_sms, int is_last, const uint64_t* d_out_size,
                                   uint32_t* d_words, cudaStream_t stream, uint64_t* launches);
size_t cham_locate_workspace_bytes(size_t nbytes);
cudaError_t cham_decode_locate(const uint8_t* d_in, size_t n_range, size_t n_halo, uint8_t* ws, uint64_t* d_map, cudaStream_t stream,
                               uint64_t* launches);

size_t chee_decode_workspace_bytes(size_t nbytes, size_t cap, int num_sms);
size_t chee_decode_tables_bytes(size_t nbytes, int num_sms);
cudaError_t chee_decode_parallel(const uint8_t* d_in, size_t nbytes, uint8_t* d_out, size_t cap, uint8_t* ws, uint8_t* tables, uint8_t* tail_ws,
                                 int num_sms, uint64_t* d_out_size, uint32_t* d_fallback, cudaStream_t stream, uint64_t* launches);
const void* chee_decode_status_ptr(uint8_t* ws, size_t nbytes, size_t cap, int num_sms, const void** cl_status);

size_t scalar_workspace_bytes(int alg);
cudaError_t scalar_encode(int alg, const uint8_t* d_in, size_t nbytes, uint8_t* d_out, size_t cap, uint8_t* ws,
                          uint64_t* d_out_size, cudaStream_t stream, uint64_t* launches, const uint32_t* d_run_if_zero = nullptr, bool keep_state = false);
cudaError_t scalar_decode(int alg, const uint8_t* d_in, size_t nbytes, uint8_t* d_out, size_t cap, uint8_t* ws,
                          uint64_t* d_out_size, cudaStream_t stream, uint64_t* launches, const uint32_t* d_run_if = nullptr, bool keep_state = false);
cudaError_t scalar_decode_tail(int alg, const uint8_t* d_in, size_t nbytes, uint8_t* d_out, size_t cap, uint8_t* ws, const void* d_bounds_status,
                               const void* d_cl_status, uint64_t* d_out_size, cudaStream_t stream, uint64_t* launches, const uint32_t* d_skip_if);

cudaError_t cham_status_accumulate(const uint8_t* ws, const ChamLayout& L, uint32_t* d_flag, cudaStream_t stream, uint64_t* launches);
cudaError_t cham_table_init(uint32_t* d_table, cudaStream_t stream, uint64_t* launches);
cudaError_t cham_rank_fold(const uint32_t* d_tables, uint32_t rank, uint32_t* d_carry, cudaStream_t stream, uint64_t* launches);
cudaError_t cham_seam_words(const uint8_t* ws, const ChamLayout& L, size_t nbytes, const uint64_t* d_out_size, uint32_t* d_words, cudaStream_t stream, uint64_t* launches);
cudaError_t cham_seam_verdict(const uint32_t* d_all_words, uint32_t world, uint32_t rank, uint32_t* d_flags, uint64_t* d_total, uint64_t* d_offsets,
                              cudaStream_t stream, uint64_t* launches);
cudaError_t cham_table_fold(uint32_t* d_acc, const uint32_t* d_next, cudaStream_t stream, uint64_t* launches);

}
```

Before: 479.3.

## Fuse chameleon phase-2 middle kernels into a cooperative kernel and cached conditional graph

The separate carry-scan, resolve, tile-size and two scan kernels are replaced by one cooperative kernel, cham_mid, which runs the selected steps with grid-wide syncs between them. The fallback path is captured into a cached CUDA graph whose conditional node runs the protected rounds only when the nonquiet flag is set. The resolve step now combines bits within a warp before issuing its atomics. The aim is to cut kernel launch overhead and host round trips between small kernels. In exchange it adds grid syncs, graph rebuild and update logic, and a dependency on cooperative launch and conditional-graph support.

Result: faster. 492.7 (median of 6 runs) (+2.8%).

```diff
diff --git a/density_b200/csrc/api.cu b/density_b200/csrc/api.cu
--- a/density_b200/csrc/api.cu
+++ b/density_b200/csrc/api.cu
@@ -1177,6 +1177,7 @@
         cudaSetDevice(d);
         c.ws.release(); c.stage_in.release(); c.stage_out.release(); c.dec_tables.release(); for (int a2 = 0; a2 < 2; ++a2) for (int rg = 0; rg < 3; ++rg) c.chee_tables[a2][rg].release();
         c.chee_epoch = 0;
+        cham_mid_graph_release();
         if (c.d_size) cudaFree(c.d_size);
         if (c.h_size) cudaFreeHost(c.h_size);
         if (c.stream) cudaStreamDestroy(c.stream);
diff --git a/density_b200/csrc/chameleon_encode.cu b/density_b200/csrc/chameleon_encode.cu
--- a/density_b200/csrc/chameleon_encode.cu
+++ b/density_b200/csrc/chameleon_encode.cu
@@ -1,9 +1,11 @@
 #include <cstdio>
+#include <cooperative_groups.h>
 #include "common.cuh"
 #include "encode_internal.cuh"
 
 namespace dns {
 namespace cham {
+namespace cg = cooperative_groups;
 
 constexpr int FP_THREADS = 1024;
 constexpr int FP_QPT = 4;
@@ -699,38 +701,6 @@
 }
 
 __device__ __forceinline__ bool gate_open(const Status* g) { return !g || (g->nonquiet && !g->converged); }
-
-__global__ void cham_carry_scan(const uint32_t* __restrict__ final_tab, const uint32_t* __restrict__ init, int init_untouched,
-                                uint32_t nruns, uint32_t* __restrict__ carry, uint32_t* __restrict__ table_out,
-                                const Status* __restrict__ gate = nullptr) {
-    if (!gate_open(gate)) return;
-    uint32_t hb = blockIdx.x * blockDim.x + threadIdx.x;
-    if (hb >= 65536) return;
-    uint32_t c = init ? init[hb] : ((hb == 0 && !init_untouched) ? 0x10000u : 0u);
-    for (uint32_t r = 0; r < nruns; ++r) {
-        if (carry) carry[(size_t)r * 65536 + hb] = c;
-        uint32_t v = final_tab[(size_t)r * 65536 + hb];
-        if (v & 0x10000u) c = v;
-    }
-    if (table_out) table_out[hb] = c;
-}
-
-__global__ void cham_resolve(const uint2* __restrict__ unres, const uint32_t* __restrict__ unres_count,
-                             const uint32_t* __restrict__ carry, uint32_t tiles_total, uint32_t nruns,
-                             uint32_t* __restrict__ sigw_g, const Status* __restrict__ gate = nullptr) {
-    if (!gate_open(gate)) return;
-    const uint32_t run = blockIdx.y;
-    const uint32_t n = unres_count[run];
-    const uint64_t run_q0 = ((uint64_t)run * tiles_total / nruns) * TILE_Q;
-    for (uint32_t i = blockIdx.x * blockDim.x + threadIdx.x; i < n; i += gridDim.x * blockDim.x) {
-        uint2 e = unres[(size_t)run * 65536 + i];
-        uint32_t c = carry[(size_t)run * 65536 + (e.y & 0xFFFFu)];
-        if ((c & 0x10000u) && (c & 0xFFFFu) == (e.y >> 16)) {
-            uint64_t gq = run_q0 + e.x;
-            atomicOr(&sigw_g[gq >> 5], 1u << (gq & 31));
-        }
-    }
-}
 
 struct ProtSmem {
     uint16_t tab[65536];
@@ -1024,47 +994,6 @@
     return copied ? blen : 8 + blen - 2 * hits;
 }
 
-__global__ void cham_tile_sizes(const uint32_t* __restrict__ sigw_g, const uint8_t* __restrict__ copymap, uint64_t nbytes,
-                                uint64_t nblocks, uint32_t ntiles, int use_copymap_if_nonquiet, int check_quiet, int assume_prev_inc,
-                                Status* __restrict__ status, uint32_t* __restrict__ tile_bytes) {
-    const uint32_t lane = threadIdx.x & 31;
-    const uint32_t tile = blockIdx.x * (blockDim.x >> 5) + (threadIdx.x >> 5);
-    if (tile >= ntiles) return;
-    if (use_copymap_if_nonquiet && !check_quiet && !status->nonquiet) return;
-    const bool use_cm = copymap && (!use_copymap_if_nonquiet || status->nonquiet);
-    uint32_t sum = 0, incm[2];
-#pragma unroll
-    for (int k = 0; k < 2; ++k) {
-        const uint64_t b = (uint64_t)tile * 64 + k * 32 + lane;
-        uint32_t sz = 0; bool inc = false;
-        if (b < nblocks) {
-            const bool copied = use_cm && copymap[b];
-            const uint32_t hits = __popc(sigw_g[2 * b]) + __popc(sigw_g[2 * b + 1]);
-            sz = block_out_bytes(b, nbytes, hits, copied);
-            inc = !copied && sz >= 256 && (nbytes - b * 256 >= 256);
-        }
-        sum += sz;
-        incm[k] = __ballot_sync(0xFFFFFFFFu, inc);
-    }
-#pragma unroll
-    for (int d = 16; d; d >>= 1) sum += __shfl_xor_sync(0xFFFFFFFFu, sum, d);
-    if (lane == 0) tile_bytes[tile] = sum;
-    if (check_quiet && lane == 0) {
-        bool prev = assume_prev_inc != 0;
-        if (tile > 0) {
-            const uint64_t b = (uint64_t)tile * 64 - 1;
-            const uint32_t hits = __popc(sigw_g[2 * b]) + __popc(sigw_g[2 * b + 1]);
-            prev = (8 + 256 - 2 * hits) >= 256;
-        }
-        const uint64_t m = ((uint64_t)incm[1] << 32) | incm[0];
-        const uint64_t pairs = m & ((m << 1) | (prev ? 1ull : 0ull));
-        if (pairs) {
-            atomicOr(&status->nonquiet, 1u);
-            atomicMin(&status->first_nonquiet_block, (unsigned long long)tile * 64 + (__ffsll((long long)pairs) - 1));
-        }
-    }
-}
-
 constexpr int SCAN_T = 1024;
 constexpr int SCAN_PER = 4;
 constexpr int SCAN_G = SCAN_T * SCAN_PER;
@@ -1125,6 +1054,217 @@
         if (total > cap) { status->error = 2; total = 0; }
         status->out_bytes = total;
         if (d_out_size) *d_out_size = total;
+    }
+}
+
+constexpr uint32_t MID_FOLD = 1, MID_RESOLVE = 2, MID_SIZES = 4, MID_SCAN = 8;
+constexpr int MID_THREADS = 1024;
+constexpr int MID_FOLD_U = 16;
+constexpr int MID_RES_U = 8;
+constexpr int MID_SZ_U = 4;
+
+struct MidParams {
+    uint32_t steps;
+    uint32_t nruns, ntiles;
+    uint64_t nbytes;
+    const uint32_t* final_tab;
+    const uint32_t* init;
+    int init_untouched;
+    uint32_t* carry;
+    uint32_t* table_out;
+    const uint2* unres;
+    const uint32_t* unres_count;
+    uint32_t* sigw;
+    const uint8_t* copymap;
+    int use_copymap_if_nonquiet;
+    int check_quiet, assume_prev_inc;
+    Status* st;
+    const Status* gate;
+    uint32_t* tile_bytes;
+    uint32_t* tile_local;
+    uint64_t* group_total;
+    uint64_t* group_off;
+    uint64_t cap;
+    uint64_t* d_out_size;
+    int set_cond;
+    cudaGraphConditionalHandle cond;
+};
+
+__device__ __forceinline__ uint2 ldcg_u2(const uint32_t* p) { return __ldcg(reinterpret_cast<const uint2*>(p)); }
+
+__global__ void __launch_bounds__(MID_THREADS, 1) cham_mid(const MidParams p) {
+    if (!gate_open(p.gate)) return;
+    cg::grid_group grid = cg::this_grid();
+    __shared__ uint64_t s_warp[33];
+    __shared__ uint64_t s_carry;
+    const uint32_t tid = threadIdx.x, lane = tid & 31, warp = tid >> 5;
+    const uint64_t nblocks = (p.nbytes + 255) / 256;
+
+    if (p.steps & MID_FOLD) {
+        const uint32_t per = ((65536 + gridDim.x - 1) / gridDim.x + 31) & ~31u;
+        for (uint32_t i = tid; i < per; i += blockDim.x) {
+            const uint32_t h = blockIdx.x * per + i;
+            if (h >= 65536) break;
+            uint32_t c = p.init ? p.init[h] : ((h == 0 && !p.init_untouched) ? 0x10000u : 0u);
+            const uint32_t* ft = p.final_tab + h;
+            uint32_t* cr = p.carry ? p.carry + h : nullptr;
+            uint32_t r = 0;
+            for (; r + MID_FOLD_U <= p.nruns; r += MID_FOLD_U) {
+                uint32_t v[MID_FOLD_U];
+#pragma unroll
+                for (int k = 0; k < MID_FOLD_U; ++k) v[k] = __ldcg(ft + (size_t)(r + k) * 65536);
+#pragma unroll
+                for (int k = 0; k < MID_FOLD_U; ++k) {
+                    if (cr) cr[(size_t)(r + k) * 65536] = c;
+                    if (v[k] & 0x10000u) c = v[k];
+                }
+            }
+            for (; r < p.nruns; ++r) {
+                const uint32_t v = __ldcg(ft + (size_t)r * 65536);
+                if (cr) cr[(size_t)r * 65536] = c;
+                if (v & 0x10000u) c = v;
+            }
+            if (p.table_out) p.table_out[h] = c;
+        }
+        if (p.steps != MID_FOLD) grid.sync();
+    }
+
+    if (p.steps & MID_RESOLVE) {
+        constexpr uint32_t CH = 32 * MID_RES_U, CH_PER_RUN = 65536 / CH;
+        const uint32_t nw = gridDim.x * (blockDim.x >> 5);
+        for (uint32_t ch = blockIdx.x * (blockDim.x >> 5) + warp; ch < p.nruns * CH_PER_RUN; ch += nw) {
+            const uint32_t run = ch / CH_PER_RUN, i0 = (ch % CH_PER_RUN) * CH;
+            const uint32_t n = __ldcg(&p.unres_count[run]);
+            if (i0 >= n) continue;
+            const uint64_t run_q0 = ((uint64_t)run * p.ntiles / p.nruns) * TILE_Q;
+            const uint2* ur = p.unres + (size_t)run * 65536;
+            const uint32_t* cr = p.carry + (size_t)run * 65536;
+            {
+                uint2 e[MID_RES_U];
+                uint32_t c[MID_RES_U];
+#pragma unroll
+                for (int k = 0; k < MID_RES_U; ++k) {
+                    const uint32_t i = i0 + k * 32 + lane;
+                    e[k] = i < n ? __ldcg(&ur[i]) : make_uint2(0xFFFFFFFFu, 0);
+                }
+#pragma unroll
+                for (int k = 0; k < MID_RES_U; ++k) c[k] = e[k].x != 0xFFFFFFFFu ? __ldcg(&cr[e[k].y & 0xFFFFu]) : 0u;
+#pragma unroll
+                for (int k = 0; k < MID_RES_U; ++k) {
+                    const bool hit = (c[k] & 0x10000u) && (c[k] & 0xFFFFu) == (e[k].y >> 16);
+                    const uint64_t gq = run_q0 + e[k].x;
+                    const uint32_t word = e[k].x != 0xFFFFFFFFu ? (uint32_t)(gq >> 5) : 0xFFFFFFFFu;
+                    uint32_t bits = hit ? 1u << (gq & 31) : 0u;
+#pragma unroll
+                    for (int d = 1; d < 32; d <<= 1) {
+                        const uint32_t ow = __shfl_down_sync(0xFFFFFFFFu, word, d), ob = __shfl_down_sync(0xFFFFFFFFu, bits, d);
+                        if (lane + d < 32 && ow == word) bits |= ob;
+                    }
+                    const uint32_t below = __shfl_up_sync(0xFFFFFFFFu, word, 1);
+                    if (bits && (lane == 0 || below != word)) atomicOr(&p.sigw[word], bits);
+                }
+            }
+        }
+        if (p.steps & (MID_SIZES | MID_SCAN)) grid.sync();
+    }
+
+    if (p.steps & MID_SIZES) {
+        const bool skip = p.use_copymap_if_nonquiet && !p.check_quiet && !*((volatile const unsigned int*)&p.st->nonquiet);
+        if (!skip) {
+            const bool use_cm = p.copymap && (!p.use_copymap_if_nonquiet || *((volatile const unsigned int*)&p.st->nonquiet));
+            const uint32_t nw = gridDim.x * (blockDim.x >> 5);
+            for (uint32_t t0 = blockIdx.x * (blockDim.x >> 5) + warp; t0 < p.ntiles; t0 += nw * MID_SZ_U) {
+                uint2 s[MID_SZ_U][2];
+                uint32_t prevw[MID_SZ_U];
+                uint8_t cm[MID_SZ_U][2];
+#pragma unroll
+                for (int j = 0; j < MID_SZ_U; ++j) {
+                    const uint32_t tile = t0 + j * nw;
+#pragma unroll
+                    for (int k = 0; k < 2; ++k) {
+                        const uint64_t b = (uint64_t)tile * 64 + k * 32 + lane;
+                        const bool ok = tile < p.ntiles && b < nblocks;
+                        s[j][k] = ok ? ldcg_u2(p.sigw + 2 * b) : make_uint2(0, 0);
+                        cm[j][k] = (ok && use_cm) ? p.copymap[b] : 0;
+                    }
+                    prevw[j] = 0;
+                    if (p.check_quiet && lane == 0 && tile < p.ntiles && tile > 0) {
+                        const uint2 pv = ldcg_u2(p.sigw + 2 * ((uint64_t)tile * 64 - 1));
+                        prevw[j] = __popc(pv.x) + __popc(pv.y);
+                    }
+                }
+#pragma unroll
+                for (int j = 0; j < MID_SZ_U; ++j) {
+                    const uint32_t tile = t0 + j * nw;
+                    if (tile >= p.ntiles) break;
+                    uint32_t sum = 0, incm[2];
+#pragma unroll
+                    for (int k = 0; k < 2; ++k) {
+                        const uint64_t b = (uint64_t)tile * 64 + k * 32 + lane;
+                        uint32_t sz = 0; bool inc = false;
+                        if (b < nblocks) {
+                            const bool copied = cm[j][k] != 0;
+                            sz = block_out_bytes(b, p.nbytes, __popc(s[j][k].x) + __popc(s[j][k].y), copied);
+                            inc = !copied && sz >= 256 && (p.nbytes - b * 256 >= 256);
+                        }
+                        sum += sz;
+                        incm[k] = __ballot_sync(0xFFFFFFFFu, inc);
+                    }
+#pragma unroll
+                    for (int d = 16; d; d >>= 1) sum += __shfl_xor_sync(0xFFFFFFFFu, sum, d);
+                    if (lane == 0) p.tile_bytes[tile] = sum;
+                    if (p.check_quiet && lane == 0) {
+                        bool prev = p.assume_prev_inc != 0;
+                        if (tile > 0) prev = (8 + 256 - 2 * prevw[j]) >= 256;
+                        const uint64_t m = ((uint64_t)incm[1] << 32) | incm[0];
+                        const uint64_t pairs = m & ((m << 1) | (prev ? 1ull : 0ull));
+                        if (pairs) {
+                            atomicOr(&p.st->nonquiet, 1u);
+                            atomicMin(&p.st->first_nonquiet_block, (unsigned long long)tile * 64 + (__ffsll((long long)pairs) - 1));
+                        }
+                    }
+                }
+            }
+        }
+        if (p.set_cond || (p.steps & MID_SCAN)) grid.sync();
+        if (p.set_cond && blockIdx.x == 0 && tid == 0) cudaGraphSetConditional(p.cond, *((volatile unsigned int*)&p.st->nonquiet) ? 1u : 0u);
+    }
+
+    if (p.steps & MID_SCAN) {
+        const uint32_t ngroups = (p.ntiles + SCAN_G - 1) / SCAN_G;
+        for (uint32_t g = blockIdx.x; g < ngroups; g += gridDim.x) {
+            const uint32_t base = g * SCAN_G + tid * SCAN_PER;
+            uint32_t v[SCAN_PER]; uint64_t sum = 0;
+#pragma unroll
+            for (int k = 0; k < SCAN_PER; ++k) { v[k] = (base + k < p.ntiles) ? __ldcg(&p.tile_bytes[base + k]) : 0u; sum += v[k]; }
+            uint64_t tot;
+            uint64_t ex = block_exclusive_scan_u64(sum, s_warp, &tot);
+#pragma unroll
+            for (int k = 0; k < SCAN_PER; ++k) { if (base + k < p.ntiles) p.tile_local[base + k] = (uint32_t)ex; ex += v[k]; }
+            if (tid == 0) p.group_total[g] = tot;
+            __syncthreads();
+        }
+        grid.sync();
+        if (blockIdx.x == 0) {
+            if (tid == 0) s_carry = 0;
+            __syncthreads();
+            for (uint32_t base = 0; base < ngroups; base += blockDim.x) {
+                const uint32_t i = base + tid;
+                const uint64_t v = (i < ngroups) ? __ldcg(&p.group_total[i]) : 0;
+                uint64_t tot;
+                const uint64_t ex = block_exclusive_scan_u64(v, s_warp, &tot);
+                if (i < ngroups) p.group_off[i] = s_carry + ex;
+                __syncthreads();
+                if (tid == 0) s_carry += tot;
+                __syncthreads();
+            }
+            if (tid == 0) {
+                uint64_t total = s_carry;
+                if (total > p.cap) { p.st->error = 2; total = 0; }
+                p.st->out_bytes = total;
+                if (p.d_out_size) *p.d_out_size = total;
+            }
+        }
     }
 }
 
@@ -1393,10 +1533,50 @@
         cham_flag_pass6<<<nruns, F6_THREADS, sizeof(Flag6Smem), stream>>>(in, nquads, ntiles, nruns, sigw, unres, unres_count, final_tab, copymap, gate);
 }
 
+template <typename... Args>
+static cudaError_t launch_coop(void (*k)(Args...), int ctas, int threads, cudaStream_t stream, Args... args) {
+    cudaLaunchConfig_t cfg = {};
+    cfg.gridDim = dim3((unsigned)ctas); cfg.blockDim = dim3((unsigned)threads); cfg.stream = stream;
+    cudaLaunchAttribute attr;
+    attr.id = cudaLaunchAttributeCooperative; attr.val.cooperative = 1;
+    cfg.attrs = &attr; cfg.numAttrs = 1;
+    return cudaLaunchKernelEx(&cfg, k, args...);
+}
+
 static cudaError_t prot_iterate_coop(int ctas, cudaStream_t stream, const uint32_t* sigw, uint64_t nbytes, uint64_t nblocks, uint32_t nseg, Status* st, int it,
                                      uint8_t* inc, uint8_t* cm_old, uint8_t* cm_new, uint32_t* in_state, uint32_t* out_state, uint16_t* ptab) {
-    void* args[] = {&sigw, &nbytes, &nblocks, &nseg, &st, &it, &inc, &cm_old, &cm_new, &in_state, &out_state, &ptab};
-    return cudaLaunchCooperativeKernel(reinterpret_cast<const void*>(prot_iterate), dim3((unsigned)ctas), dim3(PI_THREADS), args, 0, stream);
+    return launch_coop(prot_iterate, ctas, PI_THREADS, stream, sigw, nbytes, nblocks, nseg, st, it, inc, cm_old, cm_new, in_state, out_state, ptab);
+}
+
+static int device_sms() {
+    int dev = 0, n = 0;
+    cudaGetDevice(&dev);
+    cudaDeviceGetAttribute(&n, cudaDevAttrMultiProcessorCount, dev);
+    return n < 1 ? 1 : n;
+}
+
+static MidParams mid_params(uint32_t steps, size_t nbytes, uint8_t* ws, const ChamLayout& L, uint32_t nruns) {
+    MidParams p = {};
+    p.steps = steps;
+    p.nruns = nruns;
+    p.nbytes = nbytes;
+    p.ntiles = (uint32_t)(((nbytes + 255) / 256 + 63) / 64);
+    p.final_tab = reinterpret_cast<uint32_t*>(ws + L.final_tab);
+    p.carry = reinterpret_cast<uint32_t*>(ws + L.carry);
+    p.unres = reinterpret_cast<uint2*>(ws + L.unres);
+    p.unres_count = reinterpret_cast<uint32_t*>(ws + L.unres_count);
+    p.sigw = reinterpret_cast<uint32_t*>(ws + L.sigw);
+    p.st = reinterpret_cast<Status*>(ws + L.status);
+    p.tile_bytes = reinterpret_cast<uint32_t*>(ws + L.tile_bytes);
+    p.tile_local = reinterpret_cast<uint32_t*>(ws + L.tile_local);
+    p.group_total = reinterpret_cast<uint64_t*>(ws + L.group_total);
+    p.group_off = reinterpret_cast<uint64_t*>(ws + L.group_off);
+    return p;
+}
+
+static cudaError_t launch_mid(const MidParams& p, cudaStream_t stream, uint64_t* launches) {
+    ++*launches;
+    return launch_coop(cham_mid, device_sms(), MID_THREADS, stream, p);
 }
 
 cudaError_t prot_debug_read(unsigned long long* out32) { return cudaMemcpyFromSymbol(out32, g_prot_dbg, sizeof(unsigned long long) * 32); }
@@ -1434,28 +1614,23 @@
     ++*launches;
     if (ev) cudaEventRecord(ev[1], stream);
     if (d_table_out) {
-        cham_carry_scan<<<65536 / 256, 256, 0, stream>>>(reinterpret_cast<uint32_t*>(ws + L.final_tab), nullptr, 1, nruns,
-                                                        nullptr, d_table_out);
-        ++*launches;
+        MidParams p = mid_params(MID_FOLD, nbytes, ws, L, nruns);
+        p.carry = nullptr; p.init_untouched = 1; p.table_out = d_table_out;
+        e = launch_mid(p, stream, launches);
+        if (e != cudaSuccess) return e;
     }
     return cudaGetLastError();
 }
 
 cudaError_t cham_phase2_begin(const uint8_t* d_in, size_t nbytes, uint8_t* ws, const ChamLayout& L, uint32_t nruns, const uint32_t* d_carry_in,
-                              bool assume_prev_inc, cudaStream_t stream, uint64_t* launches) {
+                              bool assume_prev_inc, cudaStream_t stream, uint64_t* launches, const cudaGraphConditionalHandle* cond = nullptr) {
     (void)d_in;
-    const uint64_t nblocks = (nbytes + 255) / 256;
-    const uint32_t ntiles = (uint32_t)((nblocks + 63) / 64);
-    Status* st = reinterpret_cast<Status*>(ws + L.status);
-    uint32_t* sigw = reinterpret_cast<uint32_t*>(ws + L.sigw);
-    cham_carry_scan<<<65536 / 256, 256, 0, stream>>>(reinterpret_cast<uint32_t*>(ws + L.final_tab), d_carry_in, 0, nruns,
-                                                    reinterpret_cast<uint32_t*>(ws + L.carry), nullptr);
-    cham_resolve<<<dim3(32, nruns), 256, 0, stream>>>(reinterpret_cast<uint2*>(ws + L.unres), reinterpret_cast<uint32_t*>(ws + L.unres_count),
-                                                     reinterpret_cast<uint32_t*>(ws + L.carry), ntiles, nruns, sigw);
-    cham_tile_sizes<<<(ntiles + 7) / 8, 256, 0, stream>>>(sigw, nullptr, nbytes, nblocks, ntiles, 0, 1, assume_prev_inc ? 1 : 0, st,
-                                                          reinterpret_cast<uint32_t*>(ws + L.tile_bytes));
-    *launches += 3;
-    return cudaGetLastError();
+    MidParams p = mid_params(MID_FOLD | MID_RESOLVE | MID_SIZES, nbytes, ws, L, nruns);
+    p.init = d_carry_in;
+    p.check_quiet = 1;
+    p.assume_prev_inc = assume_prev_inc ? 1 : 0;
+    if (cond) { p.set_cond = 1; p.cond = *cond; }
+    return launch_mid(p, stream, launches);
 }
 
 cudaError_t cham_phase2_rounds(const uint8_t* d_in, size_t nbytes, uint8_t* ws, const ChamLayout& L, uint32_t nruns, const uint32_t* d_carry_in,
@@ -1468,8 +1643,7 @@
     uint8_t* copymap2 = ws + L.copymap2;
     uint32_t* seg_state = reinterpret_cast<uint32_t*>(ws + L.seg_state);
     uint8_t* incb = ws + L.incb;
-    int num_ctas = 0;
-    { int dev = 0; cudaGetDevice(&dev); cudaDeviceGetAttribute(&num_ctas, cudaDevAttrMultiProcessorCount, dev); if (num_ctas < 1) num_ctas = 1; }
+    const int num_ctas = device_sms();
     const uint32_t nseg = (uint32_t)((nblocks + PSEG - 1) / PSEG);
     const uint32_t* in32 = reinterpret_cast<const uint32_t*>(d_in);
     const uint64_t nquads = nbytes / 4;
@@ -1483,11 +1657,12 @@
             launch_flag_pass(nruns, stream, in32, nquads, ntiles, sigw,
                 reinterpret_cast<uint2*>(ws + L.unres), reinterpret_cast<uint32_t*>(ws + L.unres_count),
                 reinterpret_cast<uint32_t*>(ws + L.final_tab), copymap, st);
-            cham_carry_scan<<<65536 / 256, 256, 0, stream>>>(reinterpret_cast<uint32_t*>(ws + L.final_tab), d_carry_in, 0, nruns,
-                                                            reinterpret_cast<uint32_t*>(ws + L.carry), nullptr, st);
-            cham_resolve<<<dim3(32, nruns), 256, 0, stream>>>(reinterpret_cast<uint2*>(ws + L.unres), reinterpret_cast<uint32_t*>(ws + L.unres_count),
-                                                             reinterpret_cast<uint32_t*>(ws + L.carry), ntiles, nruns, sigw, st);
-            *launches += 3;
+            ++*launches;
+            MidParams p = mid_params(MID_FOLD | MID_RESOLVE, nbytes, ws, L, nruns);
+            p.init = d_carry_in;
+            p.gate = st;
+            cudaError_t le = launch_mid(p, stream, launches);
+            if (le != cudaSuccess) return le;
         }
         {
             cudaError_t le = prot_iterate_coop(num_ctas, stream, sigw, nbytes, nblocks, nseg, st, it, incb, copymap, copymap2, seg_state, seg_state + (nseg + 1),
@@ -1499,41 +1674,50 @@
     return cudaGetLastError();
 }
 
-cudaError_t cham_phase2_finish(const uint8_t* d_in, size_t nbytes, uint8_t* ws, const ChamLayout& L, uint8_t* d_out, size_t cap,
-                               uint64_t* d_out_size, bool with_copy_map, cudaStream_t stream, uint64_t* launches, cudaEvent_t* ev,
-                               bool inorder_fallback = true) {
+static cudaError_t phase2_copy_map_sizes(const uint8_t* d_in, size_t nbytes, uint8_t* ws, const ChamLayout& L, MidParams& p, bool inorder_fallback,
+                                         cudaStream_t stream, uint64_t* launches) {
+    if (inorder_fallback) {
+        cham_protected_pass<<<1, 1024, sizeof(ProtSmem), stream>>>(reinterpret_cast<const uint32_t*>(d_in), nbytes, reinterpret_cast<Status*>(ws + L.status),
+                                                                  1, reinterpret_cast<uint32_t*>(ws + L.sigw), ws + L.copymap);
+        ++*launches;
+    }
+    p.steps |= MID_SIZES;
+    p.copymap = ws + L.copymap;
+    p.use_copymap_if_nonquiet = 1;
+    return cudaGetLastError();
+}
+
+static cudaError_t phase2_emit(const uint8_t* d_in, size_t nbytes, uint8_t* ws, const ChamLayout& L, uint8_t* d_out, bool with_copy_map,
+                               cudaStream_t stream, uint64_t* launches, cudaEvent_t* ev) {
     const uint64_t nblocks = (nbytes + 255) / 256;
     const uint32_t ntiles = (uint32_t)((nblocks + 63) / 64);
-    const uint32_t ngroups = (ntiles + SCAN_G - 1) / SCAN_G;
-    Status* st = reinterpret_cast<Status*>(ws + L.status);
-    uint32_t* sigw = reinterpret_cast<uint32_t*>(ws + L.sigw);
-    uint8_t* copymap = ws + L.copymap;
-    if (with_copy_map) {
-        if (inorder_fallback) { cham_protected_pass<<<1, 1024, sizeof(ProtSmem), stream>>>(reinterpret_cast<const uint32_t*>(d_in), nbytes, st, 1, sigw, copymap); ++*launches; }
-        cham_tile_sizes<<<(ntiles + 7) / 8, 256, 0, stream>>>(sigw, copymap, nbytes, nblocks, ntiles, 1, 0, 0, st,
-                                                              reinterpret_cast<uint32_t*>(ws + L.tile_bytes));
-        ++*launches;
-    }
-    scan_groups_local<<<ngroups, SCAN_T, 0, stream>>>(reinterpret_cast<uint32_t*>(ws + L.tile_bytes), ntiles,
-                                                      reinterpret_cast<uint32_t*>(ws + L.tile_local),
-                                                      reinterpret_cast<uint64_t*>(ws + L.group_total));
-    scan_group_totals<<<1, SCAN_T, 0, stream>>>(reinterpret_cast<uint64_t*>(ws + L.group_total), ngroups,
-                                                reinterpret_cast<uint64_t*>(ws + L.group_off), st, (uint64_t)cap, d_out_size);
-    *launches += 2;
+    const Status* st = reinterpret_cast<const Status*>(ws + L.status);
+    const uint32_t* sigw = reinterpret_cast<const uint32_t*>(ws + L.sigw);
+    const uint8_t* copymap = with_copy_map ? ws + L.copymap : nullptr;
     if (ev) cudaEventRecord(ev[2], stream);
     if ((reinterpret_cast<uintptr_t>(d_in) & 15u) == 0)
-        cham_emit<true><<<ntiles, EM_THREADS, 0, stream>>>(reinterpret_cast<const uint32_t*>(d_in), nbytes, nblocks, sigw,
-                                                           with_copy_map ? copymap : nullptr, 1, st,
+        cham_emit<true><<<ntiles, EM_THREADS, 0, stream>>>(reinterpret_cast<const uint32_t*>(d_in), nbytes, nblocks, sigw, copymap, 1, st,
                                                            reinterpret_cast<uint32_t*>(ws + L.tile_local),
                                                            reinterpret_cast<uint64_t*>(ws + L.group_off), d_out);
     else
-        cham_emit<false><<<ntiles, EM_THREADS, 0, stream>>>(reinterpret_cast<const uint32_t*>(d_in), nbytes, nblocks, sigw,
-                                                            with_copy_map ? copymap : nullptr, 1, st,
+        cham_emit<false><<<ntiles, EM_THREADS, 0, stream>>>(reinterpret_cast<const uint32_t*>(d_in), nbytes, nblocks, sigw, copymap, 1, st,
                                                             reinterpret_cast<uint32_t*>(ws + L.tile_local),
                                                             reinterpret_cast<uint64_t*>(ws + L.group_off), d_out);
     ++*launches;
     if (ev) cudaEventRecord(ev[3], stream);
     return cudaGetLastError();
+}
+
+cudaError_t cham_phase2_finish(const uint8_t* d_in, size_t nbytes, uint8_t* ws, const ChamLayout& L, uint8_t* d_out, size_t cap,
+                               uint64_t* d_out_size, bool with_copy_map, cudaStream_t stream, uint64_t* launches, cudaEvent_t* ev,
+                               bool inorder_fallback = true) {
+    MidParams p = mid_params(MID_SCAN, nbytes, ws, L, 0);
+    p.cap = cap;
+    p.d_out_size = d_out_size;
+    cudaError_t e = with_copy_map ? phase2_copy_map_sizes(d_in, nbytes, ws, L, p, inorder_fallback, stream, launches) : cudaSuccess;
+    if (e == cudaSuccess) e = launch_mid(p, stream, launches);
+    if (e == cudaSuccess) e = phase2_emit(d_in, nbytes, ws, L, d_out, with_copy_map, stream, launches, ev);
+    return e;
 }
 
 cudaError_t cham_phase2_needs_more(uint8_t* ws, const ChamLayout& L, cudaStream_t stream, bool* more) {
@@ -1547,15 +1731,124 @@
 
 constexpr int PROT_ITERS = 4;
 
+struct MidGraphKey {
+    const uint8_t* d_in; size_t nbytes; uint8_t* ws; uint32_t nruns; const uint32_t* d_carry_in; bool assume_prev_inc; size_t cap;
+    uint64_t* d_out_size; int flag_impl; int sms;
+    bool same(const MidGraphKey& o) const {
+        return d_in == o.d_in && nbytes == o.nbytes && ws == o.ws && nruns == o.nruns && d_carry_in == o.d_carry_in &&
+               assume_prev_inc == o.assume_prev_inc && cap == o.cap && d_out_size == o.d_out_size && flag_impl == o.flag_impl && sms == o.sms;
+    }
+};
+struct MidGraph { cudaGraph_t graph = nullptr; cudaGraphExec_t exec = nullptr; cudaStream_t cs = nullptr; MidGraphKey key{}; };
+constexpr int MID_GRAPH_DEVICES = 64;
+static MidGraph g_mid_graph[MID_GRAPH_DEVICES];
+
+template <typename F>
+static cudaError_t capture_into(cudaStream_t cs, cudaGraph_t g, const cudaGraphNode_t* deps, size_t ndeps, F enqueue) {
+    cudaError_t e = cudaStreamBeginCaptureToGraph(cs, g, deps, nullptr, ndeps, cudaStreamCaptureModeThreadLocal);
+    if (e != cudaSuccess) return e;
+    const cudaError_t fe = enqueue();
+    cudaGraph_t captured = nullptr;
+    e = cudaStreamEndCapture(cs, &captured);
+    return fe != cudaSuccess ? fe : e;
+}
+
+static cudaError_t mid_graph_build(const MidGraphKey& k, const ChamLayout& L, cudaStream_t cs, cudaGraph_t* out) {
+    uint64_t n = 0;
+    cudaGraph_t g = nullptr;
+    cudaError_t e = cudaGraphCreate(&g, 0);
+    if (e != cudaSuccess) return e;
+    cudaGraphConditionalHandle h = 0;
+    e = cudaGraphConditionalHandleCreate(&h, g, 0, cudaGraphCondAssignDefault);
+    if (e == cudaSuccess)
+        e = capture_into(cs, g, nullptr, 0, [&] { return cham_phase2_begin(k.d_in, k.nbytes, k.ws, L, k.nruns, k.d_carry_in, k.assume_prev_inc, cs, &n, &h); });
+    cudaGraphNode_t begin = nullptr, cond = nullptr;
+    size_t nn = 1;
+    if (e == cudaSuccess) e = cudaGraphGetNodes(g, &begin, &nn);
+    cudaGraphNodeParams cp = {};
+    cp.type = cudaGraphNodeTypeConditional;
+    cp.conditional.handle = h;
+    cp.conditional.type = cudaGraphCondTypeIf;
+    cp.conditional.size = 1;
+    if (e == cudaSuccess) e = cudaGraphAddNode(&cond, g, &begin, 1, &cp);
+    if (e == cudaSuccess)
+        e = capture_into(cs, cp.conditional.phGraph_out[0], nullptr, 0, [&] {
+            cudaError_t r = cham_phase2_rounds(k.d_in, k.nbytes, k.ws, L, k.nruns, k.d_carry_in, 0, PROT_ITERS, false, cs, &n);
+            MidParams p = mid_params(0, k.nbytes, k.ws, L, 0);
+            if (r == cudaSuccess) r = phase2_copy_map_sizes(k.d_in, k.nbytes, k.ws, L, p, true, cs, &n);
+            if (r == cudaSuccess) r = launch_mid(p, cs, &n);
+            return r;
+        });
+    if (e == cudaSuccess)
+        e = capture_into(cs, g, &cond, 1, [&] {
+            MidParams p = mid_params(MID_SCAN, k.nbytes, k.ws, L, 0);
+            p.cap = k.cap;
+            p.d_out_size = k.d_out_size;
+            return launch_mid(p, cs, &n);
+        });
+    if (e != cudaSuccess) { cudaGraphDestroy(g); return e; }
+    *out = g;
+    return cudaSuccess;
+}
+
+static cudaError_t mid_graph_launch(const MidGraphKey& k, const ChamLayout& L, cudaStream_t stream, uint64_t* launches) {
+    int dev = 0;
+    cudaError_t e = cudaGetDevice(&dev);
+    if (e != cudaSuccess) return e;
+    if (dev < 0 || dev >= MID_GRAPH_DEVICES) return cudaErrorInvalidDevice;
+    MidGraph& G = g_mid_graph[dev];
+    if (!G.exec || !G.key.same(k)) {
+        if (!G.cs) {
+            e = cudaStreamCreateWithFlags(&G.cs, cudaStreamNonBlocking);
+            if (e != cudaSuccess) return e;
+        }
+        cudaGraph_t ng = nullptr;
+        e = mid_graph_build(k, L, G.cs, &ng);
+        if (e != cudaSuccess) return e;
+        if (G.exec && (G.key.flag_impl != k.flag_impl || G.key.sms != k.sms)) { cudaGraphExecDestroy(G.exec); G.exec = nullptr; }
+        if (G.exec) {
+            cudaGraphExecUpdateResultInfo info;
+            if (cudaGraphExecUpdate(G.exec, ng, &info) != cudaSuccess) { cudaGetLastError(); cudaGraphExecDestroy(G.exec); G.exec = nullptr; }
+        }
+        if (!G.exec) e = cudaGraphInstantiate(&G.exec, ng, 0);
+        if (G.graph) cudaGraphDestroy(G.graph);
+        G.graph = ng;
+        G.key = k;
+        if (e != cudaSuccess) { G.exec = nullptr; return e; }
+    }
+    *launches += 2;
+    return cudaGraphLaunch(G.exec, stream);
+}
+
+void cham_mid_graph_release() {
+    int dev = 0;
+    if (cudaGetDevice(&dev) != cudaSuccess || dev < 0 || dev >= MID_GRAPH_DEVICES) return;
+    MidGraph& G = g_mid_graph[dev];
+    if (G.exec) cudaGraphExecDestroy(G.exec);
+    if (G.graph) cudaGraphDestroy(G.graph);
+    if (G.cs) cudaStreamDestroy(G.cs);
+    G = MidGraph{};
+}
+
 cudaError_t cham_encode_phase2(const uint8_t* d_in, size_t nbytes, uint8_t* ws, const ChamLayout& L, uint32_t nruns,
                                const uint32_t* d_carry_in, uint8_t* d_out, size_t cap, uint64_t* d_out_size,
                                bool allow_protected_fallback, bool assume_prev_inc, cudaStream_t stream, uint64_t* launches,
                                cudaEvent_t* ev) {
     if (nbytes == 0) return cudaMemsetAsync(d_out_size, 0, sizeof(uint64_t), stream);
-    cudaError_t e = cham_phase2_begin(d_in, nbytes, ws, L, nruns, d_carry_in, assume_prev_inc, stream, launches);
-    if (e == cudaSuccess && allow_protected_fallback)
-        e = cham_phase2_rounds(d_in, nbytes, ws, L, nruns, d_carry_in, 0, PROT_ITERS, false, stream, launches);
-    if (e == cudaSuccess) e = cham_phase2_finish(d_in, nbytes, ws, L, d_out, cap, d_out_size, allow_protected_fallback, stream, launches, ev);
+    cudaError_t e;
+    if (allow_protected_fallback) {
+        const MidGraphKey k{d_in, nbytes, ws, nruns, d_carry_in, assume_prev_inc, cap, d_out_size, g_cham_flag_impl, device_sms()};
+        e = mid_graph_launch(k, L, stream, launches);
+    } else {
+        MidParams p = mid_params(MID_FOLD | MID_RESOLVE | MID_SIZES | MID_SCAN, nbytes, ws, L, nruns);
+        p.init = d_carry_in;
+        p.check_quiet = 1;
+        p.assume_prev_inc = assume_prev_inc ? 1 : 0;
+        p.cap = cap;
+        p.d_out_size = d_out_size;
+        e = launch_mid(p, stream, launches);
+    }
+    if (e == cudaSuccess) e = phase2_emit(d_in, nbytes, ws, L, d_out, allow_protected_fallback, stream, launches, ev);
     return e;
 }
 
@@ -1591,9 +1884,9 @@
     if (more) { *ok = false; return cudaSuccess; }
     e = cham_phase2_finish(d_in, nbytes, ws, L, d_out, cap, d_out_size, true, stream, launches, nullptr, false);
     if (e == cudaSuccess) {
-        cham_carry_scan<<<65536 / 256, 256, 0, stream>>>(reinterpret_cast<uint32_t*>(ws + L.final_tab), nullptr, 1, nruns, nullptr, d_table_out);
-        ++*launches;
-        e = cudaGetLastError();
+        MidParams p = mid_params(MID_FOLD, nbytes, ws, L, nruns);
+        p.carry = nullptr; p.init_untouched = 1; p.table_out = d_table_out;
+        e = launch_mid(p, stream, launches);
     }
     return e;
 }
@@ -1662,7 +1955,6 @@
     if (e != cudaSuccess) return e;
     const uint64_t nblocks = (nbytes + 255) / 256;
     const uint32_t ntiles = (uint32_t)((nblocks + 63) / 64);
-    const uint32_t ngroups = (ntiles + SCAN_G - 1) / SCAN_G;
     Status* st = reinterpret_cast<Status*>(ws + L.status);
     uint32_t* sigw = reinterpret_cast<uint32_t*>(ws + L.sigw);
     uint8_t* copymap = ws + L.copymap;
@@ -1671,16 +1963,12 @@
     if (nblocks == 0) return cudaMemsetAsync(d_out_size, 0, sizeof(uint64_t), stream);
     cham_protected_pass<<<1, 1024, sizeof(ProtSmem), stream>>>(reinterpret_cast<const uint32_t*>(d_in), nbytes, st, 0, sigw, copymap);
     ++*launches;
-    cham_tile_sizes<<<(ntiles + 7) / 8, 256, 0, stream>>>(sigw, copymap, nbytes, nblocks, ntiles, 0, 0, 0, st,
-                                                          reinterpret_cast<uint32_t*>(ws + L.tile_bytes));
-    ++*launches;
-    scan_groups_local<<<ngroups, SCAN_T, 0, stream>>>(reinterpret_cast<uint32_t*>(ws + L.tile_bytes), ntiles,
-                                                      reinterpret_cast<uint32_t*>(ws + L.tile_local),
-                                                      reinterpret_cast<uint64_t*>(ws + L.group_total));
-    ++*launches;
-    scan_group_totals<<<1, SCAN_T, 0, stream>>>(reinterpret_cast<uint64_t*>(ws + L.group_total), ngroups,
-                                                reinterpret_cast<uint64_t*>(ws + L.group_off), st, (uint64_t)cap, d_out_size);
-    ++*launches;
+    MidParams p = mid_params(MID_SIZES | MID_SCAN, nbytes, ws, L, 0);
+    p.copymap = copymap;
+    p.cap = cap;
+    p.d_out_size = d_out_size;
+    e = launch_mid(p, stream, launches);
+    if (e != cudaSuccess) return e;
     cham_emit<false><<<ntiles, EM_THREADS, 0, stream>>>(reinterpret_cast<const uint32_t*>(d_in), nbytes, nblocks, sigw, copymap, 0, st,
                                                         reinterpret_cast<uint32_t*>(ws + L.tile_local),
                                                         reinterpret_cast<uint64_t*>(ws + L.group_off), d_out);
diff --git a/density_b200/csrc/encode_internal.cuh b/density_b200/csrc/encode_internal.cuh
--- a/density_b200/csrc/encode_internal.cuh
+++ b/density_b200/csrc/encode_internal.cuh
@@ -21,6 +21,7 @@
                                cudaEvent_t* ev = nullptr);
 cudaError_t cham_encode_phase2_blocking(const uint8_t* d_in, size_t nbytes, uint8_t* ws, const ChamLayout& L, uint32_t nruns, uint8_t* d_out,
                                         size_t cap, uint64_t* d_out_size, int max_batches, cudaStream_t stream, uint64_t* launches);
+void cham_mid_graph_release();
 cudaError_t cham_encode_protected_only(const uint8_t* d_in, size_t nbytes, uint8_t* ws, const ChamLayout& L, uint8_t* d_out,
                                        size_t cap, uint64_t* d_out_size, cudaStream_t stream, uint64_t* launches);
 
```
